# ytchen0323/cloud-scale-bwamem

Hardware: AMD Instinct MI355X
Metric: pair-end 2x150bp reads aligned/sec (higher is better)
Workload: dtype int32+u16

## Files before the change

### cloud-scale-bwamem_amd/bpsw_hip/__init__.py

```python
from __future__ import annotations

import ctypes as C
import os
from dataclasses import dataclass

import numpy as np

_HERE = os.path.dirname(os.path.abspath(__file__))
PKG_ROOT = os.path.dirname(_HERE)
LIB_PATH = os.environ.get("BPSW_LIB") or os.path.join(PKG_ROOT, "lib", "libbPSW_hip.so")
SYNTH_PATH = os.path.join(PKG_ROOT, "lib", "libbpsw_synth.so")

BPSW_OK = 0
ZDROP_SCALA, ZDROP_BWA = 0, 1
RESCUE_C, RESCUE_SCALA = 0, 1
KSW_XBYTE, KSW_XSTOP, KSW_XSUBO, KSW_XSTART = 0x10000, 0x20000, 0x40000, 0x80000

ABI_SYMBOLS = [
    "bpsw_device_count", "bpsw_create", "bpsw_destroy", "bpsw_device_of", "bpsw_device_cus", "bpsw_device_slots", "bpsw_device_for_partition", "bpsw_last_error", "bpsw_version",
    "bpsw_set_ext_scoring", "bpsw_set_ext_shortcuts", "bpsw_extend_batch", "bpsw_extend_stage", "bpsw_extend_commit", "bpsw_extend_batch_classify", "bpsw_extend_batch_device", "bpsw_wire_size", "bpsw_wire_pack", "bpsw_wire_coords_size", "bpsw_wire_coords_pack",
    "bpsw_opt_default", "bpsw_swalign2_batch", "bpsw_swalign2_batch_device", "bpsw_matesw_group", "bpsw_global_batch",
    "bpsw_get_stats", "bpsw_reset_stats", "bpsw_last_kernel_ms", "bpsw_ring_stats", "bpsw_sw_batches_in_flight", "bpsw_ring_integrity",
    "bpsw_ext_group_waiting", "bpsw_ext_group_counts",
    "bpsw_ref_load", "bpsw_ref_unload", "bpsw_ref_length", "bpsw_ref_fetch", "bpsw_chain2aln_batch",
    "bpsw_tail_opt_default", "bpsw_bns_load", "bpsw_reg2aln_batch", "bpsw_sam_pe_batch", "bpsw_worker2_batch", "bpsw_last_tail_times", "bpsw_last_tail_resubmitted",
    "bpsw_tail_pool_create", "bpsw_tail_pool_destroy", "bpsw_tail_pool_submit", "bpsw_tail_pool_wait", "bpsw_tail_pool_workers",
    "bpsw_mark_primary_se", "bpsw_approx_mapq_se", "bpsw_mem_pair", "bpsw_sort_dedup", "bpsw_pe_stat",
    "bpsw_fmi_load", "bpsw_fmi_unload", "bpsw_fmi_length", "bpsw_seed_opt_default", "bpsw_seed_batch", "bpsw_chain_seeds",
    "bpsw_worker1_batch", "bpsw_last_worker1_times", "bpsw_seed_set_resident_lanes",
    "bpsw_seed_batch_ex", "bpsw_last_seed_bytes", "bpsw_scan_set_tile",
    "bpsw_chain_batch", "bpsw_chain_set_arena_budget", "bpsw_chain_last_split",
    "bpsw_chain_batch_ex", "bpsw_last_chain_bytes",
    "bpsw_sam_se_batch", "bpsw_align_se_batch", "bpsw_last_sam_se_times",
    "bpsw_sam_pe_batch_ex", "bpsw_align_pe_batch", "bpsw_last_sam_pe_times",
    "bpsw_fastq_parse", "bpsw_align_fastq_se", "bpsw_align_fastq_pe", "bpsw_last_fastq_times",
    "bpsw_bam_se_batch", "bpsw_bam_pe_batch", "bpsw_align_bam_se_batch", "bpsw_align_bam_pe_batch", "bpsw_align_fastq_bam_se", "bpsw_align_fastq_bam_pe",
    "bpsw_sam_header", "bpsw_bam_header", "bpsw_bam_eof", "bpsw_bam_set_block_payload", "bpsw_last_bam_times", "bpsw_last_bam_deflate_times",
]
JNI_SYMBOLS = [
    "Java_cs_ucla_edu_bwaspark_jni_SWExtendFPGAJNI_swExtendFPGAJNI",
    "Java_cs_ucla_edu_bwaspark_jni_MateSWJNI_mateSWJNI",
    "Java_cs_ucla_edu_bwaspark_jni_HelloWorld_helloWorld",
    "Java_cs_ucla_edu_bwaspark_jni_MateSWJNI_loadPacJNI",
    "Java_cs_ucla_edu_bwaspark_jni_SWExtendFPGAJNI_chainToAlnJNI",
    "Java_cs_ucla_edu_bwaspark_jni_MateSWJNI_loadBnsJNI",
    "Java_cs_ucla_edu_bwaspark_jni_MateSWJNI_samPeTailJNI",
    "Java_cs_ucla_edu_bwaspark_jni_MateSWJNI_samPeTailSubmitJNI",
    "Java_cs_ucla_edu_bwaspark_jni_MateSWJNI_samPeTailCollectJNI",
    "Java_cs_ucla_edu_bwaspark_jni_MateSWJNI_samPeTailCancelJNI",
    "Java_cs_ucla_edu_bwaspark_jni_MateSWJNI_mateSWFlatJNI",
    "Java_cs_ucla_edu_bwaspark_jni_SWExtendFPGAJNI_loadFmiJNI",
    "Java_cs_ucla_edu_bwaspark_jni_SWExtendFPGAJNI_worker1FlatJNI",
]


class BpswError(RuntimeError):
    pass


class AlnReg(C.Structure):
    _fields_ = [("rb", C.c_int64), ("re", C.c_int64), ("qb", C.c_int32), ("qe", C.c_int32), ("score", C.c_int32),
                ("truesc", C.c_int32), ("sub", C.c_int32), ("csub", C.c_int32), ("sub_n", C.c_int32), ("w", C.c_int32),
                ("seedcov", C.c_int32), ("secondary", C.c_int32), ("hash", C.c_uint64)]


ALNREG_DTYPE = np.dtype([("rb", "<i8"), ("re", "<i8"), ("qb", "<i4"), ("qe", "<i4"), ("score", "<i4"),
                         ("truesc", "<i4"), ("sub", "<i4"), ("csub", "<i4"), ("sub_n", "<i4"), ("w", "<i4"),
                         ("seedcov", "<i4"), ("secondary", "<i4"), ("hash", "<u8")])
assert ALNREG_DTYPE.itemsize == 64 and C.sizeof(AlnReg) == 64


class PeStat(C.Structure):
    _fields_ = [("low", C.c_int32), ("high", C.c_int32), ("failed", C.c_int32), ("pad_", C.c_int32),
                ("avg", C.c_double), ("std", C.c_double)]


class Opt(C.Structure):
    _fields_ = [(n, C.c_int32) for n in ("a", "b", "o_del", "e_del", "o_ins", "e_ins", "pen_unpaired", "pen_clip5",
                                         "pen_clip3", "w", "zdrop", "T", "flag", "min_seed_len", "max_ins",
                                         "max_matesw")] + [("mask_level_redun", C.c_float), ("mat", C.c_int8 * 25),
                                                           ("pad_", C.c_int8 * 3)]


class ExtTasks(C.Structure):
    _fields_ = [("n", C.c_int32)] + [(n, C.c_int32) for n in ("o_del", "e_del", "o_ins", "e_ins", "pen_clip5",
                                                                "pen_clip3", "w", "mat_max")] + \
               [(n, C.c_void_p) for n in ("left_qlen", "left_rlen", "right_qlen", "right_rlen", "left_q_off",
                                          "left_r_off", "right_q_off", "right_r_off", "reg_score", "q_beg", "h0", "idx",
                                          "pool")]


class ExtCoordTasks(C.Structure):
    _fields_ = [("n", C.c_int32)] + [(n, C.c_int32) for n in ("o_del", "e_del", "o_ins", "e_ins", "pen_clip5",
                                                                "pen_clip3", "w", "mat_max")] + \
               [(n, C.c_void_p) for n in ("left_qlen", "left_rlen", "right_qlen", "right_rlen", "left_q_off", "right_q_off",
                                          "reg_score", "q_beg", "h0", "idx", "seed_len", "seed_rbeg", "pool")]


class SwJobs(C.Structure):
    _fields_ = [("n", C.c_int32), ("xtra", C.c_int32)] + \
               [(n, C.c_void_p) for n in ("q_len", "t_len", "q_off", "t_off", "q_rev", "q_pool", "t_pool")] + \
               [("q_pool_bytes", C.c_size_t), ("t_pool_bytes", C.c_size_t)]


class GlobalJobs(C.Structure):
    _fields_ = [("n", C.c_int32), ("max_cigar", C.c_int32)] + \
               [(n, C.c_void_p) for n in ("q_len", "t_len", "w", "q_off", "t_off", "q_pool", "t_pool")] + \
               [("q_pool_bytes", C.c_size_t), ("t_pool_bytes", C.c_size_t)]


class Chains(C.Structure):
    _fields_ = [("n_reads", C.c_int32), ("read_len", C.c_void_p), ("read_off", C.c_void_p), ("read_pool", C.c_void_p),
                ("read_pool_bytes", C.c_size_t), ("chain_cnt", C.c_void_p), ("seed_cnt", C.c_void_p), ("seed_rbeg", C.c_void_p),
                ("seed_qbeg", C.c_void_p), ("seed_len", C.c_void_p)]


C2A_SORT_DEDUP, C2A_DEDUP_SCALA = 1, 2
W1_CHAIN_DEVICE = 4
W1_SEED_PLAN_DEVICE = 8
W1_CHAINS_RESIDENT = 16
SEED_PLAN_DEVICE = 1
CHAIN_TABLES_DEVICE = 1


class RescueGroup(C.Structure):
    _fields_ = [("group_size", C.c_int32), ("l_pac", C.c_int64), ("pes", PeStat * 4), ("seq_len", C.c_void_p),
                ("seq_off", C.c_void_p), ("seq_pool", C.c_void_p), ("seq_pool_bytes", C.c_size_t),
                ("reg_cnt", C.c_void_p), ("regs", C.c_void_p), ("ref_cnt", C.c_void_p), ("ref_rb", C.c_void_p),
                ("ref_re", C.c_void_p), ("ref_len", C.c_void_p), ("ref_off", C.c_void_p), ("ref_pool", C.c_void_p),
                ("ref_pool_bytes", C.c_size_t)]


class Stats(C.Structure):
    _fields_ = [(n, C.c_uint64) for n in ("ext_calls", "ext_tasks", "ext_wire_bytes", "sw_calls", "sw_jobs",
                                          "sw_speculated", "sw_replayed_rounds", "sw_wasted")] + \
               [(n, C.c_double) for n in ("ext_h2d_ms", "ext_kernel_ms", "ext_d2h_ms", "sw_h2d_ms", "sw_kernel_ms",
                                          "sw_d2h_ms", "sw_host_ms", "ext_host_in_ms", "ext_wait_ms", "ext_dev_ms",
                                          "ext_host_out_ms", "grp_plan_ms", "grp_pack_ms", "grp_wait_ms", "grp_dev_ms",
                                          "grp_replay_ms", "grp_out_ms")] + [("grp_calls", C.c_uint64), ("grp_pairs", C.c_uint64), ("ext_full_relaunches", C.c_uint64), ("sw_ring_calls", C.c_uint64), ("ext_ring_calls", C.c_uint64)]


_lib = None


def load_library(path: str | None = None) -> C.CDLL:
    global _lib
    if _lib is not None and path is None:
        return _lib
    p = path or LIB_PATH
    if not os.path.exists(p):
        raise BpswError(f"{p} not found: build it with `make -C {PKG_ROOT}` (or __graft_entry__.build())")
    if os.environ.get("BPSW_NO_TORCH") != "1":
        try:
            import torch
        except Exception:
            pass
    lib = C.CDLL(p)
    lib.bpsw_last_error.restype = C.c_char_p
    lib.bpsw_version.restype = C.c_char_p
    lib.bpsw_create.argtypes = [C.c_int, C.POINTER(C.c_void_p)]
    lib.bpsw_destroy.argtypes = [C.c_void_p]
    lib.bpsw_destroy.restype = None
    lib.bpsw_device_of.argtypes = [C.c_void_p]
    lib.bpsw_device_cus.argtypes = [C.c_void_p]
    lib.bpsw_set_ext_scoring.argtypes = [C.c_void_p, C.c_void_p, C.c_int, C.c_int]
    lib.bpsw_set_ext_shortcuts.argtypes = [C.c_void_p, C.c_int]
    lib.bpsw_extend_batch.argtypes = [C.c_void_p, C.c_void_p, C.c_size_t, C.c_void_p, C.c_size_t]
    lib.bpsw_extend_batch_device.argtypes = [C.c_void_p, C.c_void_p, C.c_size_t, C.c_int, C.c_void_p, C.c_void_p]
    lib.bpsw_wire_size.argtypes = [C.POINTER(ExtTasks)]
    lib.bpsw_wire_size.restype = C.c_size_t
    lib.bpsw_wire_pack.argtypes = [C.POINTER(ExtTasks), C.c_void_p, C.c_size_t, C.POINTER(C.c_size_t)]
    lib.bpsw_wire_coords_size.argtypes = [C.POINTER(ExtCoordTasks)]
    lib.bpsw_wire_coords_size.restype = C.c_size_t
    lib.bpsw_wire_coords_pack.argtypes = [C.POINTER(ExtCoordTasks), C.c_void_p, C.c_size_t, C.POINTER(C.c_size_t)]
    lib.bpsw_opt_default.argtypes = [C.POINTER(Opt)]
    lib.bpsw_opt_default.restype = None
    lib.bpsw_swalign2_batch.argtypes = [C.c_void_p, C.POINTER(Opt), C.POINTER(SwJobs), C.c_void_p]
    lib.bpsw_swalign2_batch_device.argtypes = [C.c_void_p, C.POINTER(Opt), C.POINTER(SwJobs), C.c_void_p, C.c_void_p]
    lib.bpsw_matesw_group.argtypes = [C.c_void_p, C.POINTER(Opt), C.POINTER(RescueGroup), C.c_int, C.c_void_p,
                                      C.c_void_p, C.c_int64, C.POINTER(C.c_int64)]
    lib.bpsw_global_batch.argtypes = [C.c_void_p, C.POINTER(Opt), C.POINTER(GlobalJobs), C.c_void_p, C.c_void_p, C.c_void_p]
    lib.bpsw_get_stats.argtypes = [C.c_void_p, C.POINTER(Stats)]
    lib.bpsw_reset_stats.argtypes = [C.c_void_p]
    lib.bpsw_last_kernel_ms.argtypes = [C.c_void_p, C.POINTER(C.c_float), C.POINTER(C.c_float)]
    lib.bpsw_ring_stats.argtypes = [C.c_void_p, C.POINTER(C.c_uint64), C.POINTER(C.c_uint64), C.POINTER(C.c_uint64), C.POINTER(C.c_double), C.POINTER(C.c_uint64)]
    lib.bpsw_sw_batches_in_flight.argtypes = [C.c_int]
    lib.bpsw_ext_group_waiting.argtypes = [C.c_int]
    lib.bpsw_ext_group_counts.argtypes = [C.c_int, C.POINTER(C.c_uint64)]
    lib.bpsw_ring_integrity.argtypes = [C.POINTER(C.c_uint64), C.POINTER(C.c_uint64)]
    lib.bpsw_chain2aln_batch.argtypes = [C.c_void_p, C.POINTER(Opt), C.POINTER(Chains), C.c_int, C.c_int, C.c_void_p, C.c_void_p,
                                         C.c_int64, C.POINTER(C.c_int64)]
    lib.bpsw_ref_load.argtypes = [C.c_void_p, C.c_void_p, C.c_int64]
    lib.bpsw_ref_unload.argtypes = [C.c_void_p]
    lib.bpsw_ref_length.argtypes = [C.c_void_p]
    lib.bpsw_ref_length.restype = C.c_int64
    lib.bpsw_ref_fetch.argtypes = [C.c_void_p, C.c_int32, C.c_void_p, C.c_void_p, C.c_void_p, C.c_size_t, C.c_void_p, C.c_void_p]
    lib.bpsw_tail_opt_default.argtypes = [C.c_void_p]
    lib.bpsw_tail_opt_default.restype = None
    lib.bpsw_bns_load.argtypes = [C.c_void_p, C.c_int32, C.c_void_p, C.c_void_p, C.c_char_p]
    lib.bpsw_reg2aln_batch.argtypes = [C.c_void_p, C.POINTER(Opt), C.c_void_p, C.c_void_p, C.c_void_p, C.c_void_p, C.c_void_p]
    lib.bpsw_sam_pe_batch.argtypes = [C.c_void_p, C.POINTER(Opt), C.c_void_p, C.c_void_p, C.c_void_p, C.c_size_t, C.c_void_p,
                                      C.POINTER(C.c_size_t), C.c_void_p]
    lib.bpsw_worker2_batch.argtypes = [C.c_void_p, C.POINTER(Opt), C.c_void_p, C.c_void_p, C.c_int, C.c_void_p, C.c_size_t, C.c_void_p,
                                       C.POINTER(C.c_size_t), C.c_void_p, C.c_void_p, C.c_int64, C.POINTER(C.c_int64)]
    lib.bpsw_tail_pool_create.argtypes = [C.c_int, C.c_int, C.POINTER(C.c_void_p)]
    lib.bpsw_tail_pool_destroy.argtypes = [C.c_void_p]
    lib.bpsw_tail_pool_destroy.restype = None
    lib.bpsw_tail_pool_submit.argtypes = [C.c_void_p, C.POINTER(Opt), C.c_void_p, C.c_void_p, C.c_int, C.c_void_p, C.c_size_t, C.c_void_p,
                                          C.c_void_p, C.c_void_p, C.c_int64, C.POINTER(C.c_int64)]
    lib.bpsw_tail_pool_wait.argtypes = [C.c_void_p, C.c_int64, C.POINTER(C.c_size_t), C.POINTER(C.c_int64)]
    lib.bpsw_tail_pool_workers.argtypes = [C.c_void_p]
    lib.bpsw_mark_primary_se.argtypes = [C.POINTER(Opt), C.c_void_p, C.c_int32, C.c_void_p, C.c_int64]
    lib.bpsw_approx_mapq_se.argtypes = [C.POINTER(Opt), C.c_void_p, C.c_void_p]
    lib.bpsw_mem_pair.argtypes = [C.POINTER(Opt), C.c_void_p, C.c_int64, C.c_void_p, C.c_int32, C.c_void_p, C.c_int32, C.c_void_p, C.c_int64,
                                  C.c_void_p]
    lib.bpsw_sort_dedup.argtypes = [C.c_int32, C.c_void_p, C.c_float, C.c_int]
    lib.bpsw_pe_stat.argtypes = [C.POINTER(Opt), C.c_void_p, C.c_int64, C.c_int32, C.c_void_p, C.c_void_p, C.c_void_p]
    lib.bpsw_last_tail_times.argtypes = [C.c_void_p, C.POINTER(C.c_float), C.POINTER(C.c_int32), C.c_void_p]
    lib.bpsw_last_tail_resubmitted.argtypes = [C.c_void_p, C.POINTER(C.c_int32)]
    _bind_seeding(lib)
    if path is None:
        _lib = lib
    return lib


def _bind_seeding(lib):
    sig = {
        "bpsw_fmi_load": ([C.c_void_p, C.c_int64, C.c_void_p, C.c_int64, C.c_void_p, C.c_int64, C.c_int32, C.c_int64, C.c_void_p], C.c_int),
        "bpsw_fmi_unload": ([C.c_void_p], C.c_int),
        "bpsw_fmi_length": ([C.c_void_p], C.c_int64),
        "bpsw_seed_opt_default": ([C.c_void_p], None),
        "bpsw_seed_batch": ([C.c_void_p, C.c_void_p, C.c_void_p, C.c_void_p, C.c_void_p, C.c_int64, C.POINTER(C.c_int64), C.c_void_p, C.c_void_p,
                             C.c_int64, C.POINTER(C.c_int64)], C.c_int),
        "bpsw_seed_batch_ex": ([C.c_void_p, C.c_void_p, C.c_void_p, C.c_void_p, C.c_void_p, C.c_int64, C.POINTER(C.c_int64), C.c_void_p, C.c_void_p,
                                C.c_int64, C.POINTER(C.c_int64), C.c_int], C.c_int),
        "bpsw_last_seed_bytes": ([C.c_void_p], None),
        "bpsw_scan_set_tile": ([C.c_int], None),
        "bpsw_chain_seeds": ([C.c_void_p, C.c_int32, C.c_int64, C.c_int32, C.c_void_p, C.c_int32, C.c_void_p, C.c_int32, C.c_void_p], C.c_int),
        "bpsw_worker1_batch": ([C.c_void_p, C.POINTER(Opt), C.c_void_p, C.c_void_p, C.c_int, C.c_int, C.c_void_p, C.c_void_p, C.c_int64,
                                C.POINTER(C.c_int64)], C.c_int),
        "bpsw_last_worker1_times": ([C.c_void_p], None),
        "bpsw_seed_set_resident_lanes": ([C.c_int], None),
        "bpsw_chain_batch": ([C.c_void_p, C.c_void_p, C.c_int32, C.c_int64, C.c_int32, C.c_void_p, C.c_void_p, C.c_int32, C.c_void_p, C.c_void_p,
                              C.c_int64, C.c_void_p, C.c_int64, C.POINTER(C.c_int64), C.POINTER(C.c_int64)], C.c_int),
        "bpsw_chain_batch_ex": ([C.c_void_p, C.c_void_p, C.c_int32, C.c_int64, C.c_int32, C.c_void_p, C.c_void_p, C.c_int32, C.c_void_p, C.c_void_p,
                                 C.c_int64, C.c_void_p, C.c_int64, C.POINTER(C.c_int64), C.POINTER(C.c_int64), C.c_int], C.c_int),
        "bpsw_last_chain_bytes": ([C.c_void_p], None),
        "bpsw_chain_set_arena_budget": ([C.c_int64], None),
        "bpsw_chain_last_split": ([C.c_void_p], None),
        "bpsw_sam_se_batch": ([C.c_void_p, C.POINTER(Opt), C.c_void_p, C.c_void_p, C.c_int, C.c_void_p, C.c_size_t, C.c_void_p,
                               C.POINTER(C.c_size_t), C.c_void_p], C.c_int),
        "bpsw_align_se_batch": ([C.c_void_p, C.POINTER(Opt), C.c_void_p, C.c_void_p, C.c_void_p, C.c_int, C.c_int, C.c_int, C.c_void_p,
                                 C.c_size_t, C.c_void_p, C.POINTER(C.c_size_t)], C.c_int),
        "bpsw_last_sam_se_times": ([C.c_void_p], None),
        "bpsw_sam_pe_batch_ex": ([C.c_void_p, C.POINTER(Opt), C.c_void_p, C.c_void_p, C.c_int, C.c_void_p, C.c_size_t, C.c_void_p,
                                  C.POINTER(C.c_size_t), C.c_void_p], C.c_int),
        "bpsw_align_pe_batch": ([C.c_void_p, C.POINTER(Opt), C.c_void_p, C.c_void_p, C.c_void_p, C.c_void_p, C.c_int, C.c_int, C.c_int, C.c_int,
                                 C.c_void_p, C.c_size_t, C.c_void_p, C.POINTER(C.c_size_t), C.c_void_p], C.c_int),
        "bpsw_last_sam_pe_times": ([C.c_void_p], None),
        "bpsw_fastq_parse": ([C.c_void_p, C.c_char_p, C.c_size_t, C.c_char_p, C.c_size_t, C.c_int, C.c_int64, C.c_size_t, C.c_size_t, C.c_void_p,
                              C.c_void_p, C.c_void_p, C.c_void_p, C.c_void_p, C.c_void_p, C.POINTER(C.c_int64), C.c_void_p, C.c_void_p], C.c_int),
        "bpsw_align_fastq_se": ([C.c_void_p, C.POINTER(Opt), C.c_void_p, C.c_void_p, C.c_char_p, C.c_size_t, C.c_int, C.c_int64, C.c_int32, C.c_int,
                                 C.c_int, C.c_int, C.c_void_p, C.c_size_t, C.c_void_p, C.c_int64, C.POINTER(C.c_size_t), C.POINTER(C.c_int64),
                                 C.c_void_p], C.c_int),
        "bpsw_align_fastq_pe": ([C.c_void_p, C.POINTER(Opt), C.c_void_p, C.c_void_p, C.c_char_p, C.c_size_t, C.c_char_p, C.c_size_t, C.c_int,
                                 C.c_int64, C.c_void_p, C.c_int, C.c_int, C.c_int, C.c_int, C.c_void_p, C.c_size_t, C.c_void_p, C.c_int64,
                                 C.POINTER(C.c_size_t), C.c_void_p, C.POINTER(C.c_int64), C.c_void_p], C.c_int),
        "bpsw_last_fastq_times": ([C.c_void_p], None),
        "bpsw_bam_se_batch": ([C.c_void_p, C.POINTER(Opt), C.c_void_p, C.c_void_p, C.c_int, C.c_void_p, C.c_size_t, C.POINTER(C.c_size_t),
                               C.c_void_p], C.c_int),
        "bpsw_bam_pe_batch": ([C.c_void_p, C.POINTER(Opt), C.c_void_p, C.c_void_p, C.c_int, C.c_void_p, C.c_size_t, C.POINTER(C.c_size_t),
                               C.c_void_p], C.c_int),
        "bpsw_align_bam_se_batch": ([C.c_void_p, C.POINTER(Opt), C.c_void_p, C.c_void_p, C.c_void_p, C.c_int, C.c_int, C.c_int, C.c_void_p,
                                     C.c_size_t, C.POINTER(C.c_size_t)], C.c_int),
        "bpsw_align_bam_pe_batch": ([C.c_void_p, C.POINTER(Opt), C.c_void_p, C.c_void_p, C.c_void_p, C.c_void_p, C.c_int, C.c_int, C.c_int, C.c_int,
                                     C.c_void_p, C.c_size_t, C.POINTER(C.c_size_t), C.c_void_p], C.c_int),
        "bpsw_align_fastq_bam_se": ([C.c_void_p, C.POINTER(Opt), C.c_void_p, C.c_void_p, C.c_char_p, C.c_size_t, C.c_int, C.c_int64, C.c_int32,
                                     C.c_int, C.c_int, C.c_int, C.c_void_p, C.c_size_t, C.POINTER(C.c_size_t), C.POINTER(C.c_int64), C.c_void_p],
                                    C.c_int),
        "bpsw_align_fastq_bam_pe": ([C.c_void_p, C.POINTER(Opt), C.c_void_p, C.c_void_p, C.c_char_p, C.c_size_t, C.c_char_p, C.c_size_t, C.c_int,
                                     C.c_int64, C.c_void_p, C.c_int, C.c_int, C.c_int, C.c_int, C.c_void_p, C.c_size_t, C.POINTER(C.c_size_t),
                                     C.c_void_p, C.POINTER(C.c_int64), C.c_void_p], C.c_int),
        "bpsw_sam_header": ([C.c_void_p, C.c_int32, C.c_void_p, C.c_char_p, C.c_char_p, C.c_size_t, C.c_void_p, C.c_size_t, C.POINTER(C.c_size_t)],
                            C.c_int),
        "bpsw_bam_header": ([C.c_void_p, C.c_int32, C.c_void_p, C.c_char_p, C.c_char_p, C.c_size_t, C.c_void_p, C.c_size_t, C.POINTER(C.c_size_t)],
                            C.c_int),
        "bpsw_bam_eof": ([C.c_void_p, C.c_size_t, C.POINTER(C.c_size_t)], C.c_int),
        "bpsw_bam_set_block_payload": ([C.c_int], C.c_int),
        "bpsw_last_bam_times": ([C.c_void_p], None),
        "bpsw_last_bam_deflate_times": ([C.c_void_p], None),
    }
    for name, (args, res) in sig.items():
        fn = getattr(lib, name, None)
        if fn is not None:
            fn.argtypes, fn.restype = args, res


def _ptr(a: np.ndarray | None):
    return None if a is None else a.ctypes.data_as(C.c_void_p)


def _chk(lib, rc, what):
    if rc != BPSW_OK:
        raise BpswError(f"{what} failed ({rc}): {lib.bpsw_last_error().decode()}")


def default_opt() -> Opt:
    o = Opt()
    load_library().bpsw_opt_default(C.byref(o))
    return o


@dataclass
class ExtTaskSoA:
    left_qlen: np.ndarray
    left_rlen: np.ndarray
    right_qlen: np.ndarray
    right_rlen: np.ndarray
    left_q_off: np.ndarray
    left_r_off: np.ndarray
    right_q_off: np.ndarray
    right_r_off: np.ndarray
    reg_score: np.ndarray
    q_beg: np.ndarray
    h0: np.ndarray
    idx: np.ndarray
    pool: np.ndarray
    o_del: int = 6
    e_del: int = 1
    o_ins: int = 6
    e_ins: int = 1
    pen_clip5: int = 5
    pen_clip3: int = 5
    w: int = 100
    mat_max: int = 1

    @property
    def n(self) -> int:
        return int(self.left_qlen.shape[0])

    def subset(self, sel) -> "ExtTaskSoA":
        kw = {k: getattr(self, k)[sel] for k in ("left_qlen", "left_rlen", "right_qlen", "right_rlen", "left_q_off",
                                                  "left_r_off", "right_q_off", "right_r_off", "reg_score", "q_beg",
                                                  "h0", "idx")}
        return ExtTaskSoA(pool=self.pool, o_del=self.o_del, e_del=self.e_del, o_ins=self.o_ins, e_ins=self.e_ins,
                          pen_clip5=self.pen_clip5, pen_clip3=self.pen_clip3, w=self.w, mat_max=self.mat_max,
                          **{k: np.ascontiguousarray(v) for k, v in kw.items()})

    def as_struct(self) -> ExtTasks:
        t = ExtTasks()
        t.n = self.n
        for f in ("o_del", "e_del", "o_ins", "e_ins", "pen_clip5", "pen_clip3", "w", "mat_max"):
            setattr(t, f, int(getattr(self, f)))
        for f in ("left_qlen", "left_rlen", "right_qlen", "right_rlen", "reg_score", "q_beg", "h0", "idx"):
            a = getattr(self, f)
            assert a.dtype == np.int32 and a.flags.c_contiguous
            setattr(t, f, a.ctypes.data)
        for f in ("left_q_off", "left_r_off", "right_q_off", "right_r_off"):
            a = getattr(self, f)
            assert a.dtype == np.int64 and a.flags.c_contiguous
            setattr(t, f, a.ctypes.data)
        assert self.pool.dtype == np.uint8
        t.pool = self.pool.ctypes.data
        return t


@dataclass
class ExtCoordTaskSoA:
    left_qlen: np.ndarray
    left_rlen: np.ndarray
    right_qlen: np.ndarray
    right_rlen: np.ndarray
    left_q_off: np.ndarray
    right_q_off: np.ndarray
    reg_score: np.ndarray
    q_beg: np.ndarray
    h0: np.ndarray
    idx: np.ndarray
    seed_len: np.ndarray
    seed_rbeg: np.ndarray
    pool: np.ndarray
    o_del: int = 6
    e_del: int = 1
    o_ins: int = 6
    e_ins: int = 1
    pen_clip5: int = 5
    pen_clip3: int = 5
    w: int = 100
    mat_max: int = 1

    @property
    def n(self) -> int:
        return int(self.left_qlen.shape[0])

    def as_struct(self) -> ExtCoordTasks:
        t = ExtCoordTasks()
        t.n = self.n
        for f in ("o_del", "e_del", "o_ins", "e_ins", "pen_clip5", "pen_clip3", "w", "mat_max"):
            setattr(t, f, int(getattr(self, f)))
        for f in ("left_qlen", "left_rlen", "right_qlen", "right_rlen", "reg_score", "q_beg", "h0", "idx", "seed_len"):
            a = getattr(self, f)
            assert a.dtype == np.int32 and a.flags.c_contiguous
            setattr(t, f, a.ctypes.data)
        for f in ("left_q_off", "right_q_off", "seed_rbeg"):
            a = getattr(self, f)
            assert a.dtype == np.int64 and a.flags.c_contiguous
            setattr(t, f, a.ctypes.data)
        assert self.pool.dtype == np.uint8
        t.pool = self.pool.ctypes.data
        return t


def wire_coords_pack(tasks: ExtCoordTaskSoA) -> np.ndarray:
    lib = load_library()
    st = tasks.as_struct()
    size = lib.bpsw_wire_coords_size(C.byref(st))
    buf = np.zeros(size, dtype=np.uint8)
    used = C.c_size_t(0)
    _chk(lib, lib.bpsw_wire_coords_pack(C.byref(st), _ptr(buf), size, C.byref(used)), "bpsw_wire_coords_pack")
    return buf[: used.value]


def wire_pack(tasks: ExtTaskSoA) -> np.ndarray:
    lib = load_library()
    st = tasks.as_struct()
    size = lib.bpsw_wire_size(C.byref(st))
    buf = np.zeros(size, dtype=np.uint8)
    used = C.c_size_t(0)
    _chk(lib, lib.bpsw_wire_pack(C.byref(st), _ptr(buf), size, C.byref(used)), "bpsw_wire_pack")
    return buf[: used.value]


class Context:

    def __init__(self, device: int = -1):
        self.lib = load_library()
        h = C.c_void_p()
        _chk(self.lib, self.lib.bpsw_create(device, C.byref(h)), "bpsw_create")
        self.h = h

    def close(self):
        if self.h:
            self.lib.bpsw_destroy(self.h)
            self.h = None

    def __del__(self):
        try:
            self.close()
        except Exception:
            pass

    @property
    def device(self) -> int:
        return self.lib.bpsw_device_of(self.h)

    def set_ext_scoring(self, mat=None, zdrop: int = 100, zdrop_mode: int = ZDROP_SCALA):
        m = None if mat is None else np.ascontiguousarray(mat, dtype=np.int8)
        _chk(self.lib, self.lib.bpsw_set_ext_scoring(self.h, _ptr(m), zdrop, zdrop_mode), "bpsw_set_ext_scoring")

    def set_ext_shortcuts(self, mask: int = -1):
        _chk(self.lib, self.lib.bpsw_set_ext_shortcuts(self.h, C.c_int(mask)), "bpsw_set_ext_shortcuts")

    def extend_batch(self, wire: np.ndarray) -> np.ndarray:
        wire = np.ascontiguousarray(wire, dtype=np.uint8)
        n = int(np.frombuffer(wire[8:12].tobytes(), dtype="<i4")[0]) if wire.size >= 12 else 0
        out = np.zeros(max(10 * n, 1), dtype=np.int16)
        _chk(self.lib, self.lib.bpsw_extend_batch(self.h, _ptr(wire), wire.size, _ptr(out), out.size), "bpsw_extend_batch")
        return out[: 10 * n]

    def extend_batch_classify(self, wire: np.ndarray):
        wire = np.ascontiguousarray(wire, dtype=np.uint8)
        n = int(np.frombuffer(wire[8:12].tobytes(), dtype="<i4")[0]) if wire.size >= 12 else 0
        out = np.zeros(max(10 * n, 1), dtype=np.int16)
        how = np.zeros((max(n, 1), 2), dtype=np.uint8)
        self.lib.bpsw_extend_batch_classify.argtypes = [C.c_void_p, C.c_void_p, C.c_size_t, C.c_void_p, C.c_size_t, C.c_void_p]
        _chk(self.lib, self.lib.bpsw_extend_batch_classify(self.h, _ptr(wire), wire.size, _ptr(out), out.size, _ptr(how)),
             "bpsw_extend_batch_classify")
        return out[: 10 * n], how[:n]

    def extend_batch_device(self, d_wire_ptr: int, wire_bytes: int, n_tasks: int, d_out_ptr: int, stream: int = 0):
        _chk(self.lib, self.lib.bpsw_extend_batch_device(self.h, C.c_void_p(d_wire_ptr), wire_bytes, n_tasks,
                                                        C.c_void_p(d_out_ptr), C.c_void_p(stream)),
             "bpsw_extend_batch_device")

    def swalign2_batch(self, opt: Opt, xtra: int, q_len, t_len, q_off, t_off, q_rev, q_pool, t_pool) -> np.ndarray:
        j = SwJobs()
        arrs = dict(q_len=np.ascontiguousarray(q_len, np.int32), t_len=np.ascontiguousarray(t_len, np.int32),
                    q_off=np.ascontiguousarray(q_off, np.int64), t_off=np.ascontiguousarray(t_off, np.int64),
                    q_rev=np.ascontiguousarray(q_rev, np.uint8), q_pool=np.ascontiguousarray(q_pool, np.uint8))
        if t_pool is not None:
            arrs["t_pool"] = np.ascontiguousarray(t_pool, np.uint8)
        j.n = int(arrs["q_len"].shape[0])
        j.xtra = int(xtra)
        for k, a in arrs.items():
            setattr(j, k, a.ctypes.data)
        j.q_pool_bytes = arrs["q_pool"].size
        j.t_pool_bytes = arrs["t_pool"].size if t_pool is not None else 0
        out = np.zeros((max(j.n, 1), 7), dtype=np.int32)
        _chk(self.lib, self.lib.bpsw_swalign2_batch(self.h, C.byref(opt), C.byref(j), _ptr(out)), "bpsw_swalign2_batch")
        return out[: j.n]

    def swalign2_batch_device(self, opt: Opt, jobs: SwJobs, d_out_ptr: int, stream: int = 0):
        _chk(self.lib, self.lib.bpsw_swalign2_batch_device(self.h, C.byref(opt), C.byref(jobs), C.c_void_p(d_out_ptr),
                                                          C.c_void_p(stream)), "bpsw_swalign2_batch_device")

    def global_batch(self, opt: Opt, q_len, t_len, w, q_off, t_off, q_pool, t_pool, max_cigar: int = 64):
        j = GlobalJobs()
        arrs = dict(q_len=np.ascontiguousarray(q_len, np.int32), t_len=np.ascontiguousarray(t_len, np.int32),
                    w=np.ascontiguousarray(w, np.int32), q_off=np.ascontiguousarray(q_off, np.int64),
                    t_off=np.ascontiguousarray(t_off, np.int64), q_pool=np.ascontiguousarray(q_pool, np.uint8),
                    t_pool=np.ascontiguousarray(t_pool, np.uint8))
        j.n, j.max_cigar = int(arrs["q_len"].shape[0]), int(max_cigar)
        for k, a in arrs.items():
            setattr(j, k, a.ctypes.data)
        j.q_pool_bytes, j.t_pool_bytes = arrs["q_pool"].size, arrs["t_pool"].size
        score = np.zeros(max(j.n, 1), np.int32)
        ncig = np.zeros(max(j.n, 1), np.int32)
        cig = np.zeros((max(j.n, 1), max_cigar), np.uint32)
        _chk(self.lib, self.lib.bpsw_global_batch(self.h, C.byref(opt), C.byref(j), _ptr(score), _ptr(ncig), _ptr(cig)),
             "bpsw_global_batch")
        return score[: j.n], ncig[: j.n], cig[: j.n]

    def matesw_group(self, opt: Opt, g: "RescueGroupSoA", mode: int = RESCUE_C):
        st = g.as_struct()
        out_cnt = np.zeros(2 * g.group_size, dtype=np.int32)
        cap = int(g.regs.shape[0] + 4 * g.ref_rb.shape[0] + 16)
        out = np.empty(cap, dtype=ALNREG_DTYPE)
        total = C.c_int64(0)
        _chk(self.lib, self.lib.bpsw_matesw_group(self.h, C.byref(opt), C.byref(st), mode, _ptr(out_cnt), _ptr(out), cap,
                                                 C.byref(total)), "bpsw_matesw_group")
        return out_cnt, out[: total.value]

    def ref_load(self, pac: np.ndarray, l_pac: int):
        pac = np.ascontiguousarray(pac, np.uint8)
        if pac.size < (int(l_pac) + 3) // 4:
            raise BpswError("pac shorter than (l_pac+3)/4 bytes")
        _chk(self.lib, self.lib.bpsw_ref_load(self.h, _ptr(pac), int(l_pac)), "bpsw_ref_load")

    def ref_unload(self):
        _chk(self.lib, self.lib.bpsw_ref_unload(self.h), "bpsw_ref_unload")

    def ref_length(self) -> int:
        return int(self.lib.bpsw_ref_length(self.h))

    def ref_fetch(self, beg, end):
        beg = np.ascontiguousarray(beg, np.int64)
        end = np.ascontiguousarray(end, np.int64)
        n = int(beg.shape[0])
        span = np.abs(end - beg) + 16
        off = np.zeros(n, np.int64)
        if n > 1:
            off[1:] = np.cumsum((span[:-1] + 15) & ~15)
        total = int(off[-1] + span[-1]) if n else 0
        pool = np.zeros(max(total, 16), np.uint8)
        lens = np.zeros(max(n, 1), np.int64)
        _chk(self.lib, self.lib.bpsw_ref_fetch(self.h, n, _ptr(beg), _ptr(end), _ptr(pool), pool.size, _ptr(off), _ptr(lens)),
             "bpsw_ref_fetch")
        return [pool[off[i]: off[i] + lens[i]].copy() for i in range(n)], lens[:n]

    def chain2aln_batch(self, opt: Opt, b: "ChainBatchSoA", zdrop_mode: int = ZDROP_SCALA, flags: int = 0):
        st = Chains()
        st.n_reads = b.n_reads
        for f, dt in (("read_len", np.int32), ("read_off", np.int64), ("read_pool", np.uint8), ("chain_cnt", np.int32),
                      ("seed_cnt", np.int32), ("seed_rbeg", np.int64), ("seed_qbeg", np.int32), ("seed_len", np.int32)):
            a = getattr(b, f)
            assert a.dtype == dt and a.flags.c_contiguous, f
            setattr(st, f, a.ctypes.data)
        st.read_pool_bytes = b.read_pool.size
        cap = int(b.seed_len.shape[0]) + 8
        out_cnt = np.zeros(max(b.n_reads, 1), np.int32)
        out = np.empty(cap, dtype=ALNREG_DTYPE)
        total = C.c_int64(0)
        _chk(self.lib, self.lib.bpsw_chain2aln_batch(self.h, C.byref(opt), C.byref(st), zdrop_mode, flags, _ptr(out_cnt), _ptr(out), cap,
                                                    C.byref(total)), "bpsw_chain2aln_batch")
        return out_cnt[: b.n_reads], out[: total.value]

    def fmi_load(self, idx):
        L2 = np.ascontiguousarray(idx.L2, np.int64)
        bwt = np.ascontiguousarray(idx.bwt, np.uint32)
        sa = np.ascontiguousarray(idx.sa, np.int64)
        _chk(self.lib, self.lib.bpsw_fmi_load(self.h, int(idx.primary), _ptr(L2), int(idx.seq_len), _ptr(bwt), bwt.size, int(idx.sa_intv),
                                             sa.size, _ptr(sa)), "bpsw_fmi_load")

    def fmi_unload(self):
        _chk(self.lib, self.lib.bpsw_fmi_unload(self.h), "bpsw_fmi_unload")

    def fmi_length(self) -> int:
        return int(self.lib.bpsw_fmi_length(self.h))

    def seed_batch(self, sopt, reads, flags: int | None = None, intervals: bool = True):
        from . import fmi
        st = reads.as_struct()
        n = reads.n_reads
        icnt, scnt = np.zeros(max(n, 1), np.int32), np.zeros(max(n, 1), np.int32)
        icap, scap = 8 * n + 64, 16 * n + 64
        if flags is None:
            assert intervals
        elif not intervals:
            icap = 0
        while True:
            iv, sv = (np.zeros(icap, fmi.SMEM_DTYPE) if intervals else None), np.zeros(scap, fmi.SEED_DTYPE)
            it, stt = C.c_int64(0), C.c_int64(0)
            if flags is None:
                rc = self.lib.bpsw_seed_batch(self.h, C.byref(sopt), C.byref(st), _ptr(icnt), _ptr(iv), icap, C.byref(it), _ptr(scnt), _ptr(sv),
                                              scap, C.byref(stt))
            else:
                rc = self.lib.bpsw_seed_batch_ex(self.h, C.byref(sopt), C.byref(st), _ptr(icnt), _ptr(iv), icap, C.byref(it), _ptr(scnt),
                                                 _ptr(sv), scap, C.byref(stt), flags)
            if rc == -3 and ((intervals and it.value > icap) or stt.value > scap):
                icap, scap = (max(icap, it.value) if intervals else 0), max(scap, stt.value)
                continue
            _chk(self.lib, rc, "bpsw_seed_batch" if flags is None else "bpsw_seed_batch_ex")
            return icnt[:n], (iv[: it.value] if intervals else None), scnt[:n], sv[: stt.value]

    def last_seed_bytes(self):
        b = (C.c_int64 * 2)()
        self.lib.bpsw_last_seed_bytes(b)
        return int(b[0]), int(b[1])

    def chain_batch(self, sopt, w: int, l_pac: int, seed_cnt, seeds, filter: bool = True, flags: int = 0):
        from . import fmi
        seed_cnt = np.ascontiguousarray(seed_cnt, np.int32)
        seeds = np.ascontiguousarray(seeds, fmi.SEED_DTYPE)
        n = int(seed_cnt.shape[0])
        assert int(seed_cnt.sum()) == seeds.shape[0]
        chain_cnt = np.zeros(max(n, 1), np.int32)
        ccap, scap = n + 64, 2 * n + 64
        while True:
            cnt, out = np.zeros(ccap, np.int32), np.zeros(scap, fmi.SEED_DTYPE)
            ct, st = C.c_int64(0), C.c_int64(0)
            if flags == 0:
                rc = self.lib.bpsw_chain_batch(self.h, C.byref(sopt), w, l_pac, n, _ptr(seed_cnt), _ptr(seeds), 1 if filter else 0, _ptr(chain_cnt),
                                               _ptr(cnt), ccap, _ptr(out), scap, C.byref(ct), C.byref(st))
            else:
                rc = self.lib.bpsw_chain_batch_ex(self.h, C.byref(sopt), w, l_pac, n, _ptr(seed_cnt), _ptr(seeds), 1 if filter else 0,
                                                  _ptr(chain_cnt), _ptr(cnt), ccap, _ptr(out), scap, C.byref(ct), C.byref(st), flags)
            if rc == -3 and (ct.value > ccap or st.value > scap):
                ccap, scap = max(ccap, ct.value), max(scap, st.value)
                continue
            _chk(self.lib, rc, "bpsw_chain_batch" if flags == 0 else "bpsw_chain_batch_ex")
            return chain_cnt[:n], cnt[: ct.value], out[: st.value]

    def worker1_batch(self, opt: Opt, sopt, reads, zdrop_mode: int = ZDROP_SCALA, flags: int = 0):
        st = reads.as_struct()
        n = reads.n_reads
        out_cnt = np.zeros(max(n, 1), np.int32)
        cap = 4 * n + 64
        while True:
            out = np.empty(cap, dtype=ALNREG_DTYPE)
            total = C.c_int64(0)
            rc = self.lib.bpsw_worker1_batch(self.h, C.byref(opt), C.byref(sopt), C.byref(st), zdrop_mode, flags, _ptr(out_cnt), _ptr(out), cap,
                                             C.byref(total))
            if rc == -3 and total.value > cap:
                cap = total.value
                continue
            _chk(self.lib, rc, "bpsw_worker1_batch")
            return out_cnt[:n], out[: total.value]

    def ring_stats(self):
        e, s, c = C.c_uint64(0), C.c_uint64(0), C.c_uint64(0)
        _chk(self.lib, self.lib.bpsw_ring_stats(self.h, C.byref(e), C.byref(s), C.byref(c), None, None), "bpsw_ring_stats")
        return int(e.value), int(s.value), int(c.value)

    def ring_integrity(self):
        a, b = C.c_uint64(0), C.c_uint64(0)
        on = self.lib.bpsw_ring_integrity(C.byref(a), C.byref(b))
        return bool(on), int(a.value), int(b.value)

    def sw_batches_in_flight(self):
        return int(self.lib.bpsw_sw_batches_in_flight(self.lib.bpsw_device_of(self.h)))

    def ext_group_waiting(self):
        return int(self.lib.bpsw_ext_group_waiting(self.lib.bpsw_device_of(self.h)))

    def ext_group_counts(self):
        out = (C.c_uint64 * 3)()
        _chk(self.lib, self.lib.bpsw_ext_group_counts(self.lib.bpsw_device_of(self.h), out), "bpsw_ext_group_counts")
        return int(out[0]), int(out[1]), int(out[2])

    def ring_epoch_times(self):
        ms, n = C.c_double(0.0), C.c_uint64(0)
        _chk(self.lib, self.lib.bpsw_ring_stats(self.h, None, None, None, C.byref(ms), C.byref(n)), "bpsw_ring_stats")
        return float(ms.value), int(n.value)

    def stats(self) -> Stats:
        s = Stats()
        _chk(self.lib, self.lib.bpsw_get_stats(self.h, C.byref(s)), "bpsw_get_stats")
        return s

    def last_kernel_ms(self):
        a, b = C.c_float(0), C.c_float(0)
        _chk(self.lib, self.lib.bpsw_last_kernel_ms(self.h, C.byref(a), C.byref(b)), "bpsw_last_kernel_ms")
        return a.value, b.value


def default_seed_opt():
    from . import fmi
    o = fmi.SeedOpt()
    load_library().bpsw_seed_opt_default(C.byref(o))
    return o


def chain_seeds(sopt, w: int, l_pac: int, seeds: np.ndarray, filter: bool = True):
    from . import fmi
    seeds = np.ascontiguousarray(seeds, fmi.SEED_DTYPE)
    n = int(seeds.shape[0])
    cnt = np.zeros(n + 1, np.int32)
    out = np.zeros(n + 1, fmi.SEED_DTYPE)
    lib = load_library()
    nc = lib.bpsw_chain_seeds(C.byref(sopt), w, l_pac, n, _ptr(seeds), 1 if filter else 0, _ptr(cnt), n, _ptr(out))
    if nc < 0:
        _chk(lib, nc, "bpsw_chain_seeds")
    return cnt[:nc].copy(), out[: int(cnt[:nc].sum())].copy()


def chain_last_split():
    st = (C.c_int64 * 4)()
    load_library().bpsw_chain_last_split(st)
    return tuple(st)


def last_chain_bytes():
    b = (C.c_int64 * 2)()
    load_library().bpsw_last_chain_bytes(b)
    return int(b[0]), int(b[1])


def last_worker1_times():
    ms = (C.c_double * 3)()
    load_library().bpsw_last_worker1_times(ms)
    return tuple(ms)


@dataclass
class ChainBatchSoA:
    l_pac: int
    read_len: np.ndarray
    read_off: np.ndarray
    read_pool: np.ndarray
    chain_cnt: np.ndarray
    seed_cnt: np.ndarray
    seed_rbeg: np.ndarray
    seed_qbeg: np.ndarray
    seed_len: np.ndarray

    @property
    def n_reads(self) -> int:
        return int(self.read_len.shape[0])

    def slice(self, lo: int, hi: int) -> "ChainBatchSoA":
        c0, c1 = int(self.chain_cnt[:lo].sum()), int(self.chain_cnt[:hi].sum())
        s0, s1 = int(self.seed_cnt[:c0].sum()), int(self.seed_cnt[:c1].sum())
        cp = np.ascontiguousarray
        return ChainBatchSoA(l_pac=self.l_pac, read_len=cp(self.read_len[lo:hi]), read_off=cp(self.read_off[lo:hi]),
                             read_pool=self.read_pool, chain_cnt=cp(self.chain_cnt[lo:hi]), seed_cnt=cp(self.seed_cnt[c0:c1]),
                             seed_rbeg=cp(self.seed_rbeg[s0:s1]), seed_qbeg=cp(self.seed_qbeg[s0:s1]), seed_len=cp(self.seed_len[s0:s1]))


@dataclass
class RescueGroupSoA:
    group_size: int
    l_pac: int
    pes: list
    seq_len: np.ndarray
    seq_off: np.ndarray
    seq_pool: np.ndarray
    reg_cnt: np.ndarray
    regs: np.ndarray
    ref_cnt: np.ndarray
    ref_rb: np.ndarray
    ref_re: np.ndarray
    ref_len: np.ndarray
    ref_off: np.ndarray
    ref_pool: np.ndarray | None

    def as_struct(self) -> RescueGroup:
        g = RescueGroup()
        g.group_size = self.group_size
        g.l_pac = self.l_pac
        for r in range(4):
            lo, hi, failed, avg, std = self.pes[r]
            g.pes[r].low, g.pes[r].high, g.pes[r].failed, g.pes[r].avg, g.pes[r].std = int(lo), int(hi), int(failed), float(avg), float(std)
        for f, dt in (("seq_len", np.int32), ("seq_off", np.int64), ("seq_pool", np.uint8), ("reg_cnt", np.int32),
                      ("ref_cnt", np.int32), ("ref_rb", np.int64), ("ref_re", np.int64), ("ref_len", np.int64),
                      ("ref_off", np.int64), ("ref_pool", np.uint8)):
            a = getattr(self, f)
            if a is None and f in ("ref_pool", "ref_len", "ref_off"):
                continue
            assert a.dtype == dt and a.flags.c_contiguous, f
            setattr(g, f, a.ctypes.data)
        assert self.regs.dtype == ALNREG_DTYPE
        g.regs = self.regs.ctypes.data
        g.seq_pool_bytes = self.seq_pool.size
        g.ref_pool_bytes = self.ref_pool.size if self.ref_pool is not None else 0
        return g


@dataclass
class TailGroupSoA:
    group_size: int
    l_pac: int
    id0: int
    pes: list
    read_len: np.ndarray
    read_off: np.ndarray
    read_pool: np.ndarray
    qual_pool: np.ndarray | None
    name_off: np.ndarray
    name_pool: np.ndarray
    reg_cnt: np.ndarray
    regs: np.ndarray
    ann_off: np.ndarray
    ann_len: np.ndarray
    ann_name_off: np.ndarray
    ann_name_pool: np.ndarray


def make_tail_group(chain_batch, names, qual_pool, pes, reg_cnt, regs, ann_off, ann_len, ann_names, id0=0) -> TailGroupSoA:
    n = chain_batch.n_reads
    assert n % 2 == 0 and len(names) == n // 2

    def pool(strs):
        off = np.zeros(len(strs) + 1, np.int64)
        bs = [s.encode() for s in strs]
        off[1:] = np.cumsum([len(b) for b in bs])
        return off, np.frombuffer(b"".join(bs) + b"\0", np.uint8).copy()

    name_off, name_pool = pool(names)
    a_off, a_pool = pool(ann_names)
    cp = np.ascontiguousarray
    return TailGroupSoA(group_size=n // 2, l_pac=int(chain_batch.l_pac), id0=int(id0), pes=list(pes), read_len=cp(chain_batch.read_len),
                        read_off=cp(chain_batch.read_off), read_pool=cp(chain_batch.read_pool),
                        qual_pool=None if qual_pool is None else cp(qual_pool, np.uint8), name_off=name_off, name_pool=name_pool,
                        reg_cnt=cp(reg_cnt, np.int32), regs=cp(regs), ann_off=cp(ann_off, np.int64), ann_len=cp(ann_len, np.int32),
                        ann_name_off=a_off, ann_name_pool=a_pool)


TAIL_SCALA, TAIL_C = 0, 1
MEM_F_NOPAIRING, MEM_F_ALL, MEM_F_NO_MULTI = 0x4, 0x8, 0x10
ALN_OK, ALN_XREF, ALN_NOCIGAR, ALN_OVERFLOW = 0, 1, 2, 3
ALN_DTYPE = np.dtype([("pos", "<i8"), ("rid", "<i4"), ("flag", "<i4"), ("is_rev", "<i4"), ("mapq", "<i4"), ("NM", "<i4"),
                      ("n_cigar", "<i4"), ("score", "<i4"), ("sub", "<i4"), ("md_len", "<i4"), ("status", "<i4")])


class TailOpt(C.Structure):
    _fields_ = [("mask_level", C.c_float), ("mapq_coef_len", C.c_float), ("mapq_coef_fac", C.c_int32), ("flavour", C.c_int32),
                ("rg_id", C.c_char * 64)]


class Reg2AlnJobs(C.Structure):
    _fields_ = [("n", C.c_int32), ("max_cigar", C.c_int32), ("max_md", C.c_int32), ("read_len", C.c_void_p), ("read_off", C.c_void_p),
                ("read_pool", C.c_void_p), ("read_pool_bytes", C.c_size_t), ("regs", C.c_void_p)]


class Pairs(C.Structure):
    _fields_ = [("group_size", C.c_int32), ("id0", C.c_int64), ("pes", PeStat * 4), ("read_len", C.c_void_p), ("read_off", C.c_void_p),
                ("read_pool", C.c_void_p), ("qual_pool", C.c_void_p), ("read_pool_bytes", C.c_size_t), ("name_off", C.c_void_p),
                ("name_pool", C.c_void_p), ("reg_cnt", C.c_void_p), ("regs", C.c_void_p)]


def default_tail_opt(flavour: int = TAIL_SCALA) -> TailOpt:
    t = TailOpt()
    load_library().bpsw_tail_opt_default(C.byref(t))
    t.flavour = flavour
    return t


def _ctx_bns_load(self, ann_off, ann_len, names=None):
    off = np.ascontiguousarray(ann_off, np.int64)
    ln = np.ascontiguousarray(ann_len, np.int32)
    blob = None if names is None else b"".join(n.encode() + b"\0" for n in names)
    _chk(self.lib, self.lib.bpsw_bns_load(self.h, int(off.shape[0]), _ptr(off), _ptr(ln), blob), "bpsw_bns_load")


def _ctx_reg2aln_batch(self, opt: Opt, topt: TailOpt, read_len, read_off, read_pool, regs, max_cigar: int = 64, max_md: int = 256):
    rl = np.ascontiguousarray(read_len, np.int32); ro = np.ascontiguousarray(read_off, np.int64)
    rp = np.ascontiguousarray(read_pool, np.uint8); rg = np.ascontiguousarray(regs)
    assert rg.dtype == ALNREG_DTYPE
    j = Reg2AlnJobs()
    j.n, j.max_cigar, j.max_md = int(rg.shape[0]), int(max_cigar), int(max_md)
    j.read_len, j.read_off, j.read_pool, j.read_pool_bytes, j.regs = rl.ctypes.data, ro.ctypes.data, rp.ctypes.data, rp.size, rg.ctypes.data
    alns = np.zeros(max(j.n, 1), ALN_DTYPE)
    cig = np.zeros((max(j.n, 1), max_cigar), np.uint32)
    md = np.zeros((max(j.n, 1), max_md), np.uint8)
    _chk(self.lib, self.lib.bpsw_reg2aln_batch(self.h, C.byref(opt), C.byref(topt), C.byref(j), _ptr(alns), _ptr(cig), _ptr(md)),
         "bpsw_reg2aln_batch")
    return alns[: j.n], cig[: j.n], md[: j.n]


def _pes_struct(pes):
    a = (PeStat * 4)()
    for r in range(4):
        lo, hi, failed, avg, std = pes[r]
        a[r].low, a[r].high, a[r].failed, a[r].avg, a[r].std = int(lo), int(hi), int(failed), float(avg), float(std)
    return a


def _reads_into(st, g, with_regs: bool):
    keep = []
    for f, dt in (("read_len", np.int32), ("read_off", np.int64), ("read_pool", np.uint8), ("name_off", np.int64), ("name_pool", np.uint8)):
        a = np.ascontiguousarray(getattr(g, f), dt)
        keep.append(a)
        setattr(st, f, a.ctypes.data)
    if g.qual_pool is not None:
        q = np.ascontiguousarray(g.qual_pool, np.uint8)
        keep.append(q)
        st.qual_pool = q.ctypes.data
    st.read_pool_bytes = int(np.asarray(g.read_pool).size)
    if not with_regs:
        return keep, None, None
    cnt = np.ascontiguousarray(g.reg_cnt, np.int32)
    regs = np.ascontiguousarray(g.regs)
    assert regs.dtype == ALNREG_DTYPE
    keep += [cnt, regs]
    st.reg_cnt, st.regs = cnt.ctypes.data, regs.ctypes.data
    return keep, cnt, regs


def _pairs_struct(g, with_regs: bool = True):
    st = Pairs()
    st.group_size, st.id0 = g.group_size, g.id0
    st.pes = _pes_struct(g.pes)
    keep, _, regs = _reads_into(st, g, with_regs)
    return st, keep, regs


def _text_call(lib, what, n, call, text_cap, per_read=512, slack=0, grow=None):
    off = np.zeros(n + 1, np.int64)
    need = C.c_size_t(0)
    cap = per_read * max(1, n) if text_cap is None else int(text_cap)
    while True:
        buf = np.empty(max(cap, 1), np.uint8)
        rc = call(_ptr(buf), cap, _ptr(off), C.byref(need))
        if rc == -3 and text_cap is None:
            short = [need.value > cap, grow is not None and grow()]
            if any(short):
                cap = max(cap, int(need.value) + slack)
                continue
        _chk(lib, rc, what)
        break
    text = buf[: int(off[-1])].tobytes()
    return [text[int(off[i]):int(off[i + 1])] for i in range(n)]


def _ctx_sam_pe_batch(self, opt: Opt, topt: TailOpt, g: "TailGroupSoA", flags: int = 0):
    st, keep, regs = _pairs_struct(g)
    out_regs = np.zeros(max(regs.shape[0], 1), ALNREG_DTYPE)
    head = (self.h, C.byref(opt), C.byref(topt), C.byref(st))
    if flags:
        call = lambda buf, cap, off, need: self.lib.bpsw_sam_pe_batch_ex(*head, flags, buf, cap, off, need, _ptr(out_regs))
    else:
        call = lambda buf, cap, off, need: self.lib.bpsw_sam_pe_batch(*head, buf, cap, off, need, _ptr(out_regs))
    texts = _text_call(self.lib, "bpsw_sam_pe_batch", 2 * g.group_size, call, None, per_read=1024, slack=64)
    return texts, out_regs[: regs.shape[0]]


def _ctx_worker2_batch(self, opt: Opt, topt: TailOpt, g: "TailGroupSoA", rescue_mode: int = RESCUE_C):
    st, keep, regs = _pairs_struct(g)
    cnt = np.zeros(2 * g.group_size, np.int32)
    total = C.c_int64(0)
    out = {"cap": int(regs.shape[0]) + 8 * g.group_size + 64, "regs": None}

    def call(buf, cap, off, need):
        out["regs"] = np.empty(out["cap"], ALNREG_DTYPE)
        return self.lib.bpsw_worker2_batch(self.h, C.byref(opt), C.byref(topt), C.byref(st), rescue_mode, buf, cap, off, need, _ptr(cnt),
                                           _ptr(out["regs"]), out["cap"], C.byref(total))

    def grow():
        short = total.value > out["cap"]
        out["cap"] = max(out["cap"], int(total.value) + 16)
        return short

    texts = _text_call(self.lib, "bpsw_worker2_batch", 2 * g.group_size, call, None, per_read=1024, slack=64, grow=grow)
    return texts, cnt, out["regs"][: total.value]


def _ctx_last_tail_kernel(self):
    ms, n = C.c_float(0), C.c_int32(0)
    _chk(self.lib, self.lib.bpsw_last_tail_times(self.h, C.byref(ms), C.byref(n), None), "bpsw_last_tail_times")
    return ms.value, n.value


# ... 446 lines not shown
```

### cloud-scale-bwamem_amd/csrc/bpsw_ext_group.h

```cpp
#pragma once

#include <condition_variable>
#include <deque>
#include <mutex>

namespace bpsw {

struct ExtGroupWaiter {
  enum State { WAITING, LEADER, TAKEN, DONE };
  std::condition_variable cv;
  State state = WAITING;
  bool compatible = false;
  void* item = nullptr;
  int slot = -1;
  int status = 0;
  float span_ms = 0.f;
  int group_n = 1;
};

class ExtGroupQueue {
 public:
  static constexpr int NO_SLOT = -1, OWN_SLOT = -2;
  static constexpr int MAX_GROUP = 8;

  template <class Take>
  bool acquire(ExtGroupWaiter& w, int max_group, Take&& take, ExtGroupWaiter** members, int* n_members) {
    *n_members = 0;
    std::unique_lock<std::mutex> lk(mu_);
    if (waiters_.empty()) {
      const int s = take();
      if (s != NO_SLOT) {
        w.slot = s;
        w.state = ExtGroupWaiter::LEADER;
        if (w.compatible) count_group(1);
        return true;
      }
    }
    w.state = ExtGroupWaiter::WAITING;
    waiters_.push_back(&w);
    w.cv.wait(lk, [&] { return w.state == ExtGroupWaiter::LEADER || w.state == ExtGroupWaiter::DONE; });
    if (w.state == ExtGroupWaiter::DONE) return false;
    if (w.compatible) {
      if (max_group > MAX_GROUP) max_group = MAX_GROUP;
      for (auto it = waiters_.begin(); it != waiters_.end() && *n_members + 1 < max_group;) {
        if ((*it)->compatible) {
          (*it)->state = ExtGroupWaiter::TAKEN;
          members[(*n_members)++] = *it;
          it = waiters_.erase(it);
        } else {
          ++it;
        }
      }
      count_group(1 + *n_members);
    }
    return true;
  }

  void complete(ExtGroupWaiter** members, int n_members, int status, float span_ms) {
    std::lock_guard<std::mutex> lk(mu_);
    for (int i = 0; i < n_members; ++i) {
      ExtGroupWaiter* m = members[i];
      m->status = status;
      m->span_ms = span_ms;
      m->group_n = 1 + n_members;
      m->state = ExtGroupWaiter::DONE;
      m->cv.notify_one();
    }
  }

  template <class Put, class Take>
  void release(Put&& put, Take&& take) {
    std::lock_guard<std::mutex> lk(mu_);
    put();
    while (!waiters_.empty()) {
      const int s = take();
      if (s < 0) break;
      ExtGroupWaiter* w = waiters_.front();
      waiters_.pop_front();
      w->slot = s;
      w->state = ExtGroupWaiter::LEADER;
      w->cv.notify_one();
    }
  }

  int waiting() {
    std::lock_guard<std::mutex> lk(mu_);
    return (int)waiters_.size();
  }
  int waiting_compatible() {
    std::lock_guard<std::mutex> lk(mu_);
    int n = 0;
    for (const ExtGroupWaiter* w : waiters_) n += w->compatible ? 1 : 0;
    return n;
  }
  void counts(unsigned long long out[3]) {
    std::lock_guard<std::mutex> lk(mu_);
    out[0] = groups_; out[1] = members_; out[2] = largest_;
  }

 private:
  void count_group(int n) {
    ++groups_;
    members_ += (unsigned long long)n;
    if ((unsigned long long)n > largest_) largest_ = (unsigned long long)n;
  }
  std::mutex mu_;
  std::deque<ExtGroupWaiter*> waiters_;
  unsigned long long groups_ = 0, members_ = 0, largest_ = 0;
};

}
```

### cloud-scale-bwamem_amd/csrc/bpsw_internal.h

```cpp
#pragma once

#include <hip/hip_runtime.h>
#include <stddef.h>
#include <stdint.h>

#include <condition_variable>
#include <cstdlib>
#include <mutex>
#include <string>
#include <vector>

#include "bpsw.h"
#include "bpsw_ext_group.h"
#include "bpsw_ring.h"

struct bpsw_ctx;

#include <hip/hip_ext.h>

namespace bpsw {

struct KernelEvents {
  hipEvent_t start = nullptr, stop = nullptr;
};
// ... 45 lines not shown
                             const int* d_todo_list = nullptr);
hipError_t launch_ext_sift_kernel(const uint32_t* d_wire, int n_tasks, int16_t* d_out, const ExtScoring& sc, int dmn, int qmax,
                                  uint8_t* d_flag, uint4* d_recs, hipStream_t s, KernelEvents kev = KernelEvents(),
                                  const ExtPrepass* d_pre_check = nullptr, int* d_todo_count = nullptr, int* d_todo_list = nullptr,
                                  int heavy_min = 0);
struct ExtMember {
  const uint32_t* wire;
  int16_t* out;
  int* queue;
  const int* task_list;
  const ExtPrepass* pre;
  int* defer;
  int* defer_post;
  uint8_t* sift_flag;
  uint4* sift_recs;
  int* todo_count;
  int* todo_list;
  ExtScoring sc;
  int n_tasks, short_qmax;
  int sift_dm, sift_dn, sift_qmax, heavy_min;
};
constexpr int EXT_GROUP_SLOTS = 8;
struct ExtGroupArgs {
  ExtMember m[EXT_GROUP_SLOTS];
};
static_assert(sizeof(ExtGroupArgs) <= 2048, "the descriptors travel in the kernel arguments (4 KB in all)");
struct ExtGroupMember {
  ExtMember m;
  int qcap, rcap;
};
hipError_t launch_ext_sift_members(const ExtMember* m, int k, int n_grid, hipStream_t s, KernelEvents kev);
extern "C" hipError_t launch_ext_group(const ExtGroupMember* members, int k, int num_cu, hipStream_t s, KernelEvents kev);
int sift_uniform_dm(const int8_t mat[25], int exact_a);
int sift_uniform_dn(const int8_t mat[25], int exact_a);
struct SwScoring {
  MatRows mat;
  int a, b, o_del, e_del, o_ins, e_ins;
  int xtra;
};
int make_scoring(const char* who, const bpsw_opt_t* opt, int xtra, int min_gap_ext, SwScoring* sc);

struct SwJobsDev {
  int n;
  const int32_t* q_len;
  const int32_t* t_len;
  const int64_t* q_off;
  const int64_t* t_off;
  const uint8_t* q_rev;
  const uint8_t* q_pool;
  const uint8_t* t_pool;
  const uint8_t* pac = nullptr;
  long long l_pac = 0;
  const uint32_t* packed = nullptr;
};

struct SwPrepass {
  int max_qlen;
  int max_tlen;
  int error;
  int reserved;
};
void launch_sw_prepass(const SwJobsDev& jobs, size_t q_pool_bytes, size_t t_pool_bytes, SwPrepass* d_pre, hipStream_t s);
void launch_ref_fetch(const uint8_t* d_pac, long long l_pac, int n, const long long* d_beg, const long long* d_end,
                      uint8_t* d_out_pool, size_t out_pool_bytes, const long long* d_out_off, long long* d_out_len,
                      int* d_error, hipStream_t s);
size_t sw_scratch_bytes_per_wave(int max_tlen);
bool sw_quad_enabled();
int sw_resident_waves(int num_cu);
inline bool sw_halves_for(int max_qlen) {
  static const bool off = getenv("BPSW_SW_HALVES") && atoi(getenv("BPSW_SW_HALVES")) == 0;
  return !off && max_qlen >= 1 && max_qlen <= 150;
}
hipError_t launch_sw_kernel(const SwJobsDev& jobs, const SwScoring& sc, int max_qlen, int max_tlen, int32_t* d_out,
                            uint32_t* d_scratch, int num_cu, hipStream_t s, const SwPrepass* d_pre_check = nullptr, KernelEvents kev = KernelEvents());

int sw_ring_class(const SwScoring& sc, int max_qlen, int max_tlen, int* bias_out);
hipError_t launch_swp_resident(int c_class, const RingArgs& A, int blocks, hipStream_t s);
hipError_t launch_ext_resident(const RingArgs& A, int blocks, hipStream_t s);

bool ring_enabled();
bool ring_usable(int device, int c_class);
int ring_submit(int device, int c_class, int num_cu, const RingDesc& desc);
int ring_wait(int device, int c_class, const RingDone* done, uint32_t value, double* est_ms);
constexpr int BPSW_RING_RELAUNCH = 1001;
double ring_ticks_per_ms(int device, int c_class);
bool ring_integrity_on();
void ring_poison(uint32_t* first_word, size_t stride_words, size_t n_records, size_t second_word_offset);
int ring_check(const uint32_t* first_word, size_t stride_words, size_t n_records, size_t second_word_offset, const char* what);
struct RingRecords {
  uint32_t* first_word;
  size_t stride_words, n_records, second_word_offset;
  const char* what;
};
struct RingRun {
  enum How {
    done,
    launch,
    unwritten,
    failed,
  } how;
  int rc;
  bool submitted;
  float span_ms;
};
RingRun ring_run(int device, int c_class, int num_cu, const void* payload, size_t payload_bytes, uint32_t n_units, RingDone* done,
                 uint32_t* seq, double* wait_est_ms, const RingRecords& recs);
void ring_integrity_stats(uint64_t* checked, uint64_t* faults);
void ring_pause(int device);
void ring_resume(int device);
struct RingPause {
  int d;
  explicit RingPause(int dev) : d(dev) { ring_pause(d); }
  ~RingPause() { ring_resume(d); }
  RingPause(const RingPause&) = delete;
  RingPause& operator=(const RingPause&) = delete;
};
void ring_get_stats(int device, uint64_t* epochs, uint64_t* submitted, uint64_t* carried, double* epochs_ms = nullptr, uint64_t* epochs_timed = nullptr);

struct GlobalJobsDev {
  int n;
  int max_cigar;
  const int32_t* q_len;
  const int32_t* t_len;
  const int32_t* w;
  const int64_t* q_off;
  const int64_t* t_off;
  const uint8_t* q_pool;
  const uint8_t* t_pool;
};
struct GlobalPrepass {
  int max_qlen;
  int error;
  unsigned long long max_z;
};
inline int launch_waves(int resident, int n) {
  const long long whole = ((long long)n + 3) / 4 * 4;
  return whole < resident ? (int)whole : resident;
}
void launch_global_prepass(const GlobalJobsDev& jobs, size_t q_pool_bytes, size_t t_pool_bytes, GlobalPrepass* d_pre, hipStream_t s);
int global_resident_waves(int num_cu, int qcap);
hipError_t launch_global_kernel(const GlobalJobsDev& jobs, const SwScoring& sc, int max_qlen, size_t z_per_wave,
                                int32_t* d_score, int32_t* d_ncigar, uint32_t* d_cigar, uint8_t* d_z, int num_cu,
                                hipStream_t s);

struct Reg2AlnDev {
  int n;
  int max_cigar, max_md;
  int flavour;
  int opt_w, a;
  const int32_t* read_len;
  const long long* read_off;
  const uint8_t* read_pool;
  const bpsw_alnreg_t* regs;
  const uint8_t* pac;
  long long l_pac;
  int n_seqs;
  const long long* ann_off;
  const int32_t* ann_len;
};
struct Reg2AlnOut {
  long long pos;
  int32_t rid, is_rev, NM, n_cigar, md_len, status, gscore, pad_;
};
size_t reg2aln_lds_per_wave(int qcap, int rcap, int md_cap);
int reg2aln_resident_waves(int num_cu, int qcap, int rcap, int md_cap);
hipError_t launch_reg2aln_kernel(const Reg2AlnDev& J, const SwScoring& sc, int qcap, int rcap, int md_cap, size_t z_per_wave,
                                 Reg2AlnOut* d_out, uint32_t* d_cigar, uint8_t* d_md, uint8_t* d_z, int num_cu, hipStream_t s);

struct ChainParams {
  MatRows mat;
  int mat_max, a, o_del, e_del, o_ins, e_ins, pen_clip5, pen_clip3, w, zdrop, zmode;
  int exact_a;
  int tail_bound, certify;
};
struct ChainBatchDev {
  int n_reads;
  const int32_t* read_len;
  const long long* read_off;
  const uint8_t* read_pool;
  const int32_t* chain_cnt;
  const int32_t* chain_base;
  const int32_t* seed_cnt;
  const long long* seed_base;
  const long long* seed_rbeg;
  const int32_t* seed_qbeg;
  const int32_t* seed_len;
  const long long* reg_base;
  const uint8_t* pac;
  long long l_pac;
};
int chain2aln_resident_waves(int num_cu);
hipError_t launch_chain2aln_kernel(const ChainBatchDev& B, const ChainParams& P, bpsw_alnreg_t* d_out_regs, int32_t* d_out_cnt,
                                   int32_t* d_srt_scratch, int srt_per_wave, int num_cu, int* d_counter, hipStream_t s);
int sort_dedup_regs(std::vector<bpsw_alnreg_t>& v, float mask_level_redun, int mode);
void rescue_scratch_free(void* p);

void set_error(const std::string& msg);
int fail(int code, const std::string& msg);
inline int hip_fail(hipError_t e, const char* what) { return fail(BPSW_ERR_DEVICE, std::string(what) + ": " + hipGetErrorString(e)); }
#define HIP_TRY(expr)                                         \
  do {                                                        \
    hipError_t e_ = (expr);                                   \
    if (e_ != hipSuccess) return ::bpsw::hip_fail(e_, #expr); \
  } while (0)
inline size_t align16(size_t v) { return (v + 15) & ~(size_t)15; }

struct DeviceBuffer {
  void* ptr = nullptr;
  size_t cap = 0;
  hipError_t reserve(size_t bytes);
  void release();
};
struct PinnedBuffer {
  void* ptr = nullptr;
  size_t cap = 0;
  hipError_t reserve(size_t bytes);
  void release();
};
}
#include "bpsw_stage.h"
namespace bpsw {

struct RefGate;
struct RefDepthSlot { const RefGate* gate; int depth; };
inline thread_local RefDepthSlot t_ref_depth[8] = {};
inline int* ref_depth_of(const RefGate* g) {
  RefDepthSlot* free_slot = nullptr;
  for (RefDepthSlot& s : t_ref_depth) {
    if (s.gate == g) return &s.depth;
    if (!free_slot && s.depth == 0) free_slot = &s;
  }
  if (!free_slot) abort();
  free_slot->gate = g;
  free_slot->depth = 0;
  return &free_slot->depth;
}
struct RefGate {
  std::mutex m;
  std::condition_variable cv;
  int readers = 0, writers_waiting = 0;
  bool writing = false;
  void read_lock() {
    int* depth = ref_depth_of(this);
    std::unique_lock<std::mutex> lk(m);
    if (*depth == 0) cv.wait(lk, [&] { return !writing && writers_waiting == 0; });
    else cv.wait(lk, [&] { return !writing; });
    ++readers;
    ++*depth;
  }
  void read_unlock() {
    int* depth = ref_depth_of(this);
    if (*depth <= 0) abort();
    std::lock_guard<std::mutex> lk(m);
    --*depth;
    if (--readers == 0) cv.notify_all();
  }
  void write_lock() {
    std::unique_lock<std::mutex> lk(m);
    ++writers_waiting;
    cv.wait(lk, [&] { return !writing && readers == 0; });
    --writers_waiting;
    writing = true;
  }
  void write_unlock() { { std::lock_guard<std::mutex> lk(m); writing = false; } cv.notify_all(); }
};
struct RefHold {
  RefGate* g = nullptr;
  RefHold() = default;
  explicit RefHold(RefGate* gate) : g(gate) { if (g) g->read_lock(); }
  RefHold(RefHold&& o) noexcept : g(o.g) { o.g = nullptr; }
  RefHold& operator=(RefHold&& o) noexcept { if (this != &o) { release(); g = o.g; o.g = nullptr; } return *this; }
  RefHold(const RefHold&) = delete;
  RefHold& operator=(const RefHold&) = delete;
  void release() { if (g) { g->read_unlock(); g = nullptr; } }
  ~RefHold() { release(); }
};
struct RefWriteHold {
  RefGate* g;
  explicit RefWriteHold(RefGate* gate) : g(gate) { g->write_lock(); }
  ~RefWriteHold() { g->write_unlock(); }
  RefWriteHold(const RefWriteHold&) = delete;
  RefWriteHold& operator=(const RefWriteHold&) = delete;
};

struct DeviceRef {
  RefGate gate;
  std::mutex mu;
  DeviceBuffer buf;
  long long l_pac = 0;
  DeviceBuffer ann;
  std::vector<long long> ann_off;
  std::vector<int32_t> ann_len;
  std::vector<std::string> ann_name;
};
DeviceRef& device_ref(int device);

struct StreamLease {
  int device;
  hipStream_t s;
  bool pooled;
  bool led = false;
  int slot = -1;
  double wait_ms;
  explicit StreamLease(bpsw_ctx* c, ExtGroupWaiter* w = nullptr, ExtGroupWaiter** members = nullptr, int* n_members = nullptr);
  ~StreamLease();
  StreamLease(const StreamLease&) = delete;
  StreamLease& operator=(const StreamLease&) = delete;
};
struct CopyLane {
  std::mutex mu;
  hipStream_t s = nullptr;
  hipEvent_t ev = nullptr;
};
CopyLane& copy_lane(int device);
double wall_ms();
int ext_group_max();
int ext_group_waiting(int device);
void ext_group_counts(int device, unsigned long long out[3]);
void ext_group_complete(int device, ExtGroupWaiter** members, int n_members, int status, float span_ms);
void ext_call_mark(int device);
double ext_call_age_ms(int device);
double stat_ms();
int sw_launches_in_flight(int device);
void sw_launch_in_flight(int device, int delta);
double wait_est_update(double est, double took_ms, int polls, bool napped);
bool wait_naps(double est_ms);
void wait_nap(double est_ms);
void wait_poll_pause(int polls, double waited_ms, double est_ms);
hipError_t wait_event(bpsw_ctx* c, hipEvent_t ev, int kind);
int zerocopy_mask();
bool spin_wait();
[[nodiscard]] RefHold ref_snapshot(const bpsw_ctx* c, const uint8_t** pac, long long* l_pac);

int finish_pending_ext(bpsw_ctx* c);
int finish_pending_sw(bpsw_ctx* c);
inline int finish_pending(bpsw_ctx* c) {
  const int a = finish_pending_ext(c), b = finish_pending_sw(c);
  return a != BPSW_OK ? a : b;
}

int run_sw_jobs_host(bpsw_ctx* c, const bpsw_opt_t* opt, const bpsw_sw_jobs_t* jobs, int32_t* out);
struct SwStage {
  int n;
  size_t o_qlen, o_tlen, o_qoff, o_toff, o_qrev, o_qpool, o_tpool, o_packed, total, q_pool_bytes, t_pool_bytes;
  uint8_t* base;
};
int sw_stage_begin(bpsw_ctx* c, int n, size_t q_pool_bytes, size_t t_pool_bytes, SwStage* st);
int sw_stage_run(bpsw_ctx* c, const bpsw_opt_t* opt, int xtra, const SwStage& st, int mq, int mt, bool pac_mode, const int32_t** results);

struct ChainDevJob {
  int n_reads;
  const long long* seed_beg;
  const bpsw_seed_t* d_seeds;
  const bpsw_seed_t* h_seeds;
  int filter, drop_bridging;
};
struct ChainDevResult {
  std::vector<int32_t> chain_cnt, chain_seed_cnt;
  std::vector<bpsw_seed_t> seeds;
};
struct ChainTablesDev {
  const int32_t* chain_cnt;
  const int32_t* chain_base;
  const long long* reg_base;
  const int32_t* seed_cnt;
  const long long* seed_base;
  const long long* seed_rbeg;
  const int32_t* seed_qbeg;
  const int32_t* seed_len;
  long long nchains, nseeds;
  int max_seeds;
};
int chain_dev_run(bpsw_ctx* c, const bpsw_seed_opt_t& so, int w, int64_t l_pac, const ChainDevJob& J, ChainDevResult* R,
                  ChainTablesDev* T = nullptr);

int chain2aln_check(const bpsw_opt_t* opt, int zdrop_mode, int n, const int32_t* read_len, const int64_t* read_off, size_t read_pool_bytes);
int chain2aln_back(bpsw_ctx* c, const bpsw_opt_t* opt, int zdrop_mode, int flags, ChainBatchDev B, StageIn& in, int i_rlen, int i_roff,
                   int i_pool, long long nseeds, int max_seeds, const long long* h_reg_base, int32_t* out_cnt, bpsw_alnreg_t* out_regs,
                   int64_t out_cap, int64_t* out_total);

int scan_tile_items();
long long scan_tiles(long long n, int tile);
hipError_t scan_exclusive_i64(hipStream_t s, long long* data, int cols, long long n, int tile, long long* tile_sums);

}

struct bpsw_ctx {
  int device = 0;
  int num_cu = 256;
  hipStream_t stream = nullptr;
  hipEvent_t ev[8] = {nullptr, nullptr, nullptr, nullptr, nullptr, nullptr, nullptr, nullptr};
  std::mutex mu;
  bpsw::ExtScoring ext_sc;
  int8_t ext_mat[25];
  bpsw::DeviceBuffer d_wire, d_out, d_pre, d_sw_in, d_sw_out, d_sw_scratch, d_gl_z, d_ext_lists;
  size_t staged_bytes = 0;
  bpsw::DeviceBuffer d_sift;
  bpsw::DeviceBuffer d_seed[5];
  bpsw::DeviceBuffer d_chain;
  struct PendingExt { bool active = false; const void* d_wire = nullptr; size_t wire_bytes = 0; int n_tasks = 0; void* d_out = nullptr;
                      hipStream_t s = nullptr; int qcap = 0, rcap = 0; } pend_ext;
  int ext_geom_q = 0, ext_geom_r = 0;
  struct PendingSw { bool active = false; bpsw_sw_jobs_t jobs; bpsw_opt_t opt; void* d_out = nullptr; hipStream_t s = nullptr;
                     int cap_qlen = 0, cap_tlen = 0;
                     bool verified = false;
  } pend_sw;
  int sw_geom_qlen = 0, sw_geom_tlen = 0;
  float last_tail_ms = 0.f;
  int last_tail_jobs = 0, last_tail_resubmitted = 0;
  double tail_host_ms[3] = {0., 0., 0.};
  bool have_tail_ev = false;

  bpsw::PinnedBuffer h_stage_in, h_stage_out, h_pre;
  int shortcut_mask = 63;
  std::vector<int> ext_long_tasks;
  double wait_est_ms[6] = {0., 0., 0., 0., 0., 0.};
  bool ring_abandoned = false;
  uint32_t ring_seq = 0;
  void* rescue_scratch = nullptr;
  bpsw_stats_t stats;
  float last_ext_ms = 0.f, last_sw_ms = 0.f;
  bool have_ext_ev = false, have_sw_ev = false;
  bpsw::DeviceBuffer d_chain_tab;
};

namespace bpsw {
struct ContextEntry {
  std::unique_lock<std::mutex> lock;
  int rc = BPSW_OK;
  explicit ContextEntry(bpsw_ctx* c) : lock(c->mu) {
    if (c->ring_abandoned) { rc = fail(BPSW_ERR_DEVICE, "this context gave up a ring batch (watchdog / integrity): create a new one"); return; }
    const hipError_t e = hipSetDevice(c->device);
    if (e != hipSuccess) { rc = fail(BPSW_ERR_DEVICE, std::string("hipSetDevice: ") + hipGetErrorString(e)); return; }
    rc = finish_pending(c);
  }
};
}
```

### cloud-scale-bwamem_amd/csrc/bpsw_runtime.cpp

```cpp
#include <stdlib.h>
#include <string.h>

#include <sched.h>
#include <time.h>

#include <algorithm>
#include <atomic>
#include <condition_variable>

#pragma weak launch_ext_group
#include "bpsw_internal.h"

namespace bpsw {

static thread_local std::string g_err;
void set_error(const std::string& msg) { g_err = msg; }
int fail(int code, const std::string& msg) {
  g_err = msg;
  return code;
}

struct RingPauseForFree {
  int dev = 0;
  RingPauseForFree() { if (hipGetDevice(&dev) != hipSuccess) dev = 0; ring_pause(dev); }
  ~RingPauseForFree() { ring_resume(dev); }
};

hipError_t DeviceBuffer::reserve(size_t bytes) {
  if (bytes <= cap) return hipSuccess;
  size_t want = cap ? cap : 1 << 20;
  while (want < bytes) want <<= 1;
  if (ptr) { RingPauseForFree paused; (void)hipFree(ptr); }
  ptr = nullptr;
  cap = 0;
  hipError_t e = hipMalloc(&ptr, want);
  if (e == hipSuccess) cap = want;
  return e;
}
void DeviceBuffer::release() {
  if (ptr) { RingPauseForFree paused; (void)hipFree(ptr); }
  ptr = nullptr;
  cap = 0;
}
hipError_t PinnedBuffer::reserve(size_t bytes) {
  if (bytes <= cap) return hipSuccess;
  size_t want = cap ? cap : 1 << 20;
  while (want < bytes) want <<= 1;
  if (ptr) { RingPauseForFree paused; (void)hipHostFree(ptr); }
  ptr = nullptr;
  cap = 0;
  hipError_t e = hipHostMalloc(&ptr, want, hipHostMallocDefault);
  if (e == hipSuccess) cap = want;
  return e;
}
void PinnedBuffer::release() {
  if (ptr) { RingPauseForFree paused; (void)hipHostFree(ptr); }
  ptr = nullptr;
  cap = 0;
}

MatRows pack_mat(const int8_t mat[25]) {
  MatRows m;
  for (int k = 0; k < 5; ++k) {
    unsigned long long r = 0;
    for (int c = 0; c < 5; ++c) r |= (unsigned long long)(uint8_t)mat[k * 5 + c] << (8 * c);
    m.row[k] = r;
  }
  return m;
}

int make_scoring(const char* who, const bpsw_opt_t* opt, int xtra, int min_gap_ext, SwScoring* sc) {
  if (!opt) return fail(BPSW_ERR_ARG, std::string(who) + ": null options");
  if (opt->a < 1 || opt->o_del < 0 || opt->e_del < min_gap_ext || opt->o_ins < 0 || opt->e_ins < min_gap_ext)
    return fail(BPSW_ERR_ARG, std::string(who) + (min_gap_ext > 0 ? ": scoring must have a >= 1, non-negative gap opens and gap extensions >= 1"
                                                                  : ": scoring must have a >= 1 and non-negative gap penalties"));
  sc->mat = pack_mat(opt->mat);
  sc->a = opt->a; sc->b = opt->b;
  sc->o_del = opt->o_del; sc->e_del = opt->e_del; sc->o_ins = opt->o_ins; sc->e_ins = opt->e_ins;
  sc->xtra = xtra;
  return BPSW_OK;
}


int certify_level(const int8_t mat[25]) {
  if (exact_match_score(mat) != 1) return 1;
  for (int r = 0; r < 5; ++r)
    for (int c = 0; c < 5; ++c)
      if (!(r == c && r < 4) && mat[r * 5 + c] > -1) return 1;
  return 3;
}

int exact_match_score(const int8_t mat[25]) {
  const int a = mat[0];
  if (a <= 0) return 0;
  for (int r = 0; r < 5; ++r)
    for (int c = 0; c < 5; ++c) {
      const bool diag = r == c && r < 4;
      if (diag ? mat[r * 5 + c] != a : mat[r * 5 + c] >= a) return 0;
    }
  return a;
}

int sift_uniform_dm(const int8_t mat[25], int exact_a) {
  if (exact_a <= 0) return 0;
  const int mm = mat[1];
  for (int i = 0; i < 4; ++i)
    for (int j = 0; j < 4; ++j)
      if (i != j && mat[5 * i + j] != mm) return 0;
  return exact_a - mm > 0 ? exact_a - mm : 0;
}

int sift_uniform_dn(const int8_t mat[25], int exact_a) {
  if (exact_a <= 0) return 0;
  const int sn = mat[4];
  for (int i = 0; i < 5; ++i)
    if (mat[5 * i + 4] != sn || mat[20 + i] != sn) return 0;
  return exact_a - sn > 0 ? exact_a - sn : 0;
}

void apply_shortcuts(int mask, const int8_t mat[25], int* exact_a, int* certify, int* tail_bound) {
  *exact_a = (mask & 1) ? exact_match_score(mat) : 0;
  int lvl = *exact_a > 0 ? certify_level(mat) : 0;
  const int allowed = !(mask & 2) ? 0 : (!(mask & 4) ? 1 : (!(mask & 8) ? 2 : 3));
  *certify = lvl < allowed ? lvl : allowed;
  *tail_bound = (mask & 16) ? 1 : 0;
}

static void default_mat(int8_t mat[25], int a, int b) {
  int k = 0;
  for (int i = 0; i < 4; ++i) {
    for (int j = 0; j < 4; ++j) mat[k++] = (int8_t)(i == j ? a : -b);
    mat[k++] = -1;
  }
  for (int j = 0; j < 5; ++j) mat[k++] = -1;
}

static std::vector<int> allowed_devices() {
  int n = 0;
  if (hipGetDeviceCount(&n) != hipSuccess || n <= 0) return {};
  std::vector<int> all;
  const char* env = getenv("BPSW_DEVICES");
  if (env && *env) {
    const char* p = env;
    while (*p) {
      char* q = nullptr;
      long v = strtol(p, &q, 10);
      if (q == p) break;
      if (v >= 0 && v < n) all.push_back((int)v);
      p = (*q == ',') ? q + 1 : q;
      if (*q != ',' && *q != 0) break;
    }
  }
  if (all.empty())
    for (int i = 0; i < n; ++i) all.push_back(i);
  return all;
}

bool spin_wait() {
  static const bool on = getenv("BPSW_SPIN_WAIT") && atoi(getenv("BPSW_SPIN_WAIT")) != 0;
  return on;
}

int zerocopy_mask() {
  static const int m = getenv("BPSW_ZEROCOPY") ? atoi(getenv("BPSW_ZEROCOPY")) : 7;
  return m;
}

double wait_est_update(double est, double took_ms, int polls, bool napped) {
  (void)polls; (void)napped;
  if (est <= 0.) return took_ms;
  return 0.75 * est + 0.25 * std::min(took_ms, 3.0 * est + 0.2);
}
bool wait_naps(double est_ms) { return est_ms > 0.15 && est_ms * 700.0 - 60.0 > 20.0; }

void wait_nap(double est_ms) {
  if (est_ms > 0.15) {
    const double nap_us = est_ms * 700.0 - 60.0;
    if (nap_us > 20.0) { timespec ts = {0, (long)(nap_us * 1000.0)}; nanosleep(&ts, nullptr); }
  }
}
void wait_poll_pause(int polls, double waited_ms, double est_ms) {
  if (polls < 64 && waited_ms < est_ms * 1.3 + 0.05) sched_yield();
  else { timespec ts = {0, 20000}; nanosleep(&ts, nullptr); }
}

hipError_t wait_event(bpsw_ctx* c, hipEvent_t ev, int kind) {
  if (spin_wait()) return hipEventSynchronize(ev);
  double& est = c->wait_est_ms[kind & 3];
  const double t0 = wall_ms();
  const bool napped = wait_naps(est);
  wait_nap(est);
  hipError_t e;
  int polls = 0;
  while ((e = hipEventQuery(ev)) == hipErrorNotReady) wait_poll_pause(++polls, wall_ms() - t0, est);
  est = wait_est_update(est, wall_ms() - t0, polls, napped);
  return e;
}

double stat_ms() {
  static const bool cpu = getenv("BPSW_STATS_CLOCK") && getenv("BPSW_STATS_CLOCK")[0] == 'c';
  if (!cpu) return wall_ms();
  timespec ts;
  clock_gettime(CLOCK_THREAD_CPUTIME_ID, &ts);
  return 1e3 * (double)ts.tv_sec + 1e-6 * (double)ts.tv_nsec;
}

double wall_ms() {
  timespec ts;
  clock_gettime(CLOCK_MONOTONIC, &ts);
  return 1e3 * (double)ts.tv_sec + 1e-6 * (double)ts.tv_nsec;
}

namespace {
struct StreamPool {
  ExtGroupQueue q;
  std::vector<hipStream_t> streams;
  std::vector<int> pending;
};
StreamPool& stream_pool(int device) {
  static StreamPool table[64];
  return table[device >= 0 && device < 64 ? device : 0];
}
int stream_pool_cap() {
  static const int cap = [] {
    const char* e = getenv("BPSW_STREAM_POOL");
    int v = e ? atoi(e) : 20;
    v = v < 0 ? 0 : (v > 64 ? 64 : v);
    const char* q = getenv("GPU_MAX_HW_QUEUES");
    const int queues = q && atoi(q) > 0 ? atoi(q) : 4;
    const char* force = getenv("BPSW_STREAM_POOL_FORCE");
    if (v > queues && !(force && atoi(force) != 0)) {
      fprintf(stderr, "bPSW: stream pool clamped from %d (%s) to %d: %s, so only that many calls run on the GPU at a time; start the "
                      "executor with GPU_MAX_HW_QUEUES=20 (two executors per GPU: 10 each), or set BPSW_STREAM_POOL_FORCE=1 to keep %d\n",
              v, e ? "BPSW_STREAM_POOL" : "the default", queues,
              q ? "GPU_MAX_HW_QUEUES gives this process fewer hardware queues" : "GPU_MAX_HW_QUEUES is not set and the HIP runtime's default is 4 hardware queues", v);
      v = queues;
    }
    return v;
  }();
  return cap;
}
int stream_share() {
  static const int n = [] {
    const char* e = getenv("BPSW_STREAM_SHARE");
    const int v = e ? atoi(e) : 1;
    return v < 1 ? 1 : (v > 8 ? 8 : v);
  }();
  return n;
}
}

static std::atomic<long long> g_ext_last_us[64];
void ext_call_mark(int device) { g_ext_last_us[device >= 0 && device < 64 ? device : 0].store((long long)(wall_ms() * 1e3), std::memory_order_relaxed); }
double ext_call_age_ms(int device) {
  const long long t = g_ext_last_us[device >= 0 && device < 64 ? device : 0].load(std::memory_order_relaxed);
  return t == 0 ? 1e12 : wall_ms() - (double)t * 1e-3;
}

CopyLane& copy_lane(int device) {
  static CopyLane table[64];
  return table[device >= 0 && device < 64 ? device : 0];
}

int ext_group_max() {
  static const int n = [] {
    const char* e = getenv("BPSW_EXT_GROUP_MAX");
    const int v = e ? atoi(e) : EXT_GROUP_SLOTS;
    return v < 1 ? 1 : (v > EXT_GROUP_SLOTS ? EXT_GROUP_SLOTS : v);
  }();
  return n;
}
int ext_group_waiting(int device) { return stream_pool(device).q.waiting_compatible(); }
void ext_group_counts(int device, unsigned long long out[3]) { stream_pool(device).q.counts(out); }
void ext_group_complete(int device, ExtGroupWaiter** members, int n_members, int status, float span_ms) {
  stream_pool(device).q.complete(members, n_members, status, span_ms);
}

static int pool_take(StreamPool& P, int cap) {
  if (P.streams.capacity() < 64) { P.streams.reserve(64); P.pending.reserve(64); }
  int best = -1;
  for (size_t k = 0; k < P.streams.size(); ++k)
    if (best < 0 || P.pending[k] < P.pending[(size_t)best]) best = (int)k;
  if (best >= 0 && P.pending[(size_t)best] == 0) { ++P.pending[(size_t)best]; return best; }
  if ((int)P.streams.size() < cap) {
    hipStream_t ns = nullptr;
    if (hipStreamCreateWithFlags(&ns, hipStreamNonBlocking) == hipSuccess) {
      P.streams.push_back(ns);
      P.pending.push_back(1);
      return (int)P.streams.size() - 1;
    }
    if (best < 0) return ExtGroupQueue::OWN_SLOT;
  }
  if (best >= 0 && P.pending[(size_t)best] < stream_share()) { ++P.pending[(size_t)best]; return best; }
  return ExtGroupQueue::NO_SLOT;
}

StreamLease::StreamLease(bpsw_ctx* c, ExtGroupWaiter* w, ExtGroupWaiter** members, int* n_members)
    : device(c->device), s(c->stream), pooled(false), wait_ms(0.) {
  int none = 0;
  if (n_members) *n_members = 0;
  const int cap = stream_pool_cap();
  if (cap == 0) return;
  StreamPool& P = stream_pool(device);
  const double t0 = wall_ms();
  ExtGroupWaiter alone;
  if (!w) w = &alone;
  ExtGroupWaiter* no_members[1];
  const bool leads = P.q.acquire(*w, members ? ext_group_max() : 1, [&] { return pool_take(P, cap); }, members ? members : no_members, n_members ? n_members : &none);
  wait_ms = wall_ms() - t0;
  if (!leads) { led = true; return; }
  if (w->slot < 0) return;
  slot = w->slot;
  s = P.streams[(size_t)slot];
  pooled = true;
}
StreamLease::~StreamLease() {
  if (!pooled) return;
  StreamPool& P = stream_pool(device);
  const int cap = stream_pool_cap();
  P.q.release([&] { --P.pending[(size_t)slot]; }, [&] { return pool_take(P, cap); });
}

}

using namespace bpsw;

extern "C" {

const char* bpsw_last_error(void) { return g_err.c_str(); }
double bpsw_diag_wait_est_update(double est, double took_ms, int polls, int napped) { return bpsw::wait_est_update(est, took_ms, polls, napped != 0); }
int bpsw_diag_wait_naps(double est_ms) { return bpsw::wait_naps(est_ms) ? 1 : 0; }

const char* bpsw_version(void) {
  return "bPSW-hip 0.6 (gfx950)";
}

int bpsw_device_count(void) {
  int n = 0;
  if (hipGetDeviceCount(&n) != hipSuccess) return 0;
  return n;
}

int bpsw_device_slots(void) { return (int)allowed_devices().size(); }
int bpsw_device_for_partition(int partition) {
  if (partition < 0) return -1;
  const std::vector<int> devs = allowed_devices();
  return devs.empty() ? -1 : devs[(size_t)partition % devs.size()];
}

void bpsw_opt_default(bpsw_opt_t* o) {
  memset(o, 0, sizeof *o);
  o->a = 1; o->b = 4; o->o_del = 6; o->e_del = 1; o->o_ins = 6; o->e_ins = 1;
  o->pen_unpaired = 17; o->pen_clip5 = 5; o->pen_clip3 = 5; o->w = 100; o->zdrop = 100;
  o->T = 30; o->flag = 0; o->min_seed_len = 19; o->max_ins = 10000; o->max_matesw = 100;
  o->mask_level_redun = 0.95f;
  default_mat(o->mat, o->a, o->b);
}

int bpsw_create(int device, bpsw_ctx_t** out) {
  if (!out) return fail(BPSW_ERR_ARG, "bpsw_create: null out");
  *out = nullptr;
  std::vector<int> devs = allowed_devices();
  if (devs.empty()) return fail(BPSW_ERR_DEVICE, "bpsw_create: no HIP device visible (there is no CPU fallback)");
  if (device < 0) {
    static std::atomic<unsigned> rr{0};
    device = devs[rr.fetch_add(1) % devs.size()];
  } else {
    int n = bpsw_device_count();
    if (device >= n) return fail(BPSW_ERR_ARG, "bpsw_create: device index out of range");
  }
  HIP_TRY(hipSetDevice(device));
  if (!spin_wait()) {
    (void)hipSetDeviceFlags(hipDeviceScheduleBlockingSync);
    (void)hipGetLastError();
  }
  hipDeviceProp_t prop;
  HIP_TRY(hipGetDeviceProperties(&prop, device));
  if (strncmp(prop.gcnArchName, "gfx950", 6) != 0)
    return fail(BPSW_ERR_DEVICE, std::string("bpsw_create: kernels are built for gfx950, device is ") + prop.gcnArchName);
  bpsw_ctx* c = new bpsw_ctx();
  c->device = device;
  c->num_cu = prop.multiProcessorCount > 0 ? prop.multiProcessorCount : 256;
  memset(&c->stats, 0, sizeof c->stats);
  default_mat(c->ext_mat, 1, 4);
  c->ext_sc.mat = pack_mat(c->ext_mat);
  c->ext_sc.zdrop = 100;
  c->ext_sc.zdrop_mode = BPSW_ZDROP_SCALA;
  c->ext_sc.mat_max = 1;
  c->ext_sc.side_how = nullptr;
  c->ext_sc.out_stride = 10;
  c->ext_sc.pac = nullptr; c->ext_sc.l_pac = 0;
  apply_shortcuts(c->shortcut_mask, c->ext_mat, &c->ext_sc.exact_a, &c->ext_sc.certify, &c->ext_sc.tail_bound);
  hipError_t e = hipStreamCreateWithFlags(&c->stream, hipStreamNonBlocking);
  for (int i = 0; e == hipSuccess && i < 8; ++i) e = hipEventCreateWithFlags(&c->ev[i], spin_wait() ? hipEventDefault : hipEventBlockingSync);
  if (e == hipSuccess) e = c->d_pre.reserve(512);
  if (e == hipSuccess) e = hipMemsetAsync(c->d_pre.ptr, 0, 512, c->stream);
  if (e == hipSuccess) e = hipStreamSynchronize(c->stream);
  if (e == hipSuccess) e = c->h_pre.reserve(512);
  if (e == hipSuccess) memset(c->h_pre.ptr, 0, 512);
  if (e != hipSuccess) {
    bpsw_destroy(c);
    return hip_fail(e, "bpsw_create");
  }
  *out = c;
  return BPSW_OK;
}

void bpsw_destroy(bpsw_ctx_t* c) {
  if (!c) return;
  (void)hipSetDevice(c->device);
  if (c->pend_ext.active && c->pend_ext.s) (void)hipStreamSynchronize(c->pend_ext.s);
  if (c->pend_sw.active && c->pend_sw.s) (void)hipStreamSynchronize(c->pend_sw.s);
  if (c->stream) (void)hipStreamSynchronize(c->stream);
  if (c->ring_abandoned) {
    for (int i = 0; i < 8; ++i)
      if (c->ev[i]) (void)hipEventDestroy(c->ev[i]);
    if (c->stream) (void)hipStreamDestroy(c->stream);
    rescue_scratch_free(c->rescue_scratch);
    c->ev[0] = nullptr;
    return;
  }
  RingPauseForFree paused_for_all;
  c->d_wire.release(); c->d_out.release(); c->d_pre.release();
  c->d_sw_in.release(); c->d_sw_out.release(); c->d_sw_scratch.release(); c->d_gl_z.release(); c->d_ext_lists.release(); c->d_sift.release();
  for (bpsw::DeviceBuffer& b : c->d_seed) b.release();
  c->d_chain.release();
  c->d_chain_tab.release();
  c->h_stage_in.release(); c->h_stage_out.release(); c->h_pre.release();
  rescue_scratch_free(c->rescue_scratch);
  for (int i = 0; i < 8; ++i)
    if (c->ev[i]) (void)hipEventDestroy(c->ev[i]);
  if (c->stream) (void)hipStreamDestroy(c->stream);
  delete c;
}

int bpsw_device_of(const bpsw_ctx_t* c) { return c ? c->device : -1; }
int bpsw_device_cus(const bpsw_ctx_t* c) { return c ? c->num_cu : -1; }

int bpsw_set_ext_shortcuts(bpsw_ctx_t* c, int mask) {
  if (!c) return fail(BPSW_ERR_ARG, "null context");
  std::lock_guard<std::mutex> g(c->mu);
  c->shortcut_mask = mask < 0 ? 63 : (mask & 63);
  apply_shortcuts(c->shortcut_mask, c->ext_mat, &c->ext_sc.exact_a, &c->ext_sc.certify, &c->ext_sc.tail_bound);
  return BPSW_OK;
}

int bpsw_set_ext_scoring(bpsw_ctx_t* c, const int8_t mat[25], int zdrop, int zdrop_mode) {
  if (!c) return fail(BPSW_ERR_ARG, "null context");
  if (zdrop_mode != BPSW_ZDROP_SCALA && zdrop_mode != BPSW_ZDROP_BWA) return fail(BPSW_ERR_ARG, "bad zdrop_mode");
  std::lock_guard<std::mutex> g(c->mu);
  if (mat) memcpy(c->ext_mat, mat, 25);
  c->ext_sc.mat = pack_mat(c->ext_mat);
  c->ext_sc.mat_max = c->ext_mat[0];
  for (int k = 1; k < 25; ++k) c->ext_sc.mat_max = c->ext_mat[k] > c->ext_sc.mat_max ? c->ext_mat[k] : c->ext_sc.mat_max;
  c->ext_sc.zdrop = zdrop;
  c->ext_sc.zdrop_mode = zdrop_mode;
  apply_shortcuts(c->shortcut_mask, c->ext_mat, &c->ext_sc.exact_a, &c->ext_sc.certify, &c->ext_sc.tail_bound);
  return BPSW_OK;
}



static inline int rd16(const uint8_t* b, size_t at) { return (int16_t)(b[at] | (b[at + 1] << 8)); }
static inline int rd32(const uint8_t* b, size_t at) {
  return (int32_t)((uint32_t)b[at] | ((uint32_t)b[at + 1] << 8) | ((uint32_t)b[at + 2] << 16) | ((uint32_t)b[at + 3] << 24));
}

static int scan_wire(const uint8_t* wire, size_t bytes, long long l_pac, int* n_out, int* maxq, int* maxr, bool* coord,
                     std::vector<int>* long_tasks, int* maxr_short, int* n_mid_out) {
  if (!wire || bytes < 32 || (bytes & 3)) return fail(BPSW_ERR_ARG, "extend: wire batch shorter than its header or not word sized");
  const int n = rd32(wire, 8);
  const int fmt = wire[7];
  if (fmt != 0 && fmt != BPSW_WIRE_COORDS) return fail(BPSW_ERR_ARG, "extend: unknown wire format (header byte 7)");
  const bool co = fmt == BPSW_WIRE_COORDS;
  const size_t rec_bytes = co ? 40 : 32;
  if (n < 0 || 32 + rec_bytes * (size_t)n > bytes) return fail(BPSW_ERR_ARG, "extend: task table exceeds the buffer");
  if ((int8_t)wire[0] < 0 || (int8_t)wire[1] < 1 || (int8_t)wire[2] < 0 || (int8_t)wire[3] < 1)
    return fail(BPSW_ERR_ARG, "extend: gap opens must be >= 0 and gap extensions >= 1 (a zero extension divides by zero in SWUtil.scala:110-115)");
  if ((int8_t)wire[6] < 0) return fail(BPSW_ERR_ARG, "extend: negative band width (w travels as a signed byte: at most 127)");
  if (co && l_pac <= 0) return fail(BPSW_ERR_ARG, "extend: a coordinate batch needs the reference on the device (bpsw_ref_load)");
  const int wband = (int8_t)wire[6];
  int mq = 0, mr = 0, mrs = 0;
  const size_t words = bytes >> 2;
  const bool all_long = (int8_t)wire[2] + (int8_t)wire[3] <= 0;
  long_tasks->clear();
  int mid = 0;
  for (int t = 0; t < n; ++t) {
    const size_t at = 32 + rec_bytes * (size_t)t;
    const int lq = rd16(wire, at), lr = rd16(wire, at + 2), rq = rd16(wire, at + 4), rr = rd16(wire, at + 6);
    if (lq < 0 || lr < 0 || rq < 0 || rr < 0) return fail(BPSW_ERR_ARG, "extend: negative sequence length in task table");
    const long long pos = rd32(wire, at + 8);
    const long long w = co ? ((long long)lq + rq + 7) / 8 : ((long long)lq + lr + rq + rr + 7) / 8;
    if (pos < 8 + (long long)(rec_bytes / 4) * n || (unsigned long long)(pos + w) > words)
      return fail(BPSW_ERR_ARG, "extend: task sequence offset outside the buffer");
    if (lq > mq) mq = lq;
    if (rq > mq) mq = rq;
    const bool is_long = all_long || lq > 255 || rq > 255;
    const bool is_mid = !is_long && (lq > 127 || rq > 127);
    if (is_mid) ++mid;
    if (is_long) long_tasks->push_back(t);
    int task_mr = 0;
    if (co) {
      const int len = rd16(wire, at + 18);
      long long rb;
      memcpy(&rb, wire + at + 32, 8);
      if (rb < 0 || rb > (l_pac << 1)) return fail(BPSW_ERR_ARG, "extend: task window outside the reference or bridging its two strands");
      const long long lo = rb - lr, hi = rb + len + rr;
      if (len < 0 || lo < 0 || hi > (l_pac << 1) || (lo < l_pac && hi > l_pac))
        return fail(BPSW_ERR_ARG, "extend: task window outside the reference or bridging its two strands");
      const int sl = std::min(lr, lq + 2 * wband + 2), sr = std::min(rr, rq + 2 * wband + 2);
      task_mr = std::max(sl, sr);
    } else {
      task_mr = std::max(lr, rr);
    }
    if (task_mr > mr) mr = task_mr;
    if (!is_long && task_mr > mrs) mrs = task_mr;
  }
  if (mq > BPSW_EXT_MAX_QLEN || mr > BPSW_EXT_MAX_RLEN) return fail(BPSW_ERR_LIMIT, "extend: sequence longer than the kernel limit");
  *n_out = n; *maxq = mq; *maxr = mr; *coord = co; *maxr_short = mrs; *n_mid_out = mid;
  return BPSW_OK;
}

static int extend_batch_impl(bpsw_ctx_t* c, const uint8_t* wire, size_t wire_bytes, int16_t* out, size_t out_len, uint8_t* side_how,
                             const int16_t** out_view = nullptr);

int bpsw_extend_batch(bpsw_ctx_t* c, const uint8_t* wire, size_t wire_bytes, int16_t* out, size_t out_len) {
  return extend_batch_impl(c, wire, wire_bytes, out, out_len, nullptr);
}

int bpsw_extend_stage(bpsw_ctx_t* c, size_t bytes, uint8_t** buf) {
  if (!c || !buf) return fail(BPSW_ERR_ARG, "extend_stage: null argument");
  ContextEntry entry(c);
  if (entry.rc != BPSW_OK) return entry.rc;
  HIP_TRY(c->h_stage_in.reserve(bytes + bytes / 8 + 4096));
  c->staged_bytes = bytes;
  *buf = (uint8_t*)c->h_stage_in.ptr;
  return BPSW_OK;
}

int bpsw_extend_commit(bpsw_ctx_t* c, size_t wire_bytes, const int16_t** out, size_t* out_len) {
  if (!c || !out) return fail(BPSW_ERR_ARG, "extend_commit: null argument");
  const uint8_t* staged = nullptr;
  {
    std::lock_guard<std::mutex> g(c->mu);
    if (!c->h_stage_in.ptr || c->staged_bytes == 0) return fail(BPSW_ERR_ARG, "extend_commit: nothing staged (call bpsw_extend_stage first)");
    if (wire_bytes > c->staged_bytes || wire_bytes > c->h_stage_in.cap)
      return fail(BPSW_ERR_ARG, "extend_commit: more bytes than bpsw_extend_stage was asked for");
    staged = (const uint8_t*)c->h_stage_in.ptr;
    c->staged_bytes = 0;
  }
  const int rc = extend_batch_impl(c, staged, wire_bytes, nullptr, 0, nullptr, out);
  if (rc == BPSW_OK && out_len) *out_len = *out ? 10 * (size_t)rd32((const uint8_t*)c->h_stage_in.ptr, 8) : 0;
  return rc;
}

int bpsw_extend_batch_classify(bpsw_ctx_t* c, const uint8_t* wire, size_t wire_bytes, int16_t* out, size_t out_len, uint8_t* side_how) {
  if (!side_how) return fail(BPSW_ERR_ARG, "extend_classify: null side_how");
  return extend_batch_impl(c, wire, wire_bytes, out, out_len, side_how);
}

struct ExtCallItem {
  ExtGroupMember gm;
  void* copy_dst = nullptr;
  const void* copy_src = nullptr;
  size_t copy_bytes = 0;
  double enqueued_at = 0.;
};

static int extend_batch_impl(bpsw_ctx_t* c, const uint8_t* wire, size_t wire_bytes, int16_t* out, size_t out_len, uint8_t* side_how,
                             const int16_t** out_view) {
  if (!c) return fail(BPSW_ERR_ARG, "null context");
  int n = 0, mq = 0, mr = 0;
  bool coord = false;
  ContextEntry entry(c);
  if (entry.rc != BPSW_OK) return entry.rc;
  const uint8_t* d_pac = nullptr;
  long long l_pac = 0;
  RefHold ref_hold;
  if (wire && wire_bytes >= 32 && wire[7] == BPSW_WIRE_COORDS) ref_hold = ref_snapshot(c, &d_pac, &l_pac);
  std::vector<int>& long_tasks = c->ext_long_tasks;
  int mr_short = 0;
  int n_mid = 0;
  int rc = scan_wire(wire, wire_bytes, l_pac, &n, &mq, &mr, &coord, &long_tasks, &mr_short, &n_mid);
  if (rc != BPSW_OK) return rc;
  const int n_long = (int)long_tasks.size();
  const bool use_short = 2 * (size_t)n_long <= (size_t)n;
  const bool expect_full = !use_short || n_long > 0;
  const size_t list_off = (wire_bytes + 15) & ~(size_t)15;
  const size_t stage_bytes = use_short ? list_off + 4 * (1 + (size_t)n_long) : wire_bytes;
  const size_t dev_bytes = use_short ? list_off + 4 * (1 + (size_t)n) : wire_bytes;
  if (!out_view && (!out || out_len < 10 * (size_t)n)) return fail(BPSW_ERR_CAPACITY, "extend: result buffer smaller than 10*n int16");
  if (out_view) *out_view = nullptr;
  if (n == 0) return BPSW_OK;
  const size_t out_bytes = 20 * (size_t)n;
  static const bool lazy_on = !(getenv("BPSW_EXT_LAZY_FULL") && atoi(getenv("BPSW_EXT_LAZY_FULL")) == 0);
  const bool lazy_full = lazy_on && !side_how && use_short && n_long == 0;
  const bool use_full = expect_full || (use_short && !lazy_full);
  const size_t out_post_bytes = out_bytes + (lazy_full ? 4 : 0);
  HIP_TRY(c->d_wire.reserve(dev_bytes));
  HIP_TRY(c->d_out.reserve(out_post_bytes));
  static const int sift_min = getenv("BPSW_EXT_SIFT_MIN") ? atoi(getenv("BPSW_EXT_SIFT_MIN")) : 8192;
  const int sift_dm = sift_uniform_dm(c->ext_mat, c->ext_sc.exact_a);
  const bool use_sift = n >= sift_min && (c->shortcut_mask & 32) && use_short && 16 * (size_t)n_mid <= (size_t)n && sift_dm > 0;
  const size_t sift_rec_off = ((size_t)n + 15) & ~(size_t)15;
  static const int heavy_min = getenv("BPSW_EXT_HEAVY_MIN") ? atoi(getenv("BPSW_EXT_HEAVY_MIN")) : 96;
  const size_t todo_off = sift_rec_off + 32 * (size_t)n;
  if (use_sift) HIP_TRY(c->d_sift.reserve(todo_off + 4 * (size_t)n));
  const bool staged = wire == (const uint8_t*)c->h_stage_in.ptr;
  if (staged && stage_bytes > c->h_stage_in.cap) return fail(BPSW_ERR_ARG, "extend_commit: the staged batch is larger than what bpsw_extend_stage was asked for");
  HIP_TRY(c->h_stage_in.reserve(stage_bytes));
  HIP_TRY(c->h_stage_out.reserve(out_post_bytes));
  if (lazy_full) *(volatile int*)((char*)c->h_stage_out.ptr + out_bytes) = 0;
  const double t_in = stat_ms();
  ext_call_mark(c->device);
  struct ExtMark { int d; ~ExtMark() { ext_call_mark(d); } } ext_mark{c->device};
  if (!staged) memcpy(c->h_stage_in.ptr, wire, wire_bytes);
  if (use_short) {
    int* hl = (int*)((char*)c->h_stage_in.ptr + list_off);
    hl[0] = n_long;
    if (n_long) memcpy(hl + 1, long_tasks.data(), 4 * (size_t)n_long);
  }
  const double t_staged = stat_ms();
  double t_dev0, t_dev1, copy_first_ms = 0.;
  bool kernel_was_last = false, relaunched = false;
  bool grouped = false;
  int group_n = 1;
  float group_span_ms = 0.f;
  bool via_ring = false;
  float ring_kernel_ms = 0.f;
  {
    static const bool ext_ring_on = !(getenv("BPSW_EXT_RING") && atoi(getenv("BPSW_EXT_RING")) == 0);
    static const int ext_ring_max = getenv("BPSW_EXT_RING_MAX_TASKS") ? atoi(getenv("BPSW_EXT_RING_MAX_TASKS")) : 256;
    const bool eligible = ring_enabled() && ext_ring_on && use_short && n_long == 0 && !use_sift && !side_how &&
                          (zerocopy_mask() & 1) != 0 && mq <= 255 && mr_short <= EXT_RING_RCAP && n <= ext_ring_max;
    if (eligible && ring_usable(c->device, RING_CLASS_EXT)) {
      t_dev0 = stat_ms();
      static const size_t ring_zc_bytes = getenv("BPSW_EXT_RING_ZC_BYTES") ? (size_t)atoll(getenv("BPSW_EXT_RING_ZC_BYTES")) : 65536;
      const void* ring_wire = c->h_stage_in.ptr;
      if (wire_bytes > ring_zc_bytes) {
        HIP_TRY(hipMemcpyAsync(c->d_wire.ptr, c->h_stage_in.ptr, wire_bytes, hipMemcpyHostToDevice, c->stream));
        HIP_TRY(hipEventRecord(c->ev[0], c->stream));
        HIP_TRY(wait_event(c, c->ev[0], 2));
        ring_wire = c->d_wire.ptr;
        copy_first_ms = stat_ms() - t_dev0;
      }
      const int per_unit = n <= 2048 ? 1 : 4;
      ExtRingPayload pl;
      memset(&pl, 0, sizeof pl);
      pl.wire = (uint64_t)(uintptr_t)ring_wire; pl.out = (uint64_t)(uintptr_t)c->h_stage_out.ptr;
      pl.n_tasks = n; pl.per_unit = per_unit; pl.out_stride = c->ext_sc.out_stride;
      pl.zdrop = c->ext_sc.zdrop; pl.zdrop_mode = c->ext_sc.zdrop_mode; pl.mat_max = c->ext_sc.mat_max; pl.exact_a = c->ext_sc.exact_a;
      pl.tail_bound = c->ext_sc.tail_bound; pl.certify = c->ext_sc.certify;
      pl.coord = coord ? 1 : 0; pl.pac = (uint64_t)(uintptr_t)(coord ? d_pac : nullptr); pl.l_pac = coord ? l_pac : 0;
      for (int r = 0; r < 5; ++r) pl.mat_row[r] = c->ext_sc.mat.row[r];
      const RingRun run = ring_run(c->device, RING_CLASS_EXT, c->num_cu, &pl, sizeof pl, (uint32_t)((n + per_unit - 1) / per_unit),
                                   (RingDone*)((char*)c->h_pre.ptr + 448), &c->ring_seq, &c->wait_est_ms[4],
                                   RingRecords{(uint32_t*)c->h_stage_out.ptr, 5, (size_t)n, 4, "extension"});
      if (run.how == RingRun::failed) {
        if (run.submitted) c->ring_abandoned = true;
        return run.rc;
      }
      if (run.how == RingRun::unwritten) {
        static std::atomic<bool> said{false};
        if (!said.exchange(true)) fprintf(stderr, "bPSW: an extension batch came back from the ring with unwritten records; it is run again through a launch (%s)\n", bpsw_last_error());
      }
      if (run.how == RingRun::done) {
        ring_kernel_ms = run.span_ms;
        t_dev1 = stat_ms();
        via_ring = true;
        c->stats.ext_ring_calls++;
      } else {
        copy_first_ms = 0.;
      }
    }
  }
  if (!via_ring) {
    const bool copy_first = sw_launches_in_flight(c->device) > 0;
    if (copy_first) {
      const double t_c0 = stat_ms();
      CopyLane& L = copy_lane(c->device);
      {
        std::lock_guard<std::mutex> lk(L.mu);
        if (!L.s) HIP_TRY(hipStreamCreateWithFlags(&L.s, hipStreamNonBlocking));
        HIP_TRY(hipMemcpyAsync(c->d_wire.ptr, c->h_stage_in.ptr, stage_bytes, hipMemcpyHostToDevice, L.s));
        HIP_TRY(hipStreamSynchronize(L.s));
      }
      copy_first_ms = stat_ms() - t_c0;
    }
    const bool zc_out = (zerocopy_mask() & 1) != 0;
    int16_t* k_out = zc_out ? (int16_t*)c->h_stage_out.ptr : (int16_t*)c->d_out.ptr;
    int* const d_queue_words = (int*)((char*)c->d_pre.ptr + 128);
    ExtCallItem me;
    memset(&me.gm, 0, sizeof me.gm);
    const bool groupable = &launch_ext_group != nullptr && ext_group_max() > 1 && !coord && use_sift && lazy_full && zc_out && !side_how;
    if (groupable) {
      ExtMember& m = me.gm.m;
      m.wire = (const uint32_t*)c->d_wire.ptr; m.n_tasks = n; m.out = k_out; m.sc = c->ext_sc; m.queue = d_queue_words;
      m.defer = (int*)((char*)c->d_wire.ptr + list_off); m.defer_post = (int*)(k_out + 10 * (size_t)n); m.short_qmax = 255;
      m.sift_flag = (uint8_t*)c->d_sift.ptr; m.sift_recs = (uint4*)((char*)c->d_sift.ptr + sift_rec_off);
      m.todo_count = d_queue_words + 2; m.todo_list = (int*)((char*)c->d_sift.ptr + todo_off);
      m.sift_dm = sift_dm; m.sift_dn = sift_uniform_dn(c->ext_mat, c->ext_sc.exact_a); m.sift_qmax = 127; m.heavy_min = heavy_min;
      me.gm.qcap = std::min(mq, 255); me.gm.rcap = mr_short;
      if (!copy_first) { me.copy_dst = c->d_wire.ptr; me.copy_src = c->h_stage_in.ptr; me.copy_bytes = stage_bytes; }
    }
    ExtGroupWaiter gw;
    gw.compatible = groupable;
    gw.item = &me;
    ExtGroupWaiter* led[EXT_GROUP_SLOTS];
    int n_led = 0;
    const double t_ready = stat_ms();
    StreamLease lease(c, &gw, groupable ? led : nullptr, groupable ? &n_led : nullptr);
    hipStream_t s = lease.s;
    t_dev0 = stat_ms();
    const auto late_full = [&](hipStream_t ls) -> int {
      KernelEvents kev;
      kev.start = c->ev[4]; kev.stop = c->ev[5];
      relaunched = true;
      ExtScoring sc_full = c->ext_sc;
      if (coord) { sc_full.pac = d_pac; sc_full.l_pac = l_pac; }
      const int listed = *(volatile int*)((char*)c->h_stage_out.ptr + out_bytes);
      HIP_TRY(launch_ext_kernel((const uint32_t*)c->d_wire.ptr, listed, k_out, sc_full, mq, mr, c->num_cu, d_queue_words, nullptr, ls,
                                nullptr, false, kev, false, (int*)((char*)c->d_wire.ptr + list_off)));
      if (!zc_out) HIP_TRY(hipMemcpyAsync(c->h_stage_out.ptr, c->d_out.ptr, out_bytes, hipMemcpyDeviceToHost, ls));
      if (!zc_out || side_how) HIP_TRY(hipEventRecord(c->ev[3], ls));
      HIP_TRY(wait_event(c, (!zc_out || side_how) ? c->ev[3] : c->ev[5], 0));
      c->stats.ext_full_relaunches++;
      return BPSW_OK;
    };
    if (lease.led || n_led > 0) {
      grouped = true;
      kernel_was_last = true;
      if (lease.led) {
        group_n = gw.group_n; group_span_ms = gw.span_ms;
        const double now = stat_ms();
        const double since_enq = std::max(0., wall_ms() - me.enqueued_at);
        t_dev0 = std::max(t_ready, now - since_enq);
        c->stats.ext_wait_ms += t_dev0 - t_ready;
        if (gw.status != (int)hipSuccess) {
          (void)hipMemsetAsync(d_queue_words, 0, 4 * sizeof(int), c->stream);
          (void)hipStreamSynchronize(c->stream);
          return hip_fail((hipError_t)gw.status, "extend: the launch chain this call shared with others");
        }
      } else {
        const int k = 1 + n_led;
        group_n = k;
        struct GroupDone {
          int dev; ExtGroupWaiter** m; int n; int status; float span; int* q; hipStream_t s; bool clear;
          ~GroupDone() {
            if (clear) { (void)hipMemsetAsync(q, 0, 4 * sizeof(int), s); (void)hipStreamSynchronize(s); }
            if (n) ext_group_complete(dev, m, n, status, span);
          }
        } done{c->device, led, n_led, (int)hipErrorUnknown, 0.f, d_queue_words, s, true};
        ExtGroupMember gms[EXT_GROUP_SLOTS];
        gms[0] = me.gm;
        HIP_TRY(hipEventRecord(c->ev[0], s));
        if (me.copy_bytes) HIP_TRY(hipMemcpyAsync(me.copy_dst, me.copy_src, me.copy_bytes, hipMemcpyHostToDevice, s));
        for (int i = 0; i < n_led; ++i) {
          ExtCallItem* it = (ExtCallItem*)led[i]->item;
          gms[1 + i] = it->gm;
          if (it->copy_bytes) HIP_TRY(hipMemcpyAsync(it->copy_dst, it->copy_src, it->copy_bytes, hipMemcpyHostToDevice, s));
        }
        KernelEvents kev;
        kev.start = c->ev[1]; kev.stop = c->ev[2];
        hipError_t ge = launch_ext_group(gms, k, c->num_cu, s, kev);
        const double enq = wall_ms();
        for (int i = 0; i < n_led; ++i) ((ExtCallItem*)led[i]->item)->enqueued_at = enq;
        if (ge == hipSuccess) ge = wait_event(c, c->ev[2], 3);
        done.status = (int)ge;
        if (ge != hipSuccess) return hip_fail(ge, "extend: launch chain of a group");
        done.clear = false;
        float span = 0.f;
        (void)hipEventElapsedTime(&span, c->ev[1], c->ev[2]);
        group_span_ms = done.span = span;
        c->stats.ext_wait_ms += lease.wait_ms;
      }
    }
    if (grouped) {
      if (*(volatile int*)((char*)c->h_stage_out.ptr + out_bytes) > 0) {
        if (lease.led) {
          StreamLease late(c);
          const int lrc = late_full(late.s);
          if (lrc != BPSW_OK) return lrc;
        } else {
          const int lrc = late_full(s);
          if (lrc != BPSW_OK) return lrc;
        }
      }
      t_dev1 = stat_ms();
    } else {
      HIP_TRY(hipEventRecord(c->ev[0], s));
      if (!copy_first) HIP_TRY(hipMemcpyAsync(c->d_wire.ptr, c->h_stage_in.ptr, stage_bytes, hipMemcpyHostToDevice, s));
      bool on_dispatch = false;
      {
        ExtScoring sc = c->ext_sc;
        if (coord) { sc.pac = d_pac; sc.l_pac = l_pac; }
        if (side_how) {
          HIP_TRY(c->d_ext_lists.reserve(2 * (size_t)n + 16));
          HIP_TRY(hipMemsetAsync(c->d_ext_lists.ptr, 0, 2 * (size_t)n, s));
          sc.side_how = (uint8_t*)c->d_ext_lists.ptr;
        }
        on_dispatch = true;
        int* d_queue = (int*)((char*)c->d_pre.ptr + 128);
        int* d_list = use_short ? (int*)((char*)c->d_wire.ptr + list_off) : nullptr;
        if (use_short) {
          KernelEvents kev;
          kev.start = c->ev[1]; kev.stop = (use_full && !lazy_full) ? nullptr : c->ev[2];
          uint8_t* d_sflag = use_sift ? (uint8_t*)c->d_sift.ptr : nullptr;
          uint4* d_srecs = use_sift ? (uint4*)((char*)c->d_sift.ptr + sift_rec_off) : nullptr;
          int* d_todo = use_sift ? (int*)((char*)c->d_sift.ptr + todo_off) : nullptr;
          struct TodoGuard {
            int* q; hipStream_t s; bool armed;
            ~TodoGuard() { if (armed) { (void)hipMemsetAsync(q, 0, 4 * sizeof(int), s); (void)hipStreamSynchronize(s); } }
          } todo_guard{d_queue, s, false};
          if (use_sift) {
            KernelEvents sev;
            sev.start = kev.start; kev.start = nullptr;
            todo_guard.armed = true;
            HIP_TRY(launch_ext_sift_kernel((const uint32_t*)c->d_wire.ptr, n, k_out, sc, sift_dm | (sift_uniform_dn(c->ext_mat, c->ext_sc.exact_a) << 16), 127, d_sflag, d_srecs, s, sev, nullptr,
                                           d_queue + 2, d_todo, heavy_min));
          }
          HIP_TRY(launch_ext_kernel((const uint32_t*)c->d_wire.ptr, n, k_out, sc, std::min(mq, 255), mr_short, c->num_cu, d_queue, nullptr, s,
                                    nullptr, false, kev, true, d_list, 255, d_sflag, d_srecs, lazy_full ? (int*)(k_out + 10 * (size_t)n) : nullptr, d_todo));
          todo_guard.armed = false;
        }
        if (use_full && !lazy_full) {
          KernelEvents kev;
          kev.start = use_short ? nullptr : c->ev[1]; kev.stop = c->ev[2];
          const int grid_tasks = !use_short ? n : n_long + 4;
          HIP_TRY(launch_ext_kernel((const uint32_t*)c->d_wire.ptr, grid_tasks, k_out, sc, mq, mr, c->num_cu, d_queue, nullptr, s,
                                    nullptr, false, kev, false, use_short ? d_list : nullptr));
        }
        if (side_how) HIP_TRY(hipMemcpyAsync(side_how, c->d_ext_lists.ptr, 2 * (size_t)n, hipMemcpyDeviceToHost, s));
      }
      if (!on_dispatch) HIP_TRY(hipEventRecord(c->ev[2], s));
      const bool kernel_is_last = on_dispatch && zc_out && !side_how;
      kernel_was_last = kernel_is_last;
      if (!zc_out) HIP_TRY(hipMemcpyAsync(c->h_stage_out.ptr, c->d_out.ptr, out_post_bytes, hipMemcpyDeviceToHost, s));
      if (!kernel_is_last) HIP_TRY(hipEventRecord(c->ev[3], s));
      HIP_TRY(wait_event(c, kernel_is_last ? c->ev[2] : c->ev[3], 0));
      if (lazy_full && *(volatile int*)((char*)c->h_stage_out.ptr + out_bytes) > 0) {
        const int lrc = late_full(s);
        if (lrc != BPSW_OK) return lrc;
      }
      t_dev1 = stat_ms();
      c->stats.ext_wait_ms += lease.wait_ms;
    }
  }
  if (out_view) {
    *out_view = (const int16_t*)c->h_stage_out.ptr;
  } else {
    memcpy(out, c->h_stage_out.ptr, out_bytes);
  }
  const double t_out = stat_ms();
  float a = 0, b = 0, d = 0;
  if (via_ring) {
    b = ring_kernel_ms;
    t_dev0 += copy_first_ms;
  } else {
    if (!grouped) {
      (void)hipEventElapsedTime(&a, c->ev[0], c->ev[1]);
      (void)hipEventElapsedTime(&b, c->ev[1], c->ev[2]);
    } else {
      b = group_span_ms / (float)group_n;
    }
    if (relaunched) { float b2 = 0; (void)hipEventElapsedTime(&b2, c->ev[4], c->ev[5]); b += b2; }
    if (!kernel_was_last) (void)hipEventElapsedTime(&d, relaunched ? c->ev[5] : c->ev[2], c->ev[3]);
  }
  c->stats.ext_calls++; c->stats.ext_tasks += (uint64_t)n; c->stats.ext_wire_bytes += wire_bytes;
  c->stats.ext_h2d_ms += a + copy_first_ms; c->stats.ext_kernel_ms += b; c->stats.ext_d2h_ms += d;
  c->stats.ext_host_in_ms += t_staged - t_in; c->stats.ext_dev_ms += t_dev1 - t_dev0 + copy_first_ms; c->stats.ext_host_out_ms += t_out - t_dev1;
  c->last_ext_ms = b;
  c->have_ext_ev = false;
  return BPSW_OK;
}

static const int ASYNC_QCAP = 256, ASYNC_RCAP = 4096;

static int ext_device_sync_launch(bpsw_ctx_t* c, const void* d_wire, int n_tasks, void* d_out, hipStream_t s, const ExtPrepass* h_pre) {
  HIP_TRY(hipEventRecord(c->ev[4], s));
  HIP_TRY(launch_ext_kernel((const uint32_t*)d_wire, n_tasks, (int16_t*)d_out, c->ext_sc, h_pre->max_qlen, h_pre->max_rlen, c->num_cu,
                            (int*)((char*)c->d_pre.ptr + 128), nullptr, s));
  HIP_TRY(hipEventRecord(c->ev[5], s));
  c->have_ext_ev = true;
  return BPSW_OK;
}

extern "C++" {
namespace bpsw {
int finish_pending_ext(bpsw_ctx_t* c) {
  if (!c->pend_ext.active) return BPSW_OK;
  bpsw_ctx::PendingExt p = c->pend_ext;
  c->pend_ext.active = false;
  HIP_TRY(hipStreamSynchronize(p.s));
  const ExtPrepass* h_pre = (const ExtPrepass*)c->h_pre.ptr;
  if (h_pre->error) { c->have_ext_ev = false; return fail(BPSW_ERR_ARG, "extend_device: malformed wire batch (code " + std::to_string(h_pre->error) + ")"); }
  if (h_pre->max_qlen > BPSW_EXT_MAX_QLEN || h_pre->max_rlen > BPSW_EXT_MAX_RLEN) {
    c->have_ext_ev = false;
    return fail(BPSW_ERR_LIMIT, "extend_device: sequence longer than the kernel limit");
  }
  c->ext_geom_q = std::max(c->ext_geom_q, h_pre->max_qlen);
  c->ext_geom_r = std::max(c->ext_geom_r, h_pre->max_rlen);
  if (h_pre->max_qlen > p.qcap || h_pre->max_rlen > p.rcap) {
    int rc = ext_device_sync_launch(c, p.d_wire, p.n_tasks, p.d_out, p.s, h_pre);
    if (rc != BPSW_OK) return rc;
    HIP_TRY(hipStreamSynchronize(p.s));
  }
  return BPSW_OK;
}
}
}

int bpsw_extend_batch_device(bpsw_ctx_t* c, const void* d_wire, size_t wire_bytes, int n_tasks, void* d_out,
                             void* hip_stream) {
  if (!c) return fail(BPSW_ERR_ARG, "null context");
  if (!d_wire || !d_out || n_tasks < 0 || wire_bytes < 32 + 32 * (size_t)n_tasks || (wire_bytes & 3) ||
      ((uintptr_t)d_wire & 15) || ((uintptr_t)d_out & 3))
    return fail(BPSW_ERR_ARG, "extend_device: bad buffer arguments");
  if (n_tasks == 0) return BPSW_OK;
  ContextEntry entry(c);
  if (entry.rc != BPSW_OK) return entry.rc;
  hipStream_t s = hip_stream ? (hipStream_t)hip_stream : c->stream;
  HIP_TRY(c->d_ext_lists.reserve(4 * ((size_t)n_tasks + 1) + 16));
  ExtPrepass* d_pre = (ExtPrepass*)c->d_pre.ptr;
  ExtPrepass* h_pre = (ExtPrepass*)c->h_pre.ptr;
  static_assert(sizeof(ExtPrepass) <= 64, "scan buffer layout");
  HIP_TRY(hipMemsetAsync(d_pre, 0, 128 + 16, s));
  launch_ext_prepass((const uint32_t*)d_wire, wire_bytes >> 2, n_tasks, d_pre, s);
  HIP_TRY(hipGetLastError());
  c->stats.ext_calls++; c->stats.ext_tasks += (uint64_t)n_tasks; c->stats.ext_wire_bytes += wire_bytes;
  {
    int qcap = ASYNC_QCAP, rcap = ASYNC_RCAP;
    if (c->ext_geom_q > 0) {
      qcap = std::min(ASYNC_QCAP, (c->ext_geom_q + 32 + 31) & ~31);
      rcap = std::min(ASYNC_RCAP, (c->ext_geom_r + 128 + 63) & ~63);
    }
    HIP_TRY(hipEventRecord(c->ev[4], s));
    int* d_queue = (int*)((char*)c->d_pre.ptr + 128);
    int* d_list = (int*)c->d_ext_lists.ptr;
    HIP_TRY(hipMemsetAsync(d_list, 0, sizeof(int), s));
    static const int sift_min = getenv("BPSW_EXT_SIFT_MIN") ? atoi(getenv("BPSW_EXT_SIFT_MIN")) : 8192;
    const int sift_dm = sift_uniform_dm(c->ext_mat, c->ext_sc.exact_a);
    const bool use_sift = n_tasks >= sift_min && (c->shortcut_mask & 32) && sift_dm > 0 && c->ext_geom_q > 0 && c->ext_geom_q <= 140;
    const size_t sift_rec_off = ((size_t)n_tasks + 15) & ~(size_t)15;
    uint8_t* d_sflag = nullptr;
    uint4* d_srecs = nullptr;
    if (use_sift) {
      HIP_TRY(c->d_sift.reserve(sift_rec_off + 32 * (size_t)n_tasks));
      d_sflag = (uint8_t*)c->d_sift.ptr;
      d_srecs = (uint4*)((char*)c->d_sift.ptr + sift_rec_off);
      HIP_TRY(launch_ext_sift_kernel((const uint32_t*)d_wire, n_tasks, (int16_t*)d_out, c->ext_sc, sift_dm | (sift_uniform_dn(c->ext_mat, c->ext_sc.exact_a) << 16), 127, d_sflag, d_srecs, s, KernelEvents(), d_pre));
    }
    HIP_TRY(launch_ext_kernel((const uint32_t*)d_wire, n_tasks, (int16_t*)d_out, c->ext_sc, qcap, rcap, c->num_cu, d_queue, nullptr, s,
                              d_pre, true, KernelEvents(), true, d_list, -255, d_sflag, d_srecs));
    HIP_TRY(launch_ext_kernel((const uint32_t*)d_wire, n_tasks, (int16_t*)d_out, c->ext_sc, qcap, rcap, c->num_cu,
                              d_queue, nullptr, s, d_pre, true, KernelEvents(), false, d_list));
    c->pend_ext.qcap = qcap; c->pend_ext.rcap = rcap;
    HIP_TRY(hipEventRecord(c->ev[5], s));
    HIP_TRY(hipMemcpyAsync(h_pre, d_pre, 128, hipMemcpyDeviceToHost, s));
    c->have_ext_ev = true;
    c->pend_ext.active = true; c->pend_ext.d_wire = d_wire; c->pend_ext.wire_bytes = wire_bytes; c->pend_ext.n_tasks = n_tasks;
    c->pend_ext.d_out = d_out; c->pend_ext.s = s;
    return BPSW_OK;
  }
}

int bpsw_ext_group_waiting(int device) { return device >= 0 && device < 64 ? bpsw::ext_group_waiting(device) : -1; }
int bpsw_ext_group_counts(int device, uint64_t out[3]) {
  if (!out || device < 0 || device >= 64) return fail(BPSW_ERR_ARG, "ext_group_counts: bad argument");
  unsigned long long v[3];
  bpsw::ext_group_counts(device, v);
  for (int i = 0; i < 3; ++i) out[i] = (uint64_t)v[i];
  return BPSW_OK;
}

int bpsw_get_stats(bpsw_ctx_t* c, bpsw_stats_t* out) {
  if (!c || !out) return fail(BPSW_ERR_ARG, "null argument");
  std::lock_guard<std::mutex> g(c->mu);
  *out = c->stats;
  return BPSW_OK;
}
int bpsw_reset_stats(bpsw_ctx_t* c) {
  if (!c) return fail(BPSW_ERR_ARG, "null context");
  std::lock_guard<std::mutex> g(c->mu);
  memset(&c->stats, 0, sizeof c->stats);
  return BPSW_OK;
}

}
```

### include/bpsw.h

```cpp
#ifndef BPSW_H
#define BPSW_H

#include <stddef.h>
#include <stdint.h>

#ifdef __cplusplus
extern "C" {
#endif

#define BPSW_OK 0
#define BPSW_ERR_ARG (-1)
#define BPSW_ERR_DEVICE (-2)
#define BPSW_ERR_CAPACITY (-3)
#define BPSW_ERR_LIMIT (-4)

#define BPSW_ZDROP_SCALA 0
#define BPSW_ZDROP_BWA 1

#define BPSW_RESCUE_C 0
#define BPSW_RESCUE_SCALA 1

#define BPSW_KSW_XBYTE 0x10000
#define BPSW_KSW_XSTOP 0x20000
#define BPSW_KSW_XSUBO 0x40000
// ... 81 lines not shown
  int32_t xtra;
  const int32_t *q_len, *t_len;
  const int64_t *q_off, *t_off;
  const uint8_t *q_rev;
  const uint8_t *q_pool, *t_pool;
  size_t q_pool_bytes, t_pool_bytes;
} bpsw_sw_jobs_t;
int bpsw_swalign2_batch(bpsw_ctx_t *ctx, const bpsw_opt_t *opt, const bpsw_sw_jobs_t *jobs, int32_t *out);

int bpsw_swalign2_batch_device(bpsw_ctx_t *ctx, const bpsw_opt_t *opt, const bpsw_sw_jobs_t *jobs,
                               void *d_out, void *hip_stream);

typedef struct {
  int32_t group_size;
  int64_t l_pac;
  bpsw_pestat_t pes[4];
  const int32_t *seq_len;
  const int64_t *seq_off;
  const uint8_t *seq_pool;
  size_t seq_pool_bytes;
  const int32_t *reg_cnt;
  const bpsw_alnreg_t *regs;
  const int32_t *ref_cnt;
  const int64_t *ref_rb, *ref_re, *ref_len, *ref_off;
  const uint8_t *ref_pool;
  size_t ref_pool_bytes;
} bpsw_rescue_group_t;
int bpsw_matesw_group(bpsw_ctx_t *ctx, const bpsw_opt_t *opt, const bpsw_rescue_group_t *g, int mode,
                      int32_t *out_cnt, bpsw_alnreg_t *out_regs, int64_t out_cap, int64_t *out_total);

#define BPSW_GLOBAL_MAX_QLEN 1023
#define BPSW_GLOBAL_MAX_TLEN 65535
#define BPSW_GLOBAL_MAX_CIGAR 512
typedef struct {
  int32_t n;
  int32_t max_cigar;
  const int32_t *q_len, *t_len, *w;
  const int64_t *q_off, *t_off;
  const uint8_t *q_pool, *t_pool;
  size_t q_pool_bytes, t_pool_bytes;
} bpsw_global_jobs_t;
int bpsw_global_batch(bpsw_ctx_t *ctx, const bpsw_opt_t *opt, const bpsw_global_jobs_t *jobs, int32_t *out_score,
                      int32_t *out_ncigar, uint32_t *out_cigar);

int bpsw_ref_load(bpsw_ctx_t *ctx, const uint8_t *pac, int64_t l_pac);
int bpsw_ref_unload(bpsw_ctx_t *ctx);
int64_t bpsw_ref_length(const bpsw_ctx_t *ctx);
int bpsw_ref_fetch(bpsw_ctx_t *ctx, int32_t n, const int64_t *beg, const int64_t *end, uint8_t *out_pool,
                   size_t out_pool_bytes, const int64_t *out_off, int64_t *out_len);

#define BPSW_C2A_SORT_DEDUP 1
#define BPSW_C2A_DEDUP_SCALA 2
#define BPSW_W1_CHAIN_DEVICE 4
#define BPSW_W1_SEED_PLAN_DEVICE 8
#define BPSW_W1_CHAINS_RESIDENT 16
typedef struct {
  int32_t n_reads;
  const int32_t *read_len;
  const int64_t *read_off;
  const uint8_t *read_pool;
  size_t read_pool_bytes;
  const int32_t *chain_cnt;
  const int32_t *seed_cnt;
  const int64_t *seed_rbeg;
  const int32_t *seed_qbeg, *seed_len;
} bpsw_chains_t;
int bpsw_chain2aln_batch(bpsw_ctx_t *ctx, const bpsw_opt_t *opt, const bpsw_chains_t *batch, int zdrop_mode, int flags,
                         int32_t *out_cnt, bpsw_alnreg_t *out_regs, int64_t out_cap, int64_t *out_total);

int bpsw_fmi_load(bpsw_ctx_t *ctx, int64_t primary, const int64_t L2[5], int64_t seq_len, const uint32_t *bwt, int64_t bwt_size,
                  int32_t sa_intv, int64_t n_sa, const int64_t *sa);
int bpsw_fmi_unload(bpsw_ctx_t *ctx);
int64_t bpsw_fmi_length(const bpsw_ctx_t *ctx);

#define BPSW_MEM_F_NO_EXACT 0x40
#define BPSW_SEED_MAX_QLEN 256
typedef struct {
  int32_t min_seed_len, max_occ, split_width, max_chain_gap, no_exact;
  float split_factor, chain_drop_ratio, mask_level;
} bpsw_seed_opt_t;
void bpsw_seed_opt_default(bpsw_seed_opt_t *s);

typedef struct {
  int32_t n_reads;
  const int32_t *read_len;
  const int64_t *read_off;
  const uint8_t *read_pool;
  size_t read_pool_bytes;
} bpsw_reads_t;
typedef struct {
  int64_t x0, x1, x2;
  int32_t qbeg, qend;
  int32_t kept;
  int32_t pad_;
} bpsw_smem_t;
typedef struct {
  int64_t rbeg;
  int32_t qbeg, len;
} bpsw_seed_t;

int bpsw_seed_batch(bpsw_ctx_t *ctx, const bpsw_seed_opt_t *sopt, const bpsw_reads_t *reads, int32_t *intv_cnt, bpsw_smem_t *intv,
                    int64_t intv_cap, int64_t *intv_total, int32_t *seed_cnt, bpsw_seed_t *seeds, int64_t seed_cap,
                    int64_t *seed_total);

#define BPSW_SEED_PLAN_DEVICE 1
int bpsw_seed_batch_ex(bpsw_ctx_t *ctx, const bpsw_seed_opt_t *sopt, const bpsw_reads_t *reads, int32_t *intv_cnt, bpsw_smem_t *intv,
                       int64_t intv_cap, int64_t *intv_total, int32_t *seed_cnt, bpsw_seed_t *seeds, int64_t seed_cap,
                       int64_t *seed_total, int flags);
void bpsw_last_seed_bytes(int64_t b[2]);
void bpsw_scan_set_tile(int items);

int bpsw_chain_seeds(const bpsw_seed_opt_t *sopt, int32_t w, int64_t l_pac, int32_t n_seeds, const bpsw_seed_t *seeds, int32_t filter,
                     int32_t *chain_seed_cnt, int32_t chain_cap, bpsw_seed_t *out_seeds);

int bpsw_chain_batch(bpsw_ctx_t *ctx, const bpsw_seed_opt_t *sopt, int32_t w, int64_t l_pac, int32_t n_reads, const int32_t *seed_cnt,
                     const bpsw_seed_t *seeds, int32_t filter, int32_t *chain_cnt, int32_t *chain_seed_cnt, int64_t chain_cap,
                     bpsw_seed_t *out_seeds, int64_t seed_cap, int64_t *chain_total, int64_t *seed_total);
void bpsw_chain_set_arena_budget(int64_t bytes);
void bpsw_chain_last_split(int64_t st[4]);

#define BPSW_CHAIN_TABLES_DEVICE 1
int bpsw_chain_batch_ex(bpsw_ctx_t *ctx, const bpsw_seed_opt_t *sopt, int32_t w, int64_t l_pac, int32_t n_reads, const int32_t *seed_cnt,
                        const bpsw_seed_t *seeds, int32_t filter, int32_t *chain_cnt, int32_t *chain_seed_cnt, int64_t chain_cap,
                        bpsw_seed_t *out_seeds, int64_t seed_cap, int64_t *chain_total, int64_t *seed_total, int flags);
void bpsw_last_chain_bytes(int64_t b[2]);

int bpsw_worker1_batch(bpsw_ctx_t *ctx, const bpsw_opt_t *opt, const bpsw_seed_opt_t *sopt, const bpsw_reads_t *reads, int zdrop_mode,
                       int flags, int32_t *out_cnt, bpsw_alnreg_t *out_regs, int64_t out_cap, int64_t *out_total);
void bpsw_seed_set_resident_lanes(int lanes);
void bpsw_last_worker1_times(double ms[3]);

#define BPSW_TAIL_SCALA 0
#define BPSW_TAIL_C 1
#define BPSW_MEM_F_NOPAIRING 0x4
#define BPSW_MEM_F_ALL 0x8
#define BPSW_MEM_F_NO_MULTI 0x10
#define BPSW_R2A_MAX_QLEN 1024
#define BPSW_R2A_MAX_RLEN 4096

typedef struct {
  float mask_level, mapq_coef_len;
  int32_t mapq_coef_fac;
  int32_t flavour;
  char rg_id[64];
} bpsw_tail_opt_t;
void bpsw_tail_opt_default(bpsw_tail_opt_t *t);

int bpsw_bns_load(bpsw_ctx_t *ctx, int32_t n_seqs, const int64_t *offset, const int32_t *len, const char *names);

#define BPSW_ALN_OK 0
#define BPSW_ALN_XREF 1
#define BPSW_ALN_NOCIGAR 2
#define BPSW_ALN_OVERFLOW 3
typedef struct {
  int64_t pos;
  int32_t rid, flag, is_rev, mapq, NM, n_cigar, score, sub, md_len, status;
} bpsw_aln_t;

typedef struct {
  int32_t n;
  int32_t max_cigar, max_md;
  const int32_t *read_len;
  const int64_t *read_off;
  const uint8_t *read_pool;
  size_t read_pool_bytes;
  const bpsw_alnreg_t *regs;
} bpsw_reg2aln_jobs_t;
int bpsw_reg2aln_batch(bpsw_ctx_t *ctx, const bpsw_opt_t *opt, const bpsw_tail_opt_t *topt, const bpsw_reg2aln_jobs_t *jobs,
                       bpsw_aln_t *out, uint32_t *out_cigar, uint8_t *out_md);

typedef struct {
  int32_t group_size;
  int64_t id0;
  bpsw_pestat_t pes[4];
  const int32_t *read_len;
  const int64_t *read_off;
  const uint8_t *read_pool;
  const uint8_t *qual_pool;
  size_t read_pool_bytes;
  const int64_t *name_off;
  const char *name_pool;
  const int32_t *reg_cnt;
  const bpsw_alnreg_t *regs;
} bpsw_pairs_t;
int bpsw_sam_pe_batch(bpsw_ctx_t *ctx, const bpsw_opt_t *opt, const bpsw_tail_opt_t *topt, const bpsw_pairs_t *g, char *out_text,
                      size_t text_cap, int64_t *out_off, size_t *out_needed, bpsw_alnreg_t *out_regs);
int bpsw_mark_primary_se(const bpsw_opt_t *opt, const bpsw_tail_opt_t *topt, int32_t n, bpsw_alnreg_t *regs, int64_t id);
int bpsw_approx_mapq_se(const bpsw_opt_t *opt, const bpsw_tail_opt_t *topt, const bpsw_alnreg_t *reg);
int bpsw_mem_pair(const bpsw_opt_t *opt, const bpsw_tail_opt_t *topt, int64_t l_pac, const bpsw_pestat_t pes[4], int32_t n0,
                  const bpsw_alnreg_t *regs0, int32_t n1, const bpsw_alnreg_t *regs1, int64_t id, int32_t out5[5]);
int bpsw_sort_dedup(int32_t n, bpsw_alnreg_t *regs, float mask_level_redun, int mode);
int bpsw_pe_stat(const bpsw_opt_t *opt, const bpsw_tail_opt_t *topt, int64_t l_pac, int32_t n_pairs, const int32_t *reg_cnt,
                 const bpsw_alnreg_t *regs, bpsw_pestat_t pes[4]);

int bpsw_worker2_batch(bpsw_ctx_t *ctx, const bpsw_opt_t *opt, const bpsw_tail_opt_t *topt, const bpsw_pairs_t *g, int rescue_mode,
                       char *out_text, size_t text_cap, int64_t *out_off, size_t *out_needed, int32_t *out_reg_cnt,
                       bpsw_alnreg_t *out_regs, int64_t out_regs_cap, int64_t *out_regs_total);
typedef struct bpsw_tail_pool bpsw_tail_pool_t;
#define BPSW_TAIL_POOL_TAIL_ONLY (-1)
int bpsw_tail_pool_create(int device, int n_workers, bpsw_tail_pool_t **out);
void bpsw_tail_pool_destroy(bpsw_tail_pool_t *pool);
int bpsw_tail_pool_submit(bpsw_tail_pool_t *pool, const bpsw_opt_t *opt, const bpsw_tail_opt_t *topt, const bpsw_pairs_t *g,
                          int rescue_mode, char *out_text, size_t text_cap, int64_t *out_off, int32_t *out_reg_cnt,
                          bpsw_alnreg_t *out_regs, int64_t out_regs_cap, int64_t *ticket);
int bpsw_tail_pool_wait(bpsw_tail_pool_t *pool, int64_t ticket, size_t *out_needed, int64_t *out_regs_total);
int bpsw_tail_pool_workers(const bpsw_tail_pool_t *pool);
int bpsw_last_tail_times(bpsw_ctx_t *ctx, float *kernel_ms, int32_t *n_jobs, double host_ms[3]);
int bpsw_last_tail_resubmitted(bpsw_ctx_t *ctx, int32_t *n_resubmitted);

#define BPSW_SAM_TEXT_DEVICE 1
typedef struct {
  int32_t n_reads;
  int64_t id0;
  int32_t id_step;
  const int32_t *read_len;
  const int64_t *read_off;
  const uint8_t *read_pool;
  const uint8_t *qual_pool;
  size_t read_pool_bytes;
  const int64_t *name_off;
  const char *name_pool;
  const int32_t *reg_cnt;
  const bpsw_alnreg_t *regs;
} bpsw_se_reads_t;
int bpsw_sam_se_batch(bpsw_ctx_t *ctx, const bpsw_opt_t *opt, const bpsw_tail_opt_t *topt, const bpsw_se_reads_t *reads, int flags,
                      char *out_text, size_t text_cap, int64_t *out_off, size_t *out_needed, bpsw_alnreg_t *out_regs);
int bpsw_align_se_batch(bpsw_ctx_t *ctx, const bpsw_opt_t *opt, const bpsw_seed_opt_t *sopt, const bpsw_tail_opt_t *topt,
                        const bpsw_se_reads_t *reads, int zdrop_mode, int w1_flags, int flags, char *out_text, size_t text_cap,
                        int64_t *out_off, size_t *out_needed);
void bpsw_last_sam_se_times(double ms[6]);

int bpsw_sam_pe_batch_ex(bpsw_ctx_t *ctx, const bpsw_opt_t *opt, const bpsw_tail_opt_t *topt, const bpsw_pairs_t *g, int flags,
                         char *out_text, size_t text_cap, int64_t *out_off, size_t *out_needed, bpsw_alnreg_t *out_regs);
int bpsw_align_pe_batch(bpsw_ctx_t *ctx, const bpsw_opt_t *opt, const bpsw_seed_opt_t *sopt, const bpsw_tail_opt_t *topt,
                        const bpsw_pairs_t *g, const bpsw_pestat_t *pes0, int zdrop_mode, int w1_flags, int rescue_mode, int flags,
                        char *out_text, size_t text_cap, int64_t *out_off, size_t *out_needed, bpsw_pestat_t *out_pes);
void bpsw_last_sam_pe_times(double ms[8]);

#define BPSW_FASTQ_FINAL 1
#define BPSW_FASTQ_INTERLEAVED 2
#define BPSW_FASTQ_PAIR_NAMES 4
#define BPSW_FASTQ_HOST 8
int bpsw_fastq_parse(bpsw_ctx_t *ctx, const char *text1, size_t bytes1, const char *text2, size_t bytes2, int flags, int64_t max_reads,
                     size_t pool_cap, size_t name_cap, int32_t *read_len, int64_t *read_off, uint8_t *read_pool, uint8_t *qual_pool,
                     int64_t *name_off, char *name_pool, int64_t *n_reads, int64_t consumed[2], int64_t needed[3]);
int bpsw_align_fastq_se(bpsw_ctx_t *ctx, const bpsw_opt_t *opt, const bpsw_seed_opt_t *sopt, const bpsw_tail_opt_t *topt,
                        const char *text, size_t bytes, int fastq_flags, int64_t id0, int32_t id_step, int zdrop_mode, int w1_flags,
                        int flags, char *out_text, size_t text_cap, int64_t *out_off, int64_t max_reads, size_t *out_needed,
                        int64_t *n_reads, int64_t *consumed);
int bpsw_align_fastq_pe(bpsw_ctx_t *ctx, const bpsw_opt_t *opt, const bpsw_seed_opt_t *sopt, const bpsw_tail_opt_t *topt,
                        const char *text1, size_t bytes1, const char *text2, size_t bytes2, int fastq_flags, int64_t id0,
                        const bpsw_pestat_t *pes0, int zdrop_mode, int w1_flags, int rescue_mode, int flags, char *out_text,
                        size_t text_cap, int64_t *out_off, int64_t max_reads, size_t *out_needed, bpsw_pestat_t *out_pes,
                        int64_t *n_reads, int64_t consumed[2]);
void bpsw_last_fastq_times(double ms[5]);

#define BPSW_BAM_DEFLATE 16
int bpsw_bam_se_batch(bpsw_ctx_t *ctx, const bpsw_opt_t *opt, const bpsw_tail_opt_t *topt, const bpsw_se_reads_t *reads, int flags, char *out,
                      size_t cap, size_t *out_needed, bpsw_alnreg_t *out_regs);
int bpsw_bam_pe_batch(bpsw_ctx_t *ctx, const bpsw_opt_t *opt, const bpsw_tail_opt_t *topt, const bpsw_pairs_t *g, int flags, char *out,
                      size_t cap, size_t *out_needed, bpsw_alnreg_t *out_regs);
int bpsw_align_bam_se_batch(bpsw_ctx_t *ctx, const bpsw_opt_t *opt, const bpsw_seed_opt_t *sopt, const bpsw_tail_opt_t *topt,
                            const bpsw_se_reads_t *reads, int zdrop_mode, int w1_flags, int flags, char *out, size_t cap,
                            size_t *out_needed);
int bpsw_align_bam_pe_batch(bpsw_ctx_t *ctx, const bpsw_opt_t *opt, const bpsw_seed_opt_t *sopt, const bpsw_tail_opt_t *topt,
                            const bpsw_pairs_t *g, const bpsw_pestat_t *pes0, int zdrop_mode, int w1_flags, int rescue_mode, int flags,
                            char *out, size_t cap, size_t *out_needed, bpsw_pestat_t *out_pes);
int bpsw_align_fastq_bam_se(bpsw_ctx_t *ctx, const bpsw_opt_t *opt, const bpsw_seed_opt_t *sopt, const bpsw_tail_opt_t *topt,
                            const char *text, size_t bytes, int fastq_flags, int64_t id0, int32_t id_step, int zdrop_mode, int w1_flags,
                            int flags, char *out, size_t cap, size_t *out_needed, int64_t *n_reads, int64_t *consumed);
int bpsw_align_fastq_bam_pe(bpsw_ctx_t *ctx, const bpsw_opt_t *opt, const bpsw_seed_opt_t *sopt, const bpsw_tail_opt_t *topt,
                            const char *text1, size_t bytes1, const char *text2, size_t bytes2, int fastq_flags, int64_t id0,
                            const bpsw_pestat_t *pes0, int zdrop_mode, int w1_flags, int rescue_mode, int flags, char *out, size_t cap,
                            size_t *out_needed, bpsw_pestat_t *out_pes, int64_t *n_reads, int64_t consumed[2]);
int bpsw_sam_header(bpsw_ctx_t *ctx, int32_t n_seqs, const int32_t *len, const char *names, const char *extra, size_t extra_bytes, char *out,
                    size_t cap, size_t *out_needed);
int bpsw_bam_header(bpsw_ctx_t *ctx, int32_t n_seqs, const int32_t *len, const char *names, const char *extra, size_t extra_bytes, char *out,
                    size_t cap, size_t *out_needed);
int bpsw_bam_eof(char *out, size_t cap, size_t *out_needed);
int bpsw_bam_set_block_payload(int bytes);
void bpsw_last_bam_times(double ms[5]);
void bpsw_last_bam_deflate_times(double ms[4]);

typedef struct {
  uint64_t ext_calls, ext_tasks, ext_wire_bytes;
  uint64_t sw_calls, sw_jobs, sw_speculated, sw_replayed_rounds, sw_wasted;
  double ext_h2d_ms, ext_kernel_ms, ext_d2h_ms;
  double sw_h2d_ms, sw_kernel_ms, sw_d2h_ms, sw_host_ms;
  double ext_host_in_ms, ext_wait_ms, ext_dev_ms, ext_host_out_ms;
  double grp_plan_ms, grp_pack_ms, grp_wait_ms, grp_dev_ms, grp_replay_ms, grp_out_ms;
  uint64_t grp_calls, grp_pairs;
  uint64_t ext_full_relaunches;
  uint64_t sw_ring_calls;
  uint64_t ext_ring_calls;
} bpsw_stats_t;
int bpsw_get_stats(bpsw_ctx_t *ctx, bpsw_stats_t *out);
int bpsw_reset_stats(bpsw_ctx_t *ctx);
int bpsw_last_kernel_ms(bpsw_ctx_t *ctx, float *ext_ms, float *sw_ms);
int bpsw_ring_stats(bpsw_ctx_t *ctx, uint64_t *epochs, uint64_t *submitted, uint64_t *carried, double *epochs_ms, uint64_t *epochs_timed);
int bpsw_ring_integrity(uint64_t *checked, uint64_t *faults);
int bpsw_sw_batches_in_flight(int device);
int bpsw_ext_group_waiting(int device);
int bpsw_ext_group_counts(int device, uint64_t out[3]);

#ifdef __cplusplus
}
#endif
#endif
```

Baseline: 279.7 million.

## Batch host-to-device wire copies on a shared copy lane and queue for streams

```diff
diff --git a/cloud-scale-bwamem_amd/bpsw_hip/__init__.py b/cloud-scale-bwamem_amd/bpsw_hip/__init__.py
--- a/cloud-scale-bwamem_amd/bpsw_hip/__init__.py
+++ b/cloud-scale-bwamem_amd/bpsw_hip/__init__.py
@@ -21,7 +21,7 @@
     "bpsw_set_ext_scoring", "bpsw_set_ext_shortcuts", "bpsw_extend_batch", "bpsw_extend_stage", "bpsw_extend_commit", "bpsw_extend_batch_classify", "bpsw_extend_batch_device", "bpsw_wire_size", "bpsw_wire_pack", "bpsw_wire_coords_size", "bpsw_wire_coords_pack",
     "bpsw_opt_default", "bpsw_swalign2_batch", "bpsw_swalign2_batch_device", "bpsw_matesw_group", "bpsw_global_batch",
     "bpsw_get_stats", "bpsw_reset_stats", "bpsw_last_kernel_ms", "bpsw_ring_stats", "bpsw_sw_batches_in_flight", "bpsw_ring_integrity",
-    "bpsw_ext_group_waiting", "bpsw_ext_group_counts",
+    "bpsw_ext_group_waiting", "bpsw_ext_group_counts", "bpsw_ext_lane_waiting", "bpsw_ext_lane_counts",
     "bpsw_ref_load", "bpsw_ref_unload", "bpsw_ref_length", "bpsw_ref_fetch", "bpsw_chain2aln_batch",
     "bpsw_tail_opt_default", "bpsw_bns_load", "bpsw_reg2aln_batch", "bpsw_sam_pe_batch", "bpsw_worker2_batch", "bpsw_last_tail_times", "bpsw_last_tail_resubmitted",
     "bpsw_tail_pool_create", "bpsw_tail_pool_destroy", "bpsw_tail_pool_submit", "bpsw_tail_pool_wait", "bpsw_tail_pool_workers",
@@ -187,6 +187,8 @@
     lib.bpsw_sw_batches_in_flight.argtypes = [C.c_int]
     lib.bpsw_ext_group_waiting.argtypes = [C.c_int]
     lib.bpsw_ext_group_counts.argtypes = [C.c_int, C.POINTER(C.c_uint64)]
+    lib.bpsw_ext_lane_waiting.argtypes = [C.c_int]
+    lib.bpsw_ext_lane_counts.argtypes = [C.c_int, C.POINTER(C.c_uint64)]
     lib.bpsw_ring_integrity.argtypes = [C.POINTER(C.c_uint64), C.POINTER(C.c_uint64)]
     lib.bpsw_chain2aln_batch.argtypes = [C.c_void_p, C.POINTER(Opt), C.POINTER(Chains), C.c_int, C.c_int, C.c_void_p, C.c_void_p,
                                          C.c_int64, C.POINTER(C.c_int64)]
@@ -678,6 +680,14 @@
         _chk(self.lib, self.lib.bpsw_ext_group_counts(self.lib.bpsw_device_of(self.h), out), "bpsw_ext_group_counts")
         return int(out[0]), int(out[1]), int(out[2])
 
+    def ext_lane_waiting(self):
+        return int(self.lib.bpsw_ext_lane_waiting(self.lib.bpsw_device_of(self.h)))
+
+    def ext_lane_counts(self):
+        out = (C.c_uint64 * 3)()
+        _chk(self.lib, self.lib.bpsw_ext_lane_counts(self.lib.bpsw_device_of(self.h), out), "bpsw_ext_lane_counts")
+        return int(out[0]), int(out[1]), int(out[2])
+
     def ring_epoch_times(self):
         ms, n = C.c_double(0.0), C.c_uint64(0)
         _chk(self.lib, self.lib.bpsw_ring_stats(self.h, None, None, None, C.byref(ms), C.byref(n)), "bpsw_ring_stats")
diff --git a/cloud-scale-bwamem_amd/csrc/bpsw_ext_group.h b/cloud-scale-bwamem_amd/csrc/bpsw_ext_group.h
--- a/cloud-scale-bwamem_amd/csrc/bpsw_ext_group.h
+++ b/cloud-scale-bwamem_amd/csrc/bpsw_ext_group.h
@@ -7,7 +7,7 @@
 namespace bpsw {
 
 struct ExtGroupWaiter {
-  enum State { WAITING, LEADER, TAKEN, DONE };
+  enum State { WAITING, LEADER, TAKEN, DONE, LANE_WAITING, LANE_LEADER, LANE_TAKEN };
   std::condition_variable cv;
   State state = WAITING;
   bool compatible = false;
@@ -16,6 +16,7 @@
   int status = 0;
   float span_ms = 0.f;
   int group_n = 1;
+  bool lane_failed = false;
 };
 
 class ExtGroupQueue {
@@ -38,6 +39,134 @@
     }
     w.state = ExtGroupWaiter::WAITING;
     waiters_.push_back(&w);
+    return await_locked(lk, w, max_group, members, n_members);
+  }
+
+  bool await(ExtGroupWaiter& w, int max_group, ExtGroupWaiter** members, int* n_members) {
+    *n_members = 0;
+    std::unique_lock<std::mutex> lk(mu_);
+    return await_locked(lk, w, max_group, members, n_members);
+  }
+
+  template <class Take>
+  void enqueue_for(ExtGroupWaiter& m, Take&& take) {
+    std::lock_guard<std::mutex> lk(mu_);
+    enqueue_locked(&m, take);
+  }
+
+  bool lane_enter(ExtGroupWaiter& w, int max_group, int depth, ExtGroupWaiter** members, int* n_members) {
+    *n_members = 0;
+    std::unique_lock<std::mutex> lk(mu_);
+    w.state = ExtGroupWaiter::LANE_WAITING;
+    w.lane_failed = false;
+    lane_.push_back(&w);
+    lane_promote(depth);
+    w.cv.wait(lk, [&] { return w.state == ExtGroupWaiter::LANE_LEADER || w.state == ExtGroupWaiter::LEADER || w.state == ExtGroupWaiter::DONE; });
+    if (w.state != ExtGroupWaiter::LANE_LEADER) return false;
+    if (w.compatible) {
+      if (max_group > MAX_GROUP) max_group = MAX_GROUP;
+      for (auto it = lane_.begin(); it != lane_.end() && *n_members + 1 < max_group;) {
+        if ((*it)->compatible) {
+          (*it)->state = ExtGroupWaiter::LANE_TAKEN;
+          members[(*n_members)++] = *it;
+          it = lane_.erase(it);
+        } else {
+          ++it;
+        }
+      }
+    }
+    ++lane_groups_;
+    lane_members_ += 1ull + (unsigned long long)*n_members;
+    if (1ull + (unsigned long long)*n_members > lane_largest_) lane_largest_ = 1ull + (unsigned long long)*n_members;
+    return true;
+  }
+
+  void lane_enqueued(int depth) {
+    std::lock_guard<std::mutex> lk(mu_);
+    lane_enqueueing_ = false;
+    lane_promote(depth);
+  }
+
+  template <class Take>
+  void lane_finish(ExtGroupWaiter& w, ExtGroupWaiter** members, int n_members, int status, int depth, Take&& take) {
+    std::lock_guard<std::mutex> lk(mu_);
+    --lane_active_;
+    if (status == 0) {
+      enqueue_locked(&w, take);
+      for (int i = 0; i < n_members; ++i) enqueue_locked(members[i], take);
+    } else {
+      w.state = ExtGroupWaiter::DONE;
+      w.status = status;
+      w.lane_failed = true;
+      for (int i = 0; i < n_members; ++i) {
+        ExtGroupWaiter* m = members[i];
+        m->status = status;
+        m->lane_failed = true;
+        m->group_n = 1;
+        m->span_ms = 0.f;
+        m->state = ExtGroupWaiter::DONE;
+        m->cv.notify_one();
+      }
+    }
+    lane_promote(depth);
+  }
+
+  void complete(ExtGroupWaiter** members, int n_members, int status, float span_ms) {
+    std::lock_guard<std::mutex> lk(mu_);
+    for (int i = 0; i < n_members; ++i) {
+      ExtGroupWaiter* m = members[i];
+      m->status = status;
+      m->span_ms = span_ms;
+      m->group_n = 1 + n_members;
+      m->state = ExtGroupWaiter::DONE;
+      m->cv.notify_one();
+    }
+  }
+
+  template <class Put, class Take>
+  void release(Put&& put, Take&& take) {
+    std::lock_guard<std::mutex> lk(mu_);
+    put();
+    while (!waiters_.empty()) {
+      const int s = take();
+      if (s < 0) break;
+      ExtGroupWaiter* w = waiters_.front();
+      waiters_.pop_front();
+      w->slot = s;
+      w->state = ExtGroupWaiter::LEADER;
+      w->cv.notify_one();
+    }
+  }
+
+  int waiting() {
+    std::lock_guard<std::mutex> lk(mu_);
+    return (int)waiters_.size();
+  }
+  int waiting_compatible() {
+    std::lock_guard<std::mutex> lk(mu_);
+    int n = 0;
+    for (const ExtGroupWaiter* w : waiters_) n += w->compatible ? 1 : 0;
+    return n;
+  }
+  void counts(unsigned long long out[3]) {
+    std::lock_guard<std::mutex> lk(mu_);
+    out[0] = groups_; out[1] = members_; out[2] = largest_;
+  }
+  int lane_waiting() {
+    std::lock_guard<std::mutex> lk(mu_);
+    return (int)lane_.size();
+  }
+  int lane_active() {
+    std::lock_guard<std::mutex> lk(mu_);
+    return lane_active_;
+  }
+  void lane_counts(unsigned long long out[3]) {
+    std::lock_guard<std::mutex> lk(mu_);
+    out[0] = lane_groups_; out[1] = lane_members_; out[2] = lane_largest_;
+  }
+
+ private:
+  bool await_locked(std::unique_lock<std::mutex>& lk, ExtGroupWaiter& w, int max_group, ExtGroupWaiter** members, int* n_members) {
     w.cv.wait(lk, [&] { return w.state == ExtGroupWaiter::LEADER || w.state == ExtGroupWaiter::DONE; });
     if (w.state == ExtGroupWaiter::DONE) return false;
     if (w.compatible) {
@@ -55,50 +184,29 @@
     }
     return true;
   }
-
-  void complete(ExtGroupWaiter** members, int n_members, int status, float span_ms) {
-    std::lock_guard<std::mutex> lk(mu_);
-    for (int i = 0; i < n_members; ++i) {
-      ExtGroupWaiter* m = members[i];
-      m->status = status;
-      m->span_ms = span_ms;
-      m->group_n = 1 + n_members;
-      m->state = ExtGroupWaiter::DONE;
-      m->cv.notify_one();
-    }
-  }
-
-  template <class Put, class Take>
-  void release(Put&& put, Take&& take) {
-    std::lock_guard<std::mutex> lk(mu_);
-    put();
-    while (!waiters_.empty()) {
+  template <class Take>
+  void enqueue_locked(ExtGroupWaiter* m, Take&& take) {
+    if (waiters_.empty()) {
       const int s = take();
-      if (s < 0) break;
-      ExtGroupWaiter* w = waiters_.front();
-      waiters_.pop_front();
-      w->slot = s;
-      w->state = ExtGroupWaiter::LEADER;
-      w->cv.notify_one();
-    }
-  }
-
-  int waiting() {
-    std::lock_guard<std::mutex> lk(mu_);
-    return (int)waiters_.size();
-  }
-  int waiting_compatible() {
-    std::lock_guard<std::mutex> lk(mu_);
-    int n = 0;
-    for (const ExtGroupWaiter* w : waiters_) n += w->compatible ? 1 : 0;
-    return n;
-  }
-  void counts(unsigned long long out[3]) {
-    std::lock_guard<std::mutex> lk(mu_);
-    out[0] = groups_; out[1] = members_; out[2] = largest_;
-  }
-
- private:
+      if (s != NO_SLOT) {
+        m->slot = s;
+        m->state = ExtGroupWaiter::LEADER;
+        m->cv.notify_one();
+        return;
+      }
+    }
+    m->state = ExtGroupWaiter::WAITING;
+    waiters_.push_back(m);
+  }
+  void lane_promote(int depth) {
+    if (lane_enqueueing_ || lane_active_ >= (depth < 1 ? 1 : depth) || lane_.empty()) return;
+    ExtGroupWaiter* w = lane_.front();
+    lane_.pop_front();
+    lane_enqueueing_ = true;
+    ++lane_active_;
+    w->state = ExtGroupWaiter::LANE_LEADER;
+    w->cv.notify_one();
+  }
   void count_group(int n) {
     ++groups_;
     members_ += (unsigned long long)n;
@@ -107,6 +215,33 @@
   std::mutex mu_;
   std::deque<ExtGroupWaiter*> waiters_;
   unsigned long long groups_ = 0, members_ = 0, largest_ = 0;
+  std::deque<ExtGroupWaiter*> lane_;
+  bool lane_enqueueing_ = false;
+  int lane_active_ = 0;
+  unsigned long long lane_groups_ = 0, lane_members_ = 0, lane_largest_ = 0;
 };
 
+template <class Copy, class Mark, class Wait, class Drain, class Take>
+int lane_lead(ExtGroupQueue& q, ExtGroupWaiter& w, ExtGroupWaiter** members, int n_members, int depth, Copy&& copy, Mark&& mark, Wait&& wait,
+              Drain&& drain, Take&& take) {
+  struct Guard {
+    ExtGroupQueue& q; ExtGroupWaiter& w; ExtGroupWaiter** m; int n; int depth; Take& take; Drain& drain;
+    int status; bool enqueued;
+    void enqueued_now() { if (!enqueued) { enqueued = true; q.lane_enqueued(depth); } }
+    ~Guard() {
+      enqueued_now();
+      if (status != 0) (void)drain();
+      q.lane_finish(w, m, n, status, depth, take);
+    }
+  } g{q, w, members, n_members, depth, take, drain, -1, false};
+  int st = copy(w);
+  for (int i = 0; st == 0 && i < n_members; ++i) st = copy(*members[i]);
+  if (st == 0) st = mark();
+  g.status = st != 0 ? st : -1;
+  g.enqueued_now();
+  if (st == 0) st = wait();
+  g.status = st;
+  return st;
 }
+
+}
diff --git a/cloud-scale-bwamem_amd/csrc/bpsw_internal.h b/cloud-scale-bwamem_amd/csrc/bpsw_internal.h
--- a/cloud-scale-bwamem_amd/csrc/bpsw_internal.h
+++ b/cloud-scale-bwamem_amd/csrc/bpsw_internal.h
@@ -371,7 +371,7 @@
   bool led = false;
   int slot = -1;
   double wait_ms;
-  explicit StreamLease(bpsw_ctx* c, ExtGroupWaiter* w = nullptr, ExtGroupWaiter** members = nullptr, int* n_members = nullptr);
+  explicit StreamLease(bpsw_ctx* c, ExtGroupWaiter* w = nullptr, ExtGroupWaiter** members = nullptr, int* n_members = nullptr, bool queued = false);
   ~StreamLease();
   StreamLease(const StreamLease&) = delete;
   StreamLease& operator=(const StreamLease&) = delete;
@@ -382,6 +382,10 @@
   hipEvent_t ev = nullptr;
 };
 CopyLane& copy_lane(int device);
+constexpr int EXT_LANE_DEPTH = 2;
+int ext_lane_depth();
+int ext_lane_waiting(int device);
+void ext_lane_counts(int device, unsigned long long out[3]);
 double wall_ms();
 int ext_group_max();
 int ext_group_waiting(int device);
@@ -396,6 +400,7 @@
 bool wait_naps(double est_ms);
 void wait_nap(double est_ms);
 void wait_poll_pause(int polls, double waited_ms, double est_ms);
+hipError_t wait_event_est(hipEvent_t ev, double* est_ms);
 hipError_t wait_event(bpsw_ctx* c, hipEvent_t ev, int kind);
 int zerocopy_mask();
 bool spin_wait();
@@ -483,6 +488,7 @@
   bpsw::PinnedBuffer h_stage_in, h_stage_out, h_pre;
   int shortcut_mask = 63;
   std::vector<int> ext_long_tasks;
+  double lane_wait_est_ms = 0.;
   double wait_est_ms[6] = {0., 0., 0., 0., 0., 0.};
   bool ring_abandoned = false;
   uint32_t ring_seq = 0;
diff --git a/cloud-scale-bwamem_amd/csrc/bpsw_runtime.cpp b/cloud-scale-bwamem_amd/csrc/bpsw_runtime.cpp
--- a/cloud-scale-bwamem_amd/csrc/bpsw_runtime.cpp
+++ b/cloud-scale-bwamem_amd/csrc/bpsw_runtime.cpp
@@ -10,6 +10,7 @@
 
 #pragma weak launch_ext_group
 #include "bpsw_internal.h"
+#include "bpsw_wire_scan_core.h"
 
 namespace bpsw {
 
@@ -184,9 +185,10 @@
   else { timespec ts = {0, 20000}; nanosleep(&ts, nullptr); }
 }
 
-hipError_t wait_event(bpsw_ctx* c, hipEvent_t ev, int kind) {
+hipError_t wait_event(bpsw_ctx* c, hipEvent_t ev, int kind) { return wait_event_est(ev, &c->wait_est_ms[kind & 3]); }
+hipError_t wait_event_est(hipEvent_t ev, double* est_ms) {
   if (spin_wait()) return hipEventSynchronize(ev);
-  double& est = c->wait_est_ms[kind & 3];
+  double& est = *est_ms;
   const double t0 = wall_ms();
   const bool napped = wait_naps(est);
   wait_nap(est);
@@ -270,6 +272,16 @@
   }();
   return n;
 }
+int ext_lane_depth() {
+  static const int n = [] {
+    const char* e = getenv("BPSW_EXT_LANE_DEPTH");
+    const int v = e ? atoi(e) : EXT_LANE_DEPTH;
+    return v < 1 ? 1 : (v > 4 ? 4 : v);
+  }();
+  return n;
+}
+int ext_lane_waiting(int device) { return stream_pool(device).q.lane_waiting(); }
+void ext_lane_counts(int device, unsigned long long out[3]) { stream_pool(device).q.lane_counts(out); }
 int ext_group_waiting(int device) { return stream_pool(device).q.waiting_compatible(); }
 void ext_group_counts(int device, unsigned long long out[3]) { stream_pool(device).q.counts(out); }
 void ext_group_complete(int device, ExtGroupWaiter** members, int n_members, int status, float span_ms) {
@@ -295,7 +307,7 @@
   return ExtGroupQueue::NO_SLOT;
 }
 
-StreamLease::StreamLease(bpsw_ctx* c, ExtGroupWaiter* w, ExtGroupWaiter** members, int* n_members)
+StreamLease::StreamLease(bpsw_ctx* c, ExtGroupWaiter* w, ExtGroupWaiter** members, int* n_members, bool queued)
     : device(c->device), s(c->stream), pooled(false), wait_ms(0.) {
   int none = 0;
   if (n_members) *n_members = 0;
@@ -306,7 +318,8 @@
   ExtGroupWaiter alone;
   if (!w) w = &alone;
   ExtGroupWaiter* no_members[1];
-  const bool leads = P.q.acquire(*w, members ? ext_group_max() : 1, [&] { return pool_take(P, cap); }, members ? members : no_members, n_members ? n_members : &none);
+  const bool leads = queued ? P.q.await(*w, members ? ext_group_max() : 1, members ? members : no_members, n_members ? n_members : &none)
+                            : P.q.acquire(*w, members ? ext_group_max() : 1, [&] { return pool_take(P, cap); }, members ? members : no_members, n_members ? n_members : &none);
   wait_ms = wall_ms() - t0;
   if (!leads) { led = true; return; }
   if (w->slot < 0) return;
@@ -461,63 +474,16 @@
 
 
 
-static inline int rd16(const uint8_t* b, size_t at) { return (int16_t)(b[at] | (b[at + 1] << 8)); }
-static inline int rd32(const uint8_t* b, size_t at) {
-  return (int32_t)((uint32_t)b[at] | ((uint32_t)b[at + 1] << 8) | ((uint32_t)b[at + 2] << 16) | ((uint32_t)b[at + 3] << 24));
-}
+static inline int rd32(const uint8_t* b, size_t at) { return wire_rd32(b, at); }
 
 static int scan_wire(const uint8_t* wire, size_t bytes, long long l_pac, int* n_out, int* maxq, int* maxr, bool* coord,
                      std::vector<int>* long_tasks, int* maxr_short, int* n_mid_out) {
-  if (!wire || bytes < 32 || (bytes & 3)) return fail(BPSW_ERR_ARG, "extend: wire batch shorter than its header or not word sized");
-  const int n = rd32(wire, 8);
-  const int fmt = wire[7];
-  if (fmt != 0 && fmt != BPSW_WIRE_COORDS) return fail(BPSW_ERR_ARG, "extend: unknown wire format (header byte 7)");
-  const bool co = fmt == BPSW_WIRE_COORDS;
-  const size_t rec_bytes = co ? 40 : 32;
-  if (n < 0 || 32 + rec_bytes * (size_t)n > bytes) return fail(BPSW_ERR_ARG, "extend: task table exceeds the buffer");
-  if ((int8_t)wire[0] < 0 || (int8_t)wire[1] < 1 || (int8_t)wire[2] < 0 || (int8_t)wire[3] < 1)
-    return fail(BPSW_ERR_ARG, "extend: gap opens must be >= 0 and gap extensions >= 1 (a zero extension divides by zero in SWUtil.scala:110-115)");
-  if ((int8_t)wire[6] < 0) return fail(BPSW_ERR_ARG, "extend: negative band width (w travels as a signed byte: at most 127)");
-  if (co && l_pac <= 0) return fail(BPSW_ERR_ARG, "extend: a coordinate batch needs the reference on the device (bpsw_ref_load)");
-  const int wband = (int8_t)wire[6];
-  int mq = 0, mr = 0, mrs = 0;
-  const size_t words = bytes >> 2;
-  const bool all_long = (int8_t)wire[2] + (int8_t)wire[3] <= 0;
-  long_tasks->clear();
-  int mid = 0;
-  for (int t = 0; t < n; ++t) {
-    const size_t at = 32 + rec_bytes * (size_t)t;
-    const int lq = rd16(wire, at), lr = rd16(wire, at + 2), rq = rd16(wire, at + 4), rr = rd16(wire, at + 6);
-    if (lq < 0 || lr < 0 || rq < 0 || rr < 0) return fail(BPSW_ERR_ARG, "extend: negative sequence length in task table");
-    const long long pos = rd32(wire, at + 8);
-    const long long w = co ? ((long long)lq + rq + 7) / 8 : ((long long)lq + lr + rq + rr + 7) / 8;
-    if (pos < 8 + (long long)(rec_bytes / 4) * n || (unsigned long long)(pos + w) > words)
-      return fail(BPSW_ERR_ARG, "extend: task sequence offset outside the buffer");
-    if (lq > mq) mq = lq;
-    if (rq > mq) mq = rq;
-    const bool is_long = all_long || lq > 255 || rq > 255;
-    const bool is_mid = !is_long && (lq > 127 || rq > 127);
-    if (is_mid) ++mid;
-    if (is_long) long_tasks->push_back(t);
-    int task_mr = 0;
-    if (co) {
-      const int len = rd16(wire, at + 18);
-      long long rb;
-      memcpy(&rb, wire + at + 32, 8);
-      if (rb < 0 || rb > (l_pac << 1)) return fail(BPSW_ERR_ARG, "extend: task window outside the reference or bridging its two strands");
-      const long long lo = rb - lr, hi = rb + len + rr;
-      if (len < 0 || lo < 0 || hi > (l_pac << 1) || (lo < l_pac && hi > l_pac))
-        return fail(BPSW_ERR_ARG, "extend: task window outside the reference or bridging its two strands");
-      const int sl = std::min(lr, lq + 2 * wband + 2), sr = std::min(rr, rq + 2 * wband + 2);
-      task_mr = std::max(sl, sr);
-    } else {
-      task_mr = std::max(lr, rr);
-    }
-    if (task_mr > mr) mr = task_mr;
-    if (!is_long && task_mr > mrs) mrs = task_mr;
-  }
-  if (mq > BPSW_EXT_MAX_QLEN || mr > BPSW_EXT_MAX_RLEN) return fail(BPSW_ERR_LIMIT, "extend: sequence longer than the kernel limit");
-  *n_out = n; *maxq = mq; *maxr = mr; *coord = co; *maxr_short = mrs; *n_mid_out = mid;
+  static const bool fast = !(getenv("BPSW_EXT_SCAN_FAST") && atoi(getenv("BPSW_EXT_SCAN_FAST")) == 0);
+  WireScan ws;
+  const char* msg = nullptr;
+  const int rc = wire_scan(wire, bytes, l_pac, &ws, long_tasks, &msg, fast);
+  if (rc != BPSW_OK) return fail(rc, msg);
+  *n_out = ws.n; *maxq = ws.maxq; *maxr = ws.maxr; *coord = ws.coord; *maxr_short = ws.maxr_short; *n_mid_out = ws.n_mid;
   return BPSW_OK;
 }
 
@@ -565,6 +531,10 @@
   const void* copy_src = nullptr;
   size_t copy_bytes = 0;
   double enqueued_at = 0.;
+  void* lane_dst = nullptr;
+  const void* lane_src = nullptr;
+  size_t lane_bytes = 0;
+  double copied_at = 0.;
 };
 
 static int extend_batch_impl(bpsw_ctx_t* c, const uint8_t* wire, size_t wire_bytes, int16_t* out, size_t out_len, uint8_t* side_how,
@@ -676,17 +646,6 @@
   }
   if (!via_ring) {
     const bool copy_first = sw_launches_in_flight(c->device) > 0;
-    if (copy_first) {
-      const double t_c0 = stat_ms();
-      CopyLane& L = copy_lane(c->device);
-      {
-        std::lock_guard<std::mutex> lk(L.mu);
-        if (!L.s) HIP_TRY(hipStreamCreateWithFlags(&L.s, hipStreamNonBlocking));
-        HIP_TRY(hipMemcpyAsync(c->d_wire.ptr, c->h_stage_in.ptr, stage_bytes, hipMemcpyHostToDevice, L.s));
-        HIP_TRY(hipStreamSynchronize(L.s));
-      }
-      copy_first_ms = stat_ms() - t_c0;
-    }
     const bool zc_out = (zerocopy_mask() & 1) != 0;
     int16_t* k_out = zc_out ? (int16_t*)c->h_stage_out.ptr : (int16_t*)c->d_out.ptr;
     int* const d_queue_words = (int*)((char*)c->d_pre.ptr + 128);
@@ -708,10 +667,66 @@
     gw.item = &me;
     ExtGroupWaiter* led[EXT_GROUP_SLOTS];
     int n_led = 0;
-    const double t_ready = stat_ms();
-    StreamLease lease(c, &gw, groupable ? led : nullptr, groupable ? &n_led : nullptr);
+    double t_ready = 0.;
+    bool lane_queued = false;
+    if (copy_first && ext_group_max() > 1 && stream_pool_cap() > 0) {
+      static const bool lane_poll = !(getenv("BPSW_EXT_LANE_POLL") && atoi(getenv("BPSW_EXT_LANE_POLL")) == 0);
+      const double t_c0 = stat_ms();
+      StreamPool& P = stream_pool(c->device);
+      const int cap = stream_pool_cap(), depth = ext_lane_depth();
+      me.lane_dst = c->d_wire.ptr; me.lane_src = c->h_stage_in.ptr; me.lane_bytes = stage_bytes;
+      ExtGroupWaiter* cm[EXT_GROUP_SLOTS];
+      int n_cm = 0;
+      if (P.q.lane_enter(gw, ext_group_max(), depth, cm, &n_cm)) {
+        CopyLane& L = copy_lane(c->device);
+        static const int lane_hold_us = getenv("BPSW_EXT_LANE_HOLD_US") ? atoi(getenv("BPSW_EXT_LANE_HOLD_US")) : 0;
+        if (lane_hold_us > 0) { timespec ts = {lane_hold_us / 1000000, (long)(lane_hold_us % 1000000) * 1000}; nanosleep(&ts, nullptr); }
+        const int st = lane_lead(
+            P.q, gw, cm, n_cm, depth,
+            [&](ExtGroupWaiter& w) -> int {
+              if (!L.s) {
+                const hipError_t e = hipStreamCreateWithFlags(&L.s, hipStreamNonBlocking);
+                if (e != hipSuccess) return (int)e;
+              }
+              const ExtCallItem* it = (const ExtCallItem*)w.item;
+              return (int)hipMemcpyAsync(it->lane_dst, it->lane_src, it->lane_bytes, hipMemcpyHostToDevice, L.s);
+            },
+            [&]() -> int { return (int)hipEventRecord(c->ev[0], L.s); },
+            [&]() -> int {
+              const hipError_t e = lane_poll ? wait_event_est(c->ev[0], &c->lane_wait_est_ms) : hipEventSynchronize(c->ev[0]);
+              const double now = wall_ms();
+              me.copied_at = now;
+              for (int i = 0; i < n_cm; ++i) ((ExtCallItem*)cm[i]->item)->copied_at = now;
+              return (int)e;
+            },
+            [&]() -> int { return L.s ? (int)hipStreamSynchronize(L.s) : 0; },
+            [&] { return pool_take(P, cap); });
+        if (st != 0) return hip_fail((hipError_t)st, "extend: the copies of a group on the copy lane");
+        t_ready = stat_ms();
+      } else {
+        if (gw.state == ExtGroupWaiter::DONE && gw.lane_failed)
+          return hip_fail((hipError_t)gw.status, "extend: the copy group this call's batch was copied with");
+        const double now = stat_ms();
+        t_ready = std::min(now, std::max(t_c0, now - std::max(0., wall_ms() - me.copied_at)));
+      }
+      copy_first_ms = t_ready - t_c0;
+      lane_queued = true;
+    } else if (copy_first) {
+      const double t_c0 = stat_ms();
+      CopyLane& L = copy_lane(c->device);
+      {
+        std::lock_guard<std::mutex> lk(L.mu);
+        if (!L.s) HIP_TRY(hipStreamCreateWithFlags(&L.s, hipStreamNonBlocking));
+        HIP_TRY(hipMemcpyAsync(c->d_wire.ptr, c->h_stage_in.ptr, stage_bytes, hipMemcpyHostToDevice, L.s));
+        HIP_TRY(hipStreamSynchronize(L.s));
+      }
+      copy_first_ms = stat_ms() - t_c0;
+    }
+    if (!lane_queued) t_ready = stat_ms();
+    StreamLease lease(c, &gw, groupable ? led : nullptr, groupable ? &n_led : nullptr, lane_queued);
     hipStream_t s = lease.s;
     t_dev0 = stat_ms();
+    const double lease_wait_ms = lane_queued ? std::max(0., t_dev0 - t_ready) : lease.wait_ms;
     const auto late_full = [&](hipStream_t ls) -> int {
       KernelEvents kev;
       kev.start = c->ev[4]; kev.stop = c->ev[5];
@@ -772,7 +787,7 @@
         float span = 0.f;
         (void)hipEventElapsedTime(&span, c->ev[1], c->ev[2]);
         group_span_ms = done.span = span;
-        c->stats.ext_wait_ms += lease.wait_ms;
+        c->stats.ext_wait_ms += lease_wait_ms;
       }
     }
     if (grouped) {
@@ -843,7 +858,7 @@
         if (lrc != BPSW_OK) return lrc;
       }
       t_dev1 = stat_ms();
-      c->stats.ext_wait_ms += lease.wait_ms;
+      c->stats.ext_wait_ms += lease_wait_ms;
     }
   }
   if (out_view) {
@@ -965,6 +980,14 @@
 }
 
 int bpsw_ext_group_waiting(int device) { return device >= 0 && device < 64 ? bpsw::ext_group_waiting(device) : -1; }
+int bpsw_ext_lane_waiting(int device) { return device >= 0 && device < 64 ? bpsw::ext_lane_waiting(device) : -1; }
+int bpsw_ext_lane_counts(int device, uint64_t out[3]) {
+  if (!out || device < 0 || device >= 64) return fail(BPSW_ERR_ARG, "ext_lane_counts: bad argument");
+  unsigned long long v[3];
+  bpsw::ext_lane_counts(device, v);
+  for (int i = 0; i < 3; ++i) out[i] = (uint64_t)v[i];
+  return BPSW_OK;
+}
 int bpsw_ext_group_counts(int device, uint64_t out[3]) {
   if (!out || device < 0 || device >= 64) return fail(BPSW_ERR_ARG, "ext_group_counts: bad argument");
   unsigned long long v[3];
diff --git a/cloud-scale-bwamem_amd/csrc/bpsw_wire_scan_core.h b/cloud-scale-bwamem_amd/csrc/bpsw_wire_scan_core.h
--- /dev/null
+++ b/cloud-scale-bwamem_amd/csrc/bpsw_wire_scan_core.h
@@ -0,0 +1,110 @@
+#pragma once
+
+#include <algorithm>
+#include <cstdint>
+#include <cstring>
+#include <vector>
+
+#include "bpsw.h"
+
+namespace bpsw {
+
+struct WireScan {
+  int n = 0, maxq = 0, maxr = 0;
+  bool coord = false;
+  int maxr_short = 0;
+  int n_mid = 0;
+};
+
+static inline int wire_rd16(const uint8_t* b, size_t at) { return (int16_t)(b[at] | (b[at + 1] << 8)); }
+static inline int wire_rd32(const uint8_t* b, size_t at) {
+  return (int32_t)((uint32_t)b[at] | ((uint32_t)b[at + 1] << 8) | ((uint32_t)b[at + 2] << 16) | ((uint32_t)b[at + 3] << 24));
+}
+
+static inline int wire_scan(const uint8_t* wire, size_t bytes, long long l_pac, WireScan* out, std::vector<int>* long_tasks, const char** msg,
+                            bool fast = true) {
+#define BPSW_SCAN_FAIL(code, text) do { *msg = (text); return (code); } while (0)
+  if (!wire || bytes < 32 || (bytes & 3)) BPSW_SCAN_FAIL(BPSW_ERR_ARG, "extend: wire batch shorter than its header or not word sized");
+  const int n = wire_rd32(wire, 8);
+  const int fmt = wire[7];
+  if (fmt != 0 && fmt != BPSW_WIRE_COORDS) BPSW_SCAN_FAIL(BPSW_ERR_ARG, "extend: unknown wire format (header byte 7)");
+  const bool co = fmt == BPSW_WIRE_COORDS;
+  const size_t rec_bytes = co ? 40 : 32;
+  if (n < 0 || 32 + rec_bytes * (size_t)n > bytes) BPSW_SCAN_FAIL(BPSW_ERR_ARG, "extend: task table exceeds the buffer");
+  if ((int8_t)wire[0] < 0 || (int8_t)wire[1] < 1 || (int8_t)wire[2] < 0 || (int8_t)wire[3] < 1)
+    BPSW_SCAN_FAIL(BPSW_ERR_ARG, "extend: gap opens must be >= 0 and gap extensions >= 1 (a zero extension divides by zero in SWUtil.scala:110-115)");
+  if ((int8_t)wire[6] < 0) BPSW_SCAN_FAIL(BPSW_ERR_ARG, "extend: negative band width (w travels as a signed byte: at most 127)");
+  if (co && l_pac <= 0) BPSW_SCAN_FAIL(BPSW_ERR_ARG, "extend: a coordinate batch needs the reference on the device (bpsw_ref_load)");
+  const int wband = (int8_t)wire[6];
+  int mq = 0, mr = 0, mrs = 0;
+  const size_t words = bytes >> 2;
+  const bool all_long = (int8_t)wire[2] + (int8_t)wire[3] <= 0;
+  long_tasks->clear();
+  int mid = 0;
+  int t = 0;
+  if (fast && !co && !all_long) {
+    constexpr int BLOCK = 64;
+    const long long pos_lo = 8 + 8 * (long long)n;
+    while (t < n) {
+      const int m = std::min(BLOCK, n - t);
+      const uint8_t* rec = wire + 32 + 32 * (size_t)t;
+      uint64_t flag = 0;
+      int bq = 0, br = 0;
+      for (int i = 0; i < m; ++i) {
+        uint64_t len4;
+        uint32_t pos32;
+        memcpy(&len4, rec + 32 * (size_t)i, 8);
+        memcpy(&pos32, rec + 32 * (size_t)i + 8, 4);
+        const int lq = (int)(len4 & 0xffff), lr = (int)((len4 >> 16) & 0xffff), rq = (int)((len4 >> 32) & 0xffff), rr = (int)(len4 >> 48);
+        flag |= len4 & 0x8000ff808000ff80ull;
+        const long long pos = (int32_t)pos32;
+        const long long w = ((long long)lq + lr + rq + rr + 7) >> 3;
+        flag |= (uint64_t)(pos < pos_lo) | (uint64_t)((unsigned long long)(pos + w) > words);
+        bq = std::max(bq, std::max(lq, rq));
+        br = std::max(br, std::max(lr, rr));
+      }
+      if (flag) break;
+      mq = std::max(mq, bq);
+      mr = std::max(mr, br);
+      mrs = std::max(mrs, br);
+      t += m;
+    }
+  }
+  for (; t < n; ++t) {
+    const size_t at = 32 + rec_bytes * (size_t)t;
+    const int lq = wire_rd16(wire, at), lr = wire_rd16(wire, at + 2), rq = wire_rd16(wire, at + 4), rr = wire_rd16(wire, at + 6);
+    if (lq < 0 || lr < 0 || rq < 0 || rr < 0) BPSW_SCAN_FAIL(BPSW_ERR_ARG, "extend: negative sequence length in task table");
+    const long long pos = wire_rd32(wire, at + 8);
+    const long long w = co ? ((long long)lq + rq + 7) / 8 : ((long long)lq + lr + rq + rr + 7) / 8;
+    if (pos < 8 + (long long)(rec_bytes / 4) * n || (unsigned long long)(pos + w) > words)
+      BPSW_SCAN_FAIL(BPSW_ERR_ARG, "extend: task sequence offset outside the buffer");
+    if (lq > mq) mq = lq;
+    if (rq > mq) mq = rq;
+    const bool is_long = all_long || lq > 255 || rq > 255;
+    const bool is_mid = !is_long && (lq > 127 || rq > 127);
+    if (is_mid) ++mid;
+    if (is_long) long_tasks->push_back(t);
+    int task_mr = 0;
+    if (co) {
+      const int len = wire_rd16(wire, at + 18);
+      long long rb;
+      memcpy(&rb, wire + at + 32, 8);
+      if (rb < 0 || rb > (l_pac << 1)) BPSW_SCAN_FAIL(BPSW_ERR_ARG, "extend: task window outside the reference or bridging its two strands");
+      const long long lo = rb - lr, hi = rb + len + rr;
+      if (len < 0 || lo < 0 || hi > (l_pac << 1) || (lo < l_pac && hi > l_pac))
+        BPSW_SCAN_FAIL(BPSW_ERR_ARG, "extend: task window outside the reference or bridging its two strands");
+      const int sl = std::min(lr, lq + 2 * wband + 2), sr = std::min(rr, rq + 2 * wband + 2);
+      task_mr = std::max(sl, sr);
+    } else {
+      task_mr = std::max(lr, rr);
+    }
+    if (task_mr > mr) mr = task_mr;
+    if (!is_long && task_mr > mrs) mrs = task_mr;
+  }
+  if (mq > BPSW_EXT_MAX_QLEN || mr > BPSW_EXT_MAX_RLEN) BPSW_SCAN_FAIL(BPSW_ERR_LIMIT, "extend: sequence longer than the kernel limit");
+#undef BPSW_SCAN_FAIL
+  out->n = n; out->maxq = mq; out->maxr = mr; out->coord = co; out->maxr_short = mrs; out->n_mid = mid;
+  return BPSW_OK;
+}
+
+}
diff --git a/include/bpsw.h b/include/bpsw.h
--- a/include/bpsw.h
+++ b/include/bpsw.h
@@ -407,6 +407,8 @@
 int bpsw_sw_batches_in_flight(int device);
 int bpsw_ext_group_waiting(int device);
 int bpsw_ext_group_counts(int device, uint64_t out[3]);
+int bpsw_ext_lane_waiting(int device);
+int bpsw_ext_lane_counts(int device, uint64_t out[3]);
 
 #ifdef __cplusplus
 }
```

Result: slower. 276.9 million (-1.0%).
